# kazuto1011/dusty-gan-v2

Measured on AMD Instinct MI355X. Metric: range-images/sec (G+D step) on dusty_v2 64x512, higher is better.
Workload: dtype bf16; 1 GPU; configs[2]: configs/gans/dusty_v2.yaml full G+D train step (G step + D step + lazy R1 + ADA + EMA + Adam), 64x512 synthetic; global_batch=64, per_gpu_batch=64, parallelism=dp1, hip_graph=True, d_epilogue_dtype=fp32, pe_table_precomputed=True

## Files before the change

dusty-gan-v2_amd/csrc/api.hip:

```cpp
#include "common.h"

extern "C" int dgv2_abi_version(void) { return 53; }
```

dusty-gan-v2_amd/csrc/gemm.hip:

```cpp
#include "gemm_core.h"

namespace {

template <typename T, typename TY, int TO>
int launch_bmm_nn(void* y, const void* x, const void* w, int B, int P, int I, int O, int ldx, int ldy,
                  int64_t wstride, const float* bias, int act, float alpha, float scale, hipStream_t st, float* sumsq,
                  int sumsq_cap, int* sumsq_used, const float* row_scale, const void* resid) {
  constexpr int CE = 16 / sizeof(T);
  DenseRowLoader<T> al{(const T*)w, wstride, I, O, I, (I % CE == 0) && (wstride % CE == 0) && aligned16(w)};
  DenseRowLoader<T> bl{(const T*)x, (int64_t)P * ldx, ldx, P, I, (ldx % CE == 0) && aligned16(x)};
  constexpr int YE = 16 / sizeof(TY);
  StoreEpilogue<TY> epi{(TY*)y, (int64_t)P * ldy, ldy, O, P,
                        (ldy % 4 == 0) && ((reinterpret_cast<uintptr_t>(y) & (4 * sizeof(TY) - 1)) == 0),
                        bias, act, alpha, scale, nullptr, 0.f, row_scale, (const TY*)resid};
  (void)YE;
  dim3 grid((P + 127) / 128, (O + TO - 1) / TO, B);
  const int64_t nblk = (int64_t)grid.x * grid.y * grid.z;
  if (sumsq && sumsq_used && nblk <= sumsq_cap) {
    epi.sumsq = sumsq;
    *sumsq_used = (int)nblk;
  }
  gemm_nn_kernel<T, TO, DenseRowLoader<T>, DenseRowLoader<T>, StoreEpilogue<TY>><<<grid, 256, 0, st>>>(al, bl, epi, I);
  return 0;
}

template <typename T, typename TY>
int dispatch_bmm_nn(void* y, const void* x, const void* w, int B, int P, int I, int O, int ldx, int ldy,
                    int64_t wstride, const float* bias, int act, float alpha, float scale, hipStream_t st, float* sumsq,
                    int sumsq_cap, int* sumsq_used, const float* row_scale, const void* resid) {
  if (O <= 16) return launch_bmm_nn<T, TY, 16>(y, x, w, B, P, I, O, ldx, ldy, wstride, bias, act, alpha, scale, st, sumsq, sumsq_cap, sumsq_used, row_scale, resid);
  if (O <= 32) return launch_bmm_nn<T, TY, 32>(y, x, w, B, P, I, O, ldx, ldy, wstride, bias, act, alpha, scale, st, sumsq, sumsq_cap, sumsq_used, row_scale, resid);
  if (O <= 64) return launch_bmm_nn<T, TY, 64>(y, x, w, B, P, I, O, ldx, ldy, wstride, bias, act, alpha, scale, st, sumsq, sumsq_cap, sumsq_used, row_scale, resid);
  return launch_bmm_nn<T, TY, 128>(y, x, w, B, P, I, O, ldx, ldy, wstride, bias, act, alpha, scale, st, sumsq, sumsq_cap, sumsq_used, row_scale, resid);
}

template <typename T, int TO, int TJ>
int launch_bmm_tn(float* gw, const void* gy, const void* x, int B, int P, int I, int O, int ldgy, int ldx,
                  int ksplit, hipStream_t st) {
  constexpr int CE = 16 / sizeof(T);
  DenseKLoader<T> al{(const T*)gy, (int64_t)P * ldgy, ldgy, O, (ldgy % CE == 0) && aligned16(gy)};
  DenseKLoader<T> bl{(const T*)x, (int64_t)P * ldx, ldx, I, (ldx % CE == 0) && aligned16(x)};
  const int64_t klen = (((int64_t)P + ksplit - 1) / ksplit + 31) / 32 * 32;
  dim3 grid((I + TJ - 1) / TJ, (O + TO - 1) / TO, B * ksplit);
  gemm_tn_kernel<T, TO, TJ, DenseKLoader<T>, DenseKLoader<T>><<<grid, 256, 0, st>>>(al, bl, gw, O, I, P, klen, ksplit,
                                                                                   (int64_t)O * I, I);
  return 0;
}

template <typename T, typename TY, int TO>
int launch_bmm_nn_cat(void* y, const void* xa, const void* xs, const void* w, int B, int P, int Ka, int Ks, int O,
                      const float* bias, int act, float alpha, float scale, hipStream_t st, float* sumsq, int sumsq_cap,
                      int* sumsq_used, const float* row_scale) {
  const int K = Ka + Ks;
  DenseRowLoader<T> al{(const T*)w, (int64_t)O * K, K, O, K, true};
  ConcatRowLoader<T> bl{(const T*)xa, (int64_t)P * Ka, Ka, Ka, (const T*)xs, Ks, Ks, P};
  StoreEpilogue<TY> epi{(TY*)y, (int64_t)P * O, O, O, P, (O % 4 == 0), bias, act, alpha, scale, nullptr, 0.f, row_scale};
  dim3 grid(B, (O + TO - 1) / TO, (P + 127) / 128);
  const int64_t nblk = (int64_t)grid.x * grid.y * grid.z;
  if (sumsq && sumsq_used && nblk <= sumsq_cap) {
    epi.sumsq = sumsq;
    *sumsq_used = (int)nblk;
  }
  gemm_nn_kernel<T, TO, DenseRowLoader<T>, ConcatRowLoader<T>, StoreEpilogue<TY>, true><<<grid, 256, 0, st>>>(al, bl, epi, K);
  return 0;
}

template <typename T, typename TY>
int dispatch_bmm_nn_cat(void* y, const void* xa, const void* xs, const void* w, int B, int P, int Ka, int Ks, int O,
                        const float* bias, int act, float alpha, float scale, hipStream_t st, float* sumsq, int sumsq_cap,
                        int* sumsq_used, const float* row_scale) {
  if (O <= 16) return launch_bmm_nn_cat<T, TY, 16>(y, xa, xs, w, B, P, Ka, Ks, O, bias, act, alpha, scale, st, sumsq, sumsq_cap, sumsq_used, row_scale);
  if (O <= 32) return launch_bmm_nn_cat<T, TY, 32>(y, xa, xs, w, B, P, Ka, Ks, O, bias, act, alpha, scale, st, sumsq, sumsq_cap, sumsq_used, row_scale);
  if (O <= 64) return launch_bmm_nn_cat<T, TY, 64>(y, xa, xs, w, B, P, Ka, Ks, O, bias, act, alpha, scale, st, sumsq, sumsq_cap, sumsq_used, row_scale);
  return launch_bmm_nn_cat<T, TY, 128>(y, xa, xs, w, B, P, Ka, Ks, O, bias, act, alpha, scale, st, sumsq, sumsq_cap, sumsq_used, row_scale);
}

template <typename T, int TO, int TJ>
int launch_bmm_tn_cat(float* gw, const void* gy, const void* xa, const void* xs, int B, int P, int Ca, int Cs, int O,
                      int ksplit, hipStream_t st) {
  constexpr int CE = 16 / sizeof(T);
  const int J = Ca + Cs;
  DenseKLoader<T> al{(const T*)gy, (int64_t)P * O, O, O, (O % CE == 0) && aligned16(gy)};
  ConcatKLoader<T> bl{(const T*)xa, (int64_t)P * Ca, Ca, Ca, (const T*)xs, Cs, Cs};
  const int64_t klen = (((int64_t)P + ksplit - 1) / ksplit + 31) / 32 * 32;
  dim3 grid((J + TJ - 1) / TJ, (O + TO - 1) / TO, B * ksplit);
  gemm_tn_kernel<T, TO, TJ, DenseKLoader<T>, ConcatKLoader<T>><<<grid, 256, 0, st>>>(al, bl, gw, O, J, P, klen, ksplit,
                                                                                  (int64_t)O * J, J);
  return 0;
}

}

extern "C" int dgv2_bmm_nn(void* y, const void* x, const void* w, int B, int P, int I, int O, int ldx, int ldy,
                           int64_t wstride, const float* bias, int act, float alpha, float scale, int dtype,
                           int ydtype, void* stream) {
  return dgv2_bmm_nn_sq(y, x, w, B, P, I, O, ldx, ldy, wstride, nullptr, bias, act, alpha, scale, nullptr, dtype, ydtype,
                        nullptr, 0, nullptr, stream);
}

extern "C" int dgv2_bmm_nn_sq(void* y, const void* x, const void* w, int B, int P, int I, int O, int ldx, int ldy,
                              int64_t wstride, const float* row_scale, const float* bias, int act, float alpha,
                              float scale, const void* resid, int dtype, int ydtype, float* sumsq, int sumsq_cap,
                              int* sumsq_used, void* stream) {
  if (sumsq_used) *sumsq_used = 0;
  if (!y || !x || !w || B <= 0 || P <= 0 || I <= 0 || O <= 0 || ldx < I || ldy < O) return DGV2_EINVAL;
  if (act != 0 && act != 3) return DGV2_EINVAL;
  hipStream_t st = (hipStream_t)stream;
  if (dtype == DGV2_F32 && ydtype == DGV2_F32)
    dispatch_bmm_nn<float, float>(y, x, w, B, P, I, O, ldx, ldy, wstride, bias, act, alpha, scale, st, sumsq, sumsq_cap, sumsq_used, row_scale, resid);
  else if (dtype == DGV2_BF16 && ydtype == DGV2_BF16)
    dispatch_bmm_nn<bf16_t, bf16_t>(y, x, w, B, P, I, O, ldx, ldy, wstride, bias, act, alpha, scale, st, sumsq, sumsq_cap, sumsq_used, row_scale, resid);
  else if (dtype == DGV2_BF16 && ydtype == DGV2_F32)
    dispatch_bmm_nn<bf16_t, float>(y, x, w, B, P, I, O, ldx, ldy, wstride, bias, act, alpha, scale, st, sumsq, sumsq_cap, sumsq_used, row_scale, resid);
  else
    return DGV2_EINVAL;
  DGV2_RETURN_LAST();
}

extern "C" int dgv2_bmm_tn(float* gw, const void* gy, const void* x, int B, int P, int I, int O, int ldgy, int ldx,
                           int dtype, void* stream) {
  if (!gw || !gy || !x || B <= 0 || P <= 0 || I <= 0 || O <= 0 || ldgy < O || ldx < I) return DGV2_EINVAL;
  hipStream_t st = (hipStream_t)stream;
  const int tiles = B * ((O + 63) / 64) * ((I + 127) / 128);
  int ksplit = 1;
  while (tiles * ksplit < 512 && P / (ksplit * 2) >= 512) ksplit *= 2;
  if (ksplit > 1) {
    hipError_t e = hipMemsetAsync(gw, 0, sizeof(float) * (size_t)B * O * I, st);
    if (e != hipSuccess) return (int)e;
  }
  DGV2_DISPATCH_DTYPE(dtype, {
    if (O <= 16) launch_bmm_tn<T, 16, 128>(gw, gy, x, B, P, I, O, ldgy, ldx, ksplit, st);
    else if (O <= 32) launch_bmm_tn<T, 32, 128>(gw, gy, x, B, P, I, O, ldgy, ldx, ksplit, st);
    else launch_bmm_tn<T, 64, 128>(gw, gy, x, B, P, I, O, ldgy, ldx, ksplit, st);
  });
  DGV2_RETURN_LAST();
}

extern "C" int dgv2_bmm_nn_cat(void* y, const void* xa, const void* xs, const void* w, int B, int P, int Ka, int Ks,
                               int O, const float* bias, int act, float alpha, float scale, int dtype, int ydtype,
                               void* stream) {
  return dgv2_bmm_nn_cat_sq(y, xa, xs, w, B, P, Ka, Ks, O, nullptr, bias, act, alpha, scale, dtype, ydtype, nullptr, 0, nullptr,
                            stream);
}

extern "C" int dgv2_bmm_nn_cat_sq(void* y, const void* xa, const void* xs, const void* w, int B, int P, int Ka, int Ks,
                                  int O, const float* row_scale, const float* bias, int act, float alpha, float scale, int dtype, int ydtype,
                                  float* sumsq, int sumsq_cap, int* sumsq_used, void* stream) {
  if (sumsq_used) *sumsq_used = 0;
  if (!y || !xs || !w || (Ka > 0 && !xa) || B <= 0 || P <= 0 || Ka < 0 || Ks <= 0 || O <= 0) return DGV2_EINVAL;
  if (act != 0 && act != 3) return DGV2_EINVAL;
  const int ce = dtype == DGV2_BF16 ? 8 : 4;
  if (Ka % ce || Ks % ce || !aligned16(xs) || (Ka > 0 && !aligned16(xa)) || !aligned16(w) || !aligned16(y))
    return DGV2_EINVAL;
  hipStream_t st = (hipStream_t)stream;
  if (dtype == DGV2_F32 && ydtype == DGV2_F32)
    dispatch_bmm_nn_cat<float, float>(y, xa, xs, w, B, P, Ka, Ks, O, bias, act, alpha, scale, st, sumsq, sumsq_cap, sumsq_used, row_scale);
  else if (dtype == DGV2_BF16 && ydtype == DGV2_BF16)
    dispatch_bmm_nn_cat<bf16_t, bf16_t>(y, xa, xs, w, B, P, Ka, Ks, O, bias, act, alpha, scale, st, sumsq, sumsq_cap, sumsq_used, row_scale);
  else
    return DGV2_EINVAL;
  DGV2_RETURN_LAST();
}

extern "C" int dgv2_bmm_tn_cat(float* gw, const void* gy, const void* xa, const void* xs, int B, int P, int Ka,
                               int Ks, int O, int dtype, void* stream) {
  if (!gw || !gy || !xs || (Ka > 0 && !xa) || B <= 0 || P <= 0 || Ka < 0 || Ks <= 0 || O <= 0) return DGV2_EINVAL;
  const int ce = dtype == DGV2_BF16 ? 8 : 4;
  if (Ka % ce || Ks % ce || !aligned16(xs) || (Ka > 0 && !aligned16(xa))) return DGV2_EINVAL;
  hipStream_t st = (hipStream_t)stream;
  const int J = Ka + Ks;
  const int tiles = B * ((O + 63) / 64) * ((J + 127) / 128);
  int ksplit = 1;
  while (tiles * ksplit < 512 && P / (ksplit * 2) >= 512) ksplit *= 2;
  if (ksplit > 1) {
    hipError_t e = hipMemsetAsync(gw, 0, sizeof(float) * (size_t)B * O * J, st);
    if (e != hipSuccess) return (int)e;
  }
  DGV2_DISPATCH_DTYPE(dtype, {
    if (O <= 16) launch_bmm_tn_cat<T, 16, 128>(gw, gy, xa, xs, B, P, Ka, Ks, O, ksplit, st);
    else if (O <= 32) launch_bmm_tn_cat<T, 32, 128>(gw, gy, xa, xs, B, P, Ka, Ks, O, ksplit, st);
    else launch_bmm_tn_cat<T, 64, 128>(gw, gy, xa, xs, B, P, Ka, Ks, O, ksplit, st);
  });
  DGV2_RETURN_LAST();
}

namespace {

template <typename T, int O>
__global__ __launch_bounds__(256) void bmm_tn_small_kernel(float* __restrict__ gw, const T* __restrict__ gy,
                                                           const T* __restrict__ x, int P, int I, int ppb) {
  constexpr int VN = vec16<T>::N;
  __shared__ float red[256 * VN];
  const int b = blockIdx.y;
  const int cvecs = I / VN, lanes = 256 / cvecs;
  const int cv = threadIdx.x % cvecs, pl = threadIdx.x / cvecs;
  const int p0 = blockIdx.x * ppb, p1 = min(p0 + ppb, P);
  float acc[O][VN];
#pragma unroll
  for (int o = 0; o < O; ++o)
#pragma unroll
    for (int j = 0; j < VN; ++j) acc[o][j] = 0.f;
  const T* xb = x + (int64_t)b * P * I;
  const T* gb = gy + (int64_t)b * P * O;
  constexpr int U = 4;
  for (int p = p0 + pl; p < p1; p += lanes * U) {
    vec16<T> v[U];
    float g[U][O];
#pragma unroll
    for (int u = 0; u < U; ++u) {
      const int q = p + u * lanes;
      const int qc = min(q, p1 - 1);
      v[u].load(xb + (int64_t)qc * I + cv * VN);
#pragma unroll
      for (int o = 0; o < O; ++o) g[u][o] = q < p1 ? to_f32(gb[(int64_t)qc * O + o]) : 0.f;
    }
#pragma unroll
    for (int u = 0; u < U; ++u)
#pragma unroll
      for (int o = 0; o < O; ++o)
#pragma unroll
        for (int j = 0; j < VN; ++j) acc[o][j] = fmaf(g[u][o], v[u].get(j), acc[o][j]);
  }
#pragma unroll
  for (int o = 0; o < O; ++o) {
    __syncthreads();
#pragma unroll
    for (int j = 0; j < VN; ++j) red[threadIdx.x * VN + j] = acc[o][j];
    __syncthreads();
    for (int c = threadIdx.x; c < I; c += 256) {
      const int v = c / VN, j = c - v * VN;
      float s = 0.f;
      for (int k = 0; k < lanes; ++k) s += red[(k * cvecs + v) * VN + j];
      gw[((int64_t)b * O + o) * I + c] = s;
    }
  }
}

}

extern "C" int dgv2_bmm_tn_small(float* gw, const void* gy, const void* x, int B, int P, int I, int O, int dtype,
                                 void* stream) {
  if (!gw || !gy || !x || B <= 0 || P <= 0 || I <= 0 || O <= 0) return DGV2_EINVAL;
  const int vn = dtype == DGV2_BF16 ? 8 : (dtype == DGV2_F32 ? 4 : 0);
  if (!vn) return DGV2_EINVAL;
  if (O > 4 || I % vn || 256 % (I / vn) || !aligned16(x)) return DGV2_ENOTSUP;
  hipStream_t st = (hipStream_t)stream;
  const int ppb = P;
  dim3 grid(1, B);
  DGV2_DISPATCH_DTYPE(dtype, {
    switch (O) {
      case 1: bmm_tn_small_kernel<T, 1><<<grid, 256, 0, st>>>(gw, (const T*)gy, (const T*)x, P, I, ppb); break;
      case 2: bmm_tn_small_kernel<T, 2><<<grid, 256, 0, st>>>(gw, (const T*)gy, (const T*)x, P, I, ppb); break;
      case 3: bmm_tn_small_kernel<T, 3><<<grid, 256, 0, st>>>(gw, (const T*)gy, (const T*)x, P, I, ppb); break;
      default: bmm_tn_small_kernel<T, 4><<<grid, 256, 0, st>>>(gw, (const T*)gy, (const T*)x, P, I, ppb); break;
    }
  });
  DGV2_RETURN_LAST();
}

namespace {

template <typename T, int O, bool ACT>
__global__ __launch_bounds__(256) void bmm_nn_small_kernel(T* __restrict__ y, const T* __restrict__ x,
                                                           const T* __restrict__ w, const T* __restrict__ resid, int P,
                                                           int K, int ppb, const T* __restrict__ ref = nullptr,
                                                           const float* __restrict__ row_scale = nullptr, float alpha = 1.f,
                                                           float ascale = 1.f, float* __restrict__ partial = nullptr) {
  constexpr int VN = vec16<T>::N;
  __shared__ float red[ACT ? 256 * VN : 1];
  const int b = blockIdx.y;
  const int kvecs = K / VN, lanes = 256 / kvecs;
  const int kv = threadIdx.x % kvecs, pl = threadIdx.x / kvecs;
  float wr[VN][O];
#pragma unroll
  for (int j = 0; j < VN; ++j)
#pragma unroll
    for (int o = 0; o < O; ++o) wr[j][o] = to_f32(w[((int64_t)b * K + kv * VN + j) * O + o]);
  const int p0 = blockIdx.x * ppb, p1 = min(p0 + ppb, P);
  const T* xb = x + (int64_t)b * P * O;
  float rs[VN], bsum[VN];
#pragma unroll
  for (int j = 0; j < VN; ++j) {
    rs[j] = (ACT && row_scale) ? row_scale[kv * VN + j] : 1.f;
    bsum[j] = 0.f;
  }
  for (int p = p0 + pl; p < p1; p += lanes) {
    float g[O];
#pragma unroll
    for (int o = 0; o < O; ++o) g[o] = to_f32(xb[(int64_t)p * O + o]);
    const int64_t off = ((int64_t)b * P + p) * K + kv * VN;
    vec16<T> r, f, out;
    if (resid) r.load(resid + off);
    if constexpr (ACT) f.load(ref + off);
#pragma unroll
    for (int j = 0; j < VN; ++j) {
      float s = resid ? r.get(j) : 0.f;
#pragma unroll
      for (int o = 0; o < O; ++o) s = fmaf(g[o], wr[j][o], s);
      if constexpr (ACT) {
        const float v = (f.get(j) > 0.f ? s : s * alpha) * ascale;
        out.set(j, v);
        bsum[j] += out.get(j);
        out.set(j, v * rs[j]);
      } else {
        out.set(j, s);
      }
    }
    out.store(y + off);
  }
  if constexpr (ACT) {
#pragma unroll
    for (int j = 0; j < VN; ++j) red[threadIdx.x * VN + j] = bsum[j];
    __syncthreads();
    for (int c = threadIdx.x; c < K; c += 256) {
      const int v = c / VN, j = c - v * VN;
      float s2 = 0.f;
      for (int t = 0; t < lanes; ++t) s2 += red[(t * kvecs + v) * VN + j];
      partial[((int64_t)blockIdx.y * gridDim.x + blockIdx.x) * K + c] = s2;
    }
  }
}

__global__ __launch_bounds__(256) void small_bias_reduce_kernel(float* __restrict__ gb, const float* __restrict__ partial,
                                                             int nblk, int C) {
  __shared__ float red[16];
  const int c = blockIdx.x;
  float s = 0.f;
#pragma unroll 4
  for (int k = threadIdx.x; k < nblk; k += 256) s += partial[(int64_t)k * C + c];
  s = block_sum(s, red);
  if (threadIdx.x == 0) gb[c] = s;
}

}

namespace {

template <typename T, int O>
__global__ __launch_bounds__(256) void head_bwd_kernel(T* __restrict__ y, const float* __restrict__ gyf,
                                                       const float* __restrict__ cvec, const T* __restrict__ w,
                                                       const T* __restrict__ resid, const T* __restrict__ ref, int P, int K,
                                                       int ppb, const float* __restrict__ row_scale, float alpha,
                                                       float ascale, float* __restrict__ p_gb, float* __restrict__ p_gw,
                                                       float* __restrict__ p_gbh) {
  constexpr int VN = vec16<T>::N;
  __shared__ float red[256 * VN];
  const int b = blockIdx.y;
  const int kvecs = K / VN, lanes = 256 / kvecs;
  const int kv = threadIdx.x % kvecs, pl = threadIdx.x / kvecs;
  float wr[VN][O], cv[O];
#pragma unroll
  for (int j = 0; j < VN; ++j)
#pragma unroll
    for (int o = 0; o < O; ++o) wr[j][o] = to_f32(w[((int64_t)b * K + kv * VN + j) * O + o]);
#pragma unroll
  for (int o = 0; o < O; ++o) cv[o] = cvec[o];
  const int p0 = blockIdx.x * ppb, p1 = min(p0 + ppb, P);
  const float* gb_ = gyf + (int64_t)b * P * O;
  float rs[VN], bsum[VN], hw[O][VN], hb[O];
#pragma unroll
  for (int j = 0; j < VN; ++j) {
    rs[j] = row_scale ? row_scale[kv * VN + j] : 1.f;
    bsum[j] = 0.f;
#pragma unroll
    for (int o = 0; o < O; ++o) hw[o][j] = 0.f;
  }
#pragma unroll
  for (int o = 0; o < O; ++o) hb[o] = 0.f;
  for (int p = p0 + pl; p < p1; p += lanes) {
    float g[O];
#pragma unroll
    for (int o = 0; o < O; ++o) {
      const float raw = gb_[(int64_t)p * O + o];
      if (kv == 0) hb[o] += raw;
      g[o] = to_f32(from_f32<T>(raw * cv[o]));
    }
    const int64_t off = ((int64_t)b * P + p) * K + kv * VN;
    vec16<T> r, f, out;
    if (resid) r.load(resid + off);
    f.load(ref + off);
#pragma unroll
    for (int j = 0; j < VN; ++j) {
      const float xv = f.get(j);
      float s = resid ? r.get(j) : 0.f;
#pragma unroll
      for (int o = 0; o < O; ++o) {
        s = fmaf(g[o], wr[j][o], s);
        hw[o][j] = fmaf(g[o], xv, hw[o][j]);
      }
      const float v = (xv > 0.f ? s : s * alpha) * ascale;
      out.set(j, v);
      bsum[j] += out.get(j);
      out.set(j, v * rs[j]);
    }
    out.store(y + off);
  }
  const int64_t blk = (int64_t)blockIdx.y * gridDim.x + blockIdx.x;
#pragma unroll
  for (int q = 0; q <= O; ++q) {
    __syncthreads();
#pragma unroll
    for (int j = 0; j < VN; ++j) red[threadIdx.x * VN + j] = q == 0 ? bsum[j] : hw[q > 0 ? q - 1 : 0][j];
    __syncthreads();
    for (int c = threadIdx.x; c < K; c += 256) {
      const int v = c / VN, j = c - v * VN;
      float s2 = 0.f;
      for (int t = 0; t < lanes; ++t) s2 += red[(t * kvecs + v) * VN + j];
      if (q == 0) p_gb[blk * K + c] = s2;
      else p_gw[(blk * O + (q - 1)) * K + c] = s2;
    }
  }
  __syncthreads();
#pragma unroll
  for (int o = 0; o < O; ++o) red[threadIdx.x * O + o] = kv == 0 ? hb[o] : 0.f;
  __syncthreads();
  if (threadIdx.x < O) {
    float s2 = 0.f;
    for (int t = 0; t < 256; ++t) s2 += red[t * O + threadIdx.x];
    p_gbh[blk * O + threadIdx.x] = s2;
  }
}

__global__ __launch_bounds__(256) void head_bwd_reduce_kernel(float* __restrict__ gb, float* __restrict__ gw,
                                                              float* __restrict__ gbh, const float* __restrict__ p_gb,
                                                              const float* __restrict__ p_gw, const float* __restrict__ p_gbh,
                                                              int nsplit, int B, int O, int K) {
  __shared__ float red[16];
  const int nblk = nsplit * B;
  int id = blockIdx.x;
  if (id < K) {
    float s = 0.f;
#pragma unroll 4
    for (int k = threadIdx.x; k < nblk; k += 256) s += p_gb[(int64_t)k * K + id];
    s = block_sum(s, red);
    if (threadIdx.x == 0) gb[id] = s;
    return;
  }
  id -= K;
  if (id < B * O) {
    const int b = id / O, o = id - b * O;
    for (int c = threadIdx.x; c < K; c += 256) {
      float s = 0.f;
      for (int k = 0; k < nsplit; ++k) s += p_gw[(((int64_t)b * nsplit + k) * O + o) * K + c];
      gw[((int64_t)b * O + o) * K + c] = s;
    }
    return;
  }
  id -= B * O;
  float s = 0.f;
  for (int k = threadIdx.x; k < nblk; k += 256) s += p_gbh[(int64_t)k * O + id];
  s = block_sum(s, red);
  if (threadIdx.x == 0) gbh[id] = s;
}

}

extern "C" int dgv2_head_bwd(void* y, float* gw, float* gbh, float* gb_up, float* scratch, int64_t scratch_elems,
                             int64_t* blocks_needed, const float* gyf, const float* cvec, const void* w, const void* resid,
                             const void* ref, const float* row_scale, float alpha, float ascale, int B, int P, int O, int K,
                             int dtype, void* stream) {
  if (B <= 0 || P <= 0 || O <= 0 || K <= 0) return DGV2_EINVAL;
  const int vn = dtype == DGV2_BF16 ? 8 : (dtype == DGV2_F32 ? 4 : 0);
  if (!vn) return DGV2_EINVAL;
  if (O > 4 || K % vn || 256 % (K / vn)) return DGV2_ENOTSUP;
  const int lanes = 256 / (K / vn);
  int nsplit = (2048 + B - 1) / B;
  const int minpix = lanes * 8;
  if ((int64_t)nsplit * minpix > P) nsplit = (P + minpix - 1) / minpix;
  nsplit = nsplit < 1 ? 1 : nsplit;
  const int ppb = (P + nsplit - 1) / nsplit;
  dim3 grid((P + ppb - 1) / ppb, B);
  const int64_t nblk = (int64_t)grid.x * grid.y;
  if (blocks_needed) *blocks_needed = nblk;
  if (blocks_needed && !y) return 0;
  if (!y || !gw || !gbh || !gb_up || !scratch || !gyf || !cvec || !w || !ref) return DGV2_EINVAL;
  if (scratch_elems < nblk * ((int64_t)K + (int64_t)O * K + O)) return DGV2_EINVAL;
// ... 67 lines not shown
```

dusty-gan-v2_amd/csrc/gemm_core.h:

```cpp
#pragma once
#include "common.h"

template <typename T> struct Mfma16;

template <> struct Mfma16<bf16_t> {
  __device__ static __forceinline__ void run(f32x4& acc, const uint4& a, const uint4& b) {
    union { uint4 u; bf16x8 v; } ua, ub;
    ua.u = a;
    ub.u = b;
    acc = __builtin_amdgcn_mfma_f32_16x16x32_bf16(ua.v, ub.v, acc, 0, 0, 0);
  }
};

template <> struct Mfma16<fp8_t> {
  __device__ static __forceinline__ void run(f32x4& acc, const uint4& a, const uint4& b) {
    const long a0 = (long)(((unsigned long)a.y << 32) | a.x), a1 = (long)(((unsigned long)a.w << 32) | a.z);
    const long b0 = (long)(((unsigned long)b.y << 32) | b.x), b1 = (long)(((unsigned long)b.w << 32) | b.z);
    acc = __builtin_amdgcn_mfma_f32_16x16x32_fp8_fp8(a0, b0, acc, 0, 0, 0);
    acc = __builtin_amdgcn_mfma_f32_16x16x32_fp8_fp8(a1, b1, acc, 0, 0, 0);
  }
};

template <> struct Mfma16<float> {
  __device__ static __forceinline__ void run(f32x4& acc, const uint4& a, const uint4& b) {
// ... 138 lines not shown
      }
    return v.raw;
  }
};

template <typename T> struct Im2colDgradLoader {
  const T* gy;
  ConvGeom g;
  int Hp, Wp, npix, K;
  bool vec;
  __device__ __forceinline__ const T* src(int b, int hp, int wp, int kk, int& o) const {
    const int tap = kk / g.O;
    o = kk - tap * g.O;
    const int ky = tap / g.kw, kx = tap - ky * g.kw;
    const int nh = hp - ky, nw = wp - kx;
    if (nh < 0 || nw < 0 || nh % g.stride != 0 || nw % g.stride != 0) return nullptr;
    const int ho = nh / g.stride, wo = nw / g.stride;
    if (ho >= g.Ho || wo >= g.Wo) return nullptr;
    return gy + (((int64_t)b * g.Ho + ho) * g.Wo + wo) * g.O;
  }
  __device__ __forceinline__ uint4 load(int, int row, int kchunk) const {
    constexpr int CE = 16 / sizeof(T);
    const int k = kchunk * CE;
    if (row >= npix || k >= K) return make_uint4(0, 0, 0, 0);
    const int wp = row % Wp;
    const int t = row / Wp;
    const int hp = t % Hp;
    const int b = t / Hp;
    int o;
    if (vec) {
      const T* p = src(b, hp, wp, k, o);
      return p ? *reinterpret_cast<const uint4*>(p + o) : make_uint4(0, 0, 0, 0);
    }
    vec16<T> v;
    v.raw = make_uint4(0, 0, 0, 0);
#pragma unroll
    for (int j = 0; j < CE; ++j)
      if (k + j < K) {
        const T* p = src(b, hp, wp, k + j, o);
        if (p) v.e[j] = p[o];
      }
    return v.raw;
  }
};

template <typename T, int TO, class ALoad, class BLoad, class Epi, bool BATCH_FAST = false>
__global__ __launch_bounds__(256) void gemm_nn_kernel(ALoad al, BLoad bl, Epi epi, int K) {
  constexpr int TP = 128;
  constexpr int MF = TO / 16;
  constexpr int NF = 2;
  constexpr int CE = 16 / sizeof(T);
  constexpr int ACH = (TO * 4 + 255) / 256;
  __shared__ __attribute__((aligned(16))) uint4 ldsA[2][TO * 4];
  __shared__ __attribute__((aligned(16))) uint4 ldsB[2][TP * 4];

  const int tid = threadIdx.x;
  const int wave = tid >> 6, lane = tid & 63;
  const int lr = lane & 15, lc = lane >> 4;
  const int batch = BATCH_FAST ? blockIdx.x : blockIdx.z;
  const int m0 = blockIdx.y * TO;
  const int n0 = (BATCH_FAST ? blockIdx.z : blockIdx.x) * TP;
  const int nk = (K + 4 * CE - 1) / (4 * CE);

  uint4 ra[ACH], rb[2];
  auto swz = [](int row, int ch) { return row * 4 + (ch ^ ((row >> 2) & 3)); };
  auto gload = [&](int kt) {
#pragma unroll
    for (int i = 0; i < 2; ++i) {
      const int id = tid + i * 256;
      rb[i] = bl.load(batch, n0 + (id >> 2), kt * 4 + (id & 3));
    }
#pragma unroll
    for (int i = 0; i < ACH; ++i) {
      const int id = tid + i * 256;
      if (id < TO * 4) ra[i] = al.load(batch, m0 + (id >> 2), kt * 4 + (id & 3));
    }
  };
  auto lstore = [&](int buf) {
#pragma unroll
    for (int i = 0; i < 2; ++i) {
      const int id = tid + i * 256;
      ldsB[buf][swz(id >> 2, id & 3)] = rb[i];
    }
#pragma unroll
    for (int i = 0; i < ACH; ++i) {
      const int id = tid + i * 256;
      if (id < TO * 4) ldsA[buf][swz(id >> 2, id & 3)] = ra[i];
    }
  };

  f32x4 acc[MF][NF];
#pragma unroll
  for (int mf = 0; mf < MF; ++mf)
#pragma unroll
    for (int nf = 0; nf < NF; ++nf) acc[mf][nf] = (f32x4){0.f, 0.f, 0.f, 0.f};

  gload(0);
  lstore(0);
  __syncthreads();
  int cur = 0;
  for (int kt = 0; kt < nk; ++kt) {
    if (kt + 1 < nk) gload(kt + 1);
    uint4 a[MF], b[NF];
#pragma unroll
    for (int mf = 0; mf < MF; ++mf) a[mf] = ldsA[cur][swz(mf * 16 + lr, lc)];
#pragma unroll
    for (int nf = 0; nf < NF; ++nf) b[nf] = ldsB[cur][swz(wave * 32 + nf * 16 + lr, lc)];
#pragma unroll
    for (int mf = 0; mf < MF; ++mf)
#pragma unroll
      for (int nf = 0; nf < NF; ++nf) Mfma16<T>::run(acc[mf][nf], a[mf], b[nf]);
    if (kt + 1 < nk) lstore(cur ^ 1);
    __syncthreads();
    cur ^= 1;
  }
#pragma unroll
  for (int mf = 0; mf < MF; ++mf)
#pragma unroll
    for (int nf = 0; nf < NF; ++nf)
      epi(batch, m0 + mf * 16 + lc * 4, n0 + wave * 32 + nf * 16 + lr, acc[mf][nf]);
  if (epi.sumsq) {
    __shared__ float red[16];
    const float s = block_sum(epi.ss, red);
    if (tid == 0) epi.sumsq[(blockIdx.z * gridDim.y + blockIdx.y) * gridDim.x + blockIdx.x] = s;
  }
}

template <typename TY> struct StoreEpilogue {
  TY* y;
  int64_t batch_stride;
  int ld, M, N;
  bool vec;
  const float* bias;
  int act;
  float alpha, scale;
  float* sumsq;
  float ss;
  const float* row_scale;
  const TY* resid;
  __device__ __forceinline__ void operator()(int batch, int m, int n, f32x4 acc) {
    if (n >= N || m >= M) return;
    if (row_scale) {
#pragma unroll
      for (int r = 0; r < 4; ++r)
        if (m + r < M) acc[r] *= row_scale[m + r];
    }
    if (bias || act) {
#pragma unroll
      for (int r = 0; r < 4; ++r) {
        float v = acc[r];
        if (bias && m + r < M) v += bias[m + r];
        if (act == 3) v = (v > 0.f ? v : v * alpha) * scale;
        acc[r] = v;
      }
    }
    TY* p = y + batch * batch_stride + (int64_t)n * ld + m;
    if (resid) {
      const TY* rp = resid + batch * batch_stride + (int64_t)n * ld + m;
      if (vec && m + 3 < M) {
        if constexpr (sizeof(TY) == 4) {
          const f32x4 rv = *reinterpret_cast<const f32x4*>(rp);
#pragma unroll
          for (int r = 0; r < 4; ++r) acc[r] += rv[r];
        } else {
          union { uint2 u; bf16_t e[4]; } rv;
          rv.u = *reinterpret_cast<const uint2*>(rp);
#pragma unroll
          for (int r = 0; r < 4; ++r) acc[r] += (float)rv.e[r];
        }
      } else {
#pragma unroll
        for (int r = 0; r < 4; ++r)
          if (m + r < M) acc[r] += to_f32(rp[r]);
      }
    }
    if (sumsq) {
#pragma unroll
      for (int r = 0; r < 4; ++r)
        if (m + r < M) {
          const float v = to_f32(from_f32<TY>(acc[r]));
          ss = fmaf(v, v, ss);
        }
    }
    if (vec && m + 3 < M) {
      if constexpr (sizeof(TY) == 4) {
        *reinterpret_cast<f32x4*>(p) = acc;
      } else {
        union { uint2 u; bf16_t e[4]; } o;
#pragma unroll
        for (int r = 0; r < 4; ++r) o.e[r] = (bf16_t)acc[r];
        *reinterpret_cast<uint2*>(p) = o.u;
      }
    } else {
#pragma unroll
      for (int r = 0; r < 4; ++r)
        if (m + r < M) p[r] = from_f32<TY>(acc[r]);
    }
  }
};

template <typename T> struct DenseKLoader {
  const T* base;
  int64_t batch_stride;
  int ld, cols;
  bool vec;
  __device__ __forceinline__ uint4 load(int batch, int64_t k, int64_t K, int colchunk) const {
    constexpr int CE = 16 / sizeof(T);
    const int col = colchunk * CE;
    if (k >= K || col >= cols) return make_uint4(0, 0, 0, 0);
    const T* p = base + batch * batch_stride + k * ld + col;
    if (vec && col + CE <= cols) return *reinterpret_cast<const uint4*>(p);
    vec16<T> v;
    v.raw = make_uint4(0, 0, 0, 0);
#pragma unroll
    for (int j = 0; j < CE; ++j)
      if (col + j < cols) v.e[j] = p[j];
    return v.raw;
  }
};

template <typename T> struct ConcatKLoader {
  const T* a;
  int64_t a_batch_stride;
  int lda, Ca;
  const T* s;
  int lds_, Cs;
  __device__ __forceinline__ uint4 load(int batch, int64_t k, int64_t K, int colchunk) const {
    constexpr int CE = 16 / sizeof(T);
    const int col = colchunk * CE;
    if (k >= K) return make_uint4(0, 0, 0, 0);
    if (col < Ca) return *reinterpret_cast<const uint4*>(a + batch * a_batch_stride + k * lda + col);
    const int c2 = col - Ca;
    if (c2 + CE <= Cs) return *reinterpret_cast<const uint4*>(s + k * lds_ + c2);
    return make_uint4(0, 0, 0, 0);
  }
};

template <typename T> struct Im2colWgradLoader {
  const T* x;
  ConvGeom g;
  int cols;
  bool vec;
  __device__ __forceinline__ uint4 load(int, int64_t k, int64_t K, int colchunk) const {
    constexpr int CE = 16 / sizeof(T);
    const int col = colchunk * CE;
    if (k >= K || col >= cols) return make_uint4(0, 0, 0, 0);
    const int wo = (int)(k % g.Wo);
    const int64_t t = k / g.Wo;
    const int ho = (int)(t % g.Ho);
    const int b = (int)(t / g.Ho);
    vec16<T> v;
    v.raw = make_uint4(0, 0, 0, 0);
    if (vec) {
      const int tap = col / g.C, c = col - tap * g.C;
      const int ky = tap / g.kw, kx = tap - ky * g.kw;
      const int hi = conv_src_h(g, ho * g.stride + ky - g.pad);
      const int wi = conv_src_w(g, wo * g.stride + kx - g.pad);
      return *reinterpret_cast<const uint4*>(x + (((int64_t)b * g.H + hi) * g.W + wi) * g.C + c);
    }
#pragma unroll
    for (int j = 0; j < CE; ++j)
      if (col + j < cols) {
        const int cc = col + j;
        const int tap = cc / g.C, c = cc - tap * g.C;
        const int ky = tap / g.kw, kx = tap - ky * g.kw;
        const int hi = conv_src_h(g, ho * g.stride + ky - g.pad);
        const int wi = conv_src_w(g, wo * g.stride + kx - g.pad);
        v.e[j] = x[(((int64_t)b * g.H + hi) * g.W + wi) * g.C + c];
      }
    return v.raw;
  }
};

template <typename T> struct TnFrag;

template <> struct TnFrag<bf16_t> {
  static constexpr int KS = 32;
  template <int ROWLEN>
  __device__ static __forceinline__ uint4 read(const bf16_t* tile, int c0, int lane) {
    const int g = lane >> 4, i = lane & 15;
    const int q = i >> 2, p = i & 3;
    typedef __attribute__((address_space(3))) s16x4 lds_s16x4;
    const bf16_t* a0 = tile + (8 * g + q) * ROWLEN + c0 + 4 * p;
    const bf16_t* a1 = a0 + 4 * ROWLEN;
    union { uint4 u; s16x4 h[2]; } r;
    r.h[0] = __builtin_amdgcn_ds_read_tr16_b64_v4i16((lds_s16x4*)a0);
    r.h[1] = __builtin_amdgcn_ds_read_tr16_b64_v4i16((lds_s16x4*)a1);
    return r.u;
  }
};

template <> struct TnFrag<float> {
  static constexpr int KS = 16;
  template <int ROWLEN>
  __device__ static __forceinline__ uint4 read(const float* tile, int c0, int lane) {
    const int g = lane >> 4, i = lane & 15;
    union { uint4 u; float f[4]; } r;
#pragma unroll
    for (int s = 0; s < 4; ++s) r.f[s] = tile[(4 * s + g) * ROWLEN + c0 + i];
    return r.u;
  }
};

template <typename T, int TO, int TJ, class ALoad, class BLoad>
__global__ __launch_bounds__(256) void gemm_tn_kernel(ALoad al, BLoad bl, float* __restrict__ out, int M, int J,
                                                      int64_t K, int64_t klen, int ksplit, int64_t out_batch_stride,
                                                      int ldo) {
  constexpr int KS = TnFrag<T>::KS;
  constexpr int CE = 16 / sizeof(T);
  constexpr int MF = TO / 16;
  constexpr int NF = TJ / 64;
  constexpr int ACH_ROW = TO / CE, BCH_ROW = TJ / CE;
  constexpr int ACH = (KS * ACH_ROW + 255) / 256, BCH = (KS * BCH_ROW + 255) / 256;
  __shared__ __attribute__((aligned(16))) T ldsA[2][KS * TO];
  __shared__ __attribute__((aligned(16))) T ldsB[2][KS * TJ];

  const int tid = threadIdx.x;
  const int wave = tid >> 6, lane = tid & 63;
  const int batch = blockIdx.z / ksplit;
  const int ks = blockIdx.z % ksplit;
  const int m0 = blockIdx.y * TO;
  const int j0 = blockIdx.x * TJ;
  const int64_t kbeg = ks * klen;
  const int64_t kend = (kbeg + klen < K) ? kbeg + klen : K;
  const int nk = (int)((kend - kbeg + KS - 1) / KS);

  uint4 ra[ACH], rb[BCH];
  auto gload = [&](int kt) {
    const int64_t kb = kbeg + (int64_t)kt * KS;
#pragma unroll
    for (int i = 0; i < ACH; ++i) {
      const int id = tid + i * 256;
      if (id < KS * ACH_ROW) ra[i] = al.load(batch, kb + id / ACH_ROW, kend, (m0 / CE) + id % ACH_ROW);
    }
#pragma unroll
    for (int i = 0; i < BCH; ++i) {
      const int id = tid + i * 256;
      if (id < KS * BCH_ROW) rb[i] = bl.load(batch, kb + id / BCH_ROW, kend, (j0 / CE) + id % BCH_ROW);
    }
  };
  auto lstore = [&](int buf) {
#pragma unroll
    for (int i = 0; i < ACH; ++i) {
      const int id = tid + i * 256;
      if (id < KS * ACH_ROW) reinterpret_cast<uint4*>(ldsA[buf])[id] = ra[i];
    }
#pragma unroll
    for (int i = 0; i < BCH; ++i) {
      const int id = tid + i * 256;
      if (id < KS * BCH_ROW) reinterpret_cast<uint4*>(ldsB[buf])[id] = rb[i];
    }
  };

  f32x4 acc[MF][NF];
#pragma unroll
  for (int mf = 0; mf < MF; ++mf)
#pragma unroll
    for (int nf = 0; nf < NF; ++nf) acc[mf][nf] = (f32x4){0.f, 0.f, 0.f, 0.f};

  if (nk > 0) {
    gload(0);
    lstore(0);
  }
  __syncthreads();
  int cur = 0;
  for (int kt = 0; kt < nk; ++kt) {
    if (kt + 1 < nk) gload(kt + 1);
    uint4 a[MF], b[NF];
#pragma unroll
    for (int mf = 0; mf < MF; ++mf) a[mf] = TnFrag<T>::template read<TO>(ldsA[cur], mf * 16, lane);
#pragma unroll
    for (int nf = 0; nf < NF; ++nf) b[nf] = TnFrag<T>::template read<TJ>(ldsB[cur], wave * (TJ / 4) + nf * 16, lane);
#pragma unroll
    for (int mf = 0; mf < MF; ++mf)
#pragma unroll
      for (int nf = 0; nf < NF; ++nf) Mfma16<T>::run(acc[mf][nf], a[mf], b[nf]);
    if (kt + 1 < nk) lstore(cur ^ 1);
    __syncthreads();
    cur ^= 1;
  }
  const int lr = lane & 15, lc = lane >> 4;
  float* ob = out + batch * out_batch_stride;
#pragma unroll
  for (int mf = 0; mf < MF; ++mf)
#pragma unroll
    for (int nf = 0; nf < NF; ++nf) {
      const int j = j0 + wave * (TJ / 4) + nf * 16 + lr;
      if (j >= J) continue;
#pragma unroll
      for (int r = 0; r < 4; ++r) {
        const int m = m0 + mf * 16 + lc * 4 + r;
        if (m < M) {
          float* p = ob + (int64_t)m * ldo + j;
          if (ksplit > 1) atomicAdd(p, acc[mf][nf][r]);
          else *p = acc[mf][nf][r];
        }
      }
    }
}
```

dusty-gan-v2_amd/dgv2_native/__init__.py:

```python
import ctypes
import os

import torch

_HERE = os.path.dirname(os.path.abspath(__file__))
LIB_PATH = os.environ.get("DGV2_LIB_PATH") or os.path.join(os.path.dirname(_HERE), "lib", "libdgv2.so")

F32, BF16 = 0, 1
ABI_VERSION = 53

_c_int, _c_i64, _c_f32, _c_ptr = ctypes.c_int, ctypes.c_int64, ctypes.c_float, ctypes.c_void_p

SIGNATURES = {
    "dgv2_abi_version": [],
    "dgv2_fused_bias_act": [_c_ptr] * 4 + [_c_i64] * 3 + [_c_int, _c_int, _c_f32, _c_f32, _c_int, _c_ptr],
    "dgv2_bias_grad": [_c_ptr, _c_ptr, _c_i64, _c_i64, _c_i64, _c_int, _c_ptr],
    "dgv2_bias_act_bwd": [_c_ptr] * 4 + [_c_i64, _c_int, _c_f32, _c_f32, _c_ptr, _c_i64, _c_int, _c_ptr],
    "dgv2_bias_act_bwd_rs": [_c_ptr] * 4 + [_c_i64, _c_int, _c_f32, _c_f32, _c_ptr, _c_ptr, _c_i64, _c_int, _c_ptr],
    "dgv2_surface_normal": [_c_ptr, _c_ptr] + [_c_int] * 5 + [_c_ptr],
    "dgv2_mbstd_cat_fwd": [_c_ptr] * 3 + [_c_int] * 7 + [_c_ptr],
    "dgv2_mbstd_cat_bwd": [_c_ptr] * 3 + [_c_int] * 7 + [_c_ptr],
    "dgv2_gemm_x3": [_c_ptr, _c_ptr, _c_i64, _c_ptr, _c_ptr, _c_int, _c_int, _c_i64, _c_int, _c_int, _c_i64, _c_i64, _c_i64,
                     _c_int, _c_f32, _c_ptr],
    "dgv2_pe_wgrad_scratch": [_c_ptr] + [_c_int] * 4,
    "dgv2_pe_wgrad": [_c_ptr, _c_ptr, _c_i64, _c_ptr, _c_ptr] + [_c_int] * 4 + [_c_i64, _c_int, _c_ptr],
    "dgv2_mbstd_cat_fwd_x": [_c_ptr] * 3 + [_c_int] * 8 + [_c_ptr],
    "dgv2_mbstd_cat_bwd_x": [_c_ptr] * 3 + [_c_int] * 8 + [_c_ptr],
    "dgv2_scale_cast": [_c_ptr] * 3 + [_c_i64, _c_int, _c_int, _c_int, _c_ptr],
    "dgv2_upfirdn2d": [_c_ptr] * 3 + [_c_int] * 15 + [_c_ptr],
    "dgv2_resample": [_c_ptr] * 4 + [_c_int] * 19 + [_c_ptr],
    "dgv2_resample_tab": [_c_ptr] * 5 + [_c_int] + [_c_ptr] * 3 + [_c_int] * 10 + [_c_ptr],
    "dgv2_resample_tab_add": [_c_ptr] * 6 + [_c_int] + [_c_ptr] * 3 + [_c_int] * 8 + [_c_ptr],
    "dgv2_resample_tab_add_affine": [_c_ptr] * 8 + [_c_int] + [_c_ptr] * 3 + [_c_int] * 8 + [_c_ptr],
    "dgv2_fourier_feature": [_c_ptr] * 5 + [_c_int] * 8 + [_c_ptr],
    "dgv2_downsample_angle": [_c_ptr] * 4 + [_c_int] * 5 + [_c_ptr],
    "dgv2_bmm_nn": [_c_ptr] * 3 + [_c_int] * 6 + [_c_i64, _c_ptr, _c_int, _c_f32, _c_f32, _c_int, _c_int, _c_ptr],
    "dgv2_bmm_tn": [_c_ptr] * 3 + [_c_int] * 7 + [_c_ptr],
    "dgv2_bmm_nn_cat": [_c_ptr] * 4 + [_c_int] * 5 + [_c_ptr, _c_int, _c_f32, _c_f32, _c_int, _c_int, _c_ptr],
    "dgv2_bmm_nn_cat_sq": [_c_ptr] * 4 + [_c_int] * 5 + [_c_ptr, _c_ptr, _c_int, _c_f32, _c_f32, _c_int, _c_int, _c_ptr, _c_int, _c_ptr,
                           _c_ptr],
    "dgv2_bmm_nn_sq": [_c_ptr] * 3 + [_c_int] * 6 + [_c_i64, _c_ptr, _c_ptr, _c_int, _c_f32, _c_f32, _c_ptr, _c_int, _c_int, _c_ptr, _c_int,
                       _c_ptr, _c_ptr],
    "dgv2_modconv_pe_fwd": [_c_ptr] * 4 + [_c_int] * 5 + [_c_ptr, _c_int, _c_f32, _c_f32, _c_int, _c_ptr],
    "dgv2_modconv_pe_fwd_sq": [_c_ptr] * 4 + [_c_int] * 5 + [_c_ptr, _c_ptr, _c_int, _c_f32, _c_f32, _c_int, _c_ptr, _c_int, _c_ptr,
                               _c_ptr],
    "dgv2_modconv_pe_fwd_head": [_c_ptr] * 4 + [_c_int] * 5 + [_c_ptr, _c_ptr, _c_int, _c_f32, _c_f32, _c_int, _c_ptr, _c_int, _c_ptr,
                                 _c_ptr, _c_ptr, _c_ptr],
    "dgv2_kitti_rows": [_c_ptr, _c_ptr, _c_ptr, _c_int, _c_int, _c_ptr],
    "dgv2_kitti_project": [_c_ptr] * 4 + [_c_int] * 4 + [_c_f32, _c_f32, _c_int, _c_ptr],
    "dgv2_fps_scratch": [_c_ptr, _c_int, _c_int],
    "dgv2_fps": [_c_ptr] * 3 + [_c_int] * 3 + [_c_ptr],
    "dgv2_gather_points": [_c_ptr] * 3 + [_c_int] * 4 + [_c_ptr],
    "dgv2_gather_points_grad": [_c_ptr] * 3 + [_c_int] * 4 + [_c_ptr],
    "dgv2_chamfer_fwd": [_c_ptr] * 6 + [_c_int] * 3 + [_c_ptr],
    "dgv2_nn_search": [_c_ptr] * 4 + [_c_int] * 4 + [_c_ptr],
    "dgv2_chamfer_bwd": [_c_ptr] * 8 + [_c_int] * 3 + [_c_ptr],
    "dgv2_emd_approxmatch": [_c_ptr] * 4 + [_c_int] * 3 + [_c_ptr],
    "dgv2_emd_matchcost": [_c_ptr] * 4 + [_c_int] * 3 + [_c_ptr],
    "dgv2_emd_matchcost_grad": [_c_ptr] * 5 + [_c_int] * 3 + [_c_ptr],
    "dgv2_nsgan_loss": [_c_ptr, _c_ptr, _c_ptr, _c_int, _c_int, _c_f32, _c_ptr, _c_ptr, _c_ptr],
    "dgv2_modconv_pe_dgrad_actbwd": [_c_ptr, _c_ptr, _c_ptr, _c_i64] + [_c_ptr] * 5 + [_c_f32, _c_f32] + [_c_int] * 4 + [_c_ptr],
    "dgv2_colmean_lerp": [_c_ptr, _c_ptr, _c_int, _c_int, _c_i64, _c_f32, _c_ptr],
    "dgv2_d_tail_fwd": [_c_ptr] * 6 + [_c_int, _c_int] + [_c_f32] * 4 + [_c_ptr],
    "dgv2_d_tail_bwd": [_c_ptr] * 7 + [_c_int, _c_int] + [_c_f32] * 4 + [_c_ptr],
    "dgv2_rng_fill": [_c_ptr] * 5 + [_c_int, _c_ptr, _c_ptr],
    "dgv2_modconv_up_fwd": [_c_ptr] * 4 + [_c_int] * 7 + [_c_ptr] * 6 + [_c_int, _c_f32, _c_f32, _c_int, _c_ptr, _c_int, _c_ptr,
                            _c_ptr],
    "dgv2_modconv_up_t_lag": [_c_ptr] * 4 + [_c_f32] + [_c_ptr] * 4 + [_c_int] * 9 + [_c_ptr, _c_int, _c_ptr, _c_ptr],
    "dgv2_fir_same_mfma_q8": [_c_ptr] * 3 + [_c_int] * 4 + [_c_ptr],
    "dgv2_resample_tab_q8": [_c_ptr] * 5 + [_c_int] + [_c_ptr] * 3 + [_c_int] * 7 + [_c_ptr],
    "dgv2_fp8_quant_weights": [_c_ptr] * 6 + [_c_int] + [_c_ptr] * 3,
    "dgv2_fp8_dequant": [_c_ptr, _c_ptr, _c_i64, _c_f32, _c_ptr],
    "dgv2_conv_taps_fp8": [_c_ptr] * 4 + [_c_int] * 14 + [_c_ptr, _c_int, _c_ptr, _c_ptr, _c_int, _c_f32, _c_f32, _c_ptr],
    "dgv2_modconv_up_t": [_c_ptr] * 5 + [_c_f32] + [_c_int] * 9 + [_c_ptr],
    "dgv2_up2_lag_sumsq": [_c_ptr] * 5 + [_c_int] * 5 + [_c_ptr, _c_int, _c_ptr, _c_ptr],
    "dgv2_resample_tab_actbwd": [_c_ptr, _c_ptr, _c_ptr, _c_i64, _c_ptr, _c_ptr, _c_ptr] + [_c_ptr] * 3 + [_c_int] + [_c_ptr] * 3
                                + [_c_int] * 7 + [_c_f32, _c_f32, _c_int, _c_ptr],
    "dgv2_fir_same_mfma_prep": [_c_ptr, _c_i64, _c_ptr] + [_c_ptr] * 3 + [_c_int] + [_c_ptr] * 3 + [_c_int] * 3 + [_c_ptr, _c_ptr],
    "dgv2_fir_same_mfma": [_c_ptr] * 3 + [_c_int] * 4 + [_c_ptr],
    "dgv2_fir_same_mfma_actbwd": [_c_ptr, _c_ptr, _c_ptr, _c_i64, _c_ptr, _c_ptr, _c_ptr, _c_ptr] + [_c_int] * 4
                                 + [_c_f32, _c_f32, _c_ptr],
    "dgv2_resample_tab_sq": [_c_ptr] * 5 + [_c_int] + [_c_ptr] * 3 + [_c_int] * 10 + [_c_ptr, _c_int, _c_ptr, _c_ptr],
    "dgv2_bmm_tn_cat": [_c_ptr] * 4 + [_c_int] * 6 + [_c_ptr],
    "dgv2_lerp_list": [_c_ptr] * 3 + [_c_int, _c_f32, _c_ptr],
    "dgv2_adam_prep": [_c_ptr, _c_ptr, _c_f32, _c_f32, _c_ptr],
    "dgv2_adam_step": [_c_ptr] * 5 + [_c_int, _c_ptr] + [_c_f32] * 4 + [_c_ptr],
    "dgv2_pack2d": [_c_ptr] * 4 + [_c_int] * 3 + [_c_ptr],
    "dgv2_unpack2d": [_c_ptr] * 4 + [_c_int] * 3 + [_c_ptr],
    "dgv2_ema_scalar": [_c_ptr] * 3 + [_c_int] + [_c_f32] * 3 + [_c_int, _c_ptr, _c_int, _c_ptr],
    "dgv2_ema_scalar_group": [_c_ptr, _c_ptr, _c_int, _c_ptr, _c_int] + [_c_f32] * 3 + [_c_int, _c_ptr, _c_ptr],
    "dgv2_bmm_nn_small": [_c_ptr] * 4 + [_c_int] * 5 + [_c_ptr],
    "dgv2_bmm_nn_small_act": [_c_ptr] * 4 + [_c_int] * 4 + [_c_ptr, _c_ptr, _c_f32, _c_f32, _c_ptr, _c_ptr, _c_i64, _c_ptr, _c_int,
                              _c_ptr],
    "dgv2_bmm_tn_small": [_c_ptr] * 3 + [_c_int] * 5 + [_c_ptr],
    "dgv2_head_bwd": [_c_ptr] * 5 + [_c_i64] + [_c_ptr] * 7 + [_c_f32, _c_f32] + [_c_int] * 5 + [_c_ptr],
    "dgv2_transpose_list": [_c_ptr] * 5 + [_c_int] * 3 + [_c_ptr],
    "dgv2_mod_prep_all_fwd": [_c_ptr] * 13 + [_c_ptr, _c_int, _c_int, _c_ptr],
    "dgv2_mod_prep_all_bwd": [_c_ptr, _c_i64] + [_c_ptr] * 15 + [_c_ptr, _c_int, _c_int, _c_ptr, _c_i64, _c_ptr],
    "dgv2_mod_prep_all_bwd_scratch": [_c_ptr, _c_ptr, _c_ptr, _c_int, _c_int],
    "dgv2_mod_prep_fwd": [_c_ptr] * 8 + [_c_int] * 9 + [_c_ptr],
    "dgv2_mod_prep_bwd": [_c_ptr] * 11 + [_c_int] * 9 + [_c_ptr],
    "dgv2_sum_squares": [_c_ptr, _c_ptr, _c_i64, _c_int, _c_int, _c_int, _c_ptr],
    "dgv2_conv_fwd": [_c_ptr] * 3 + [_c_int] * 10 + [_c_ptr, _c_int, _c_f32, _c_f32, _c_int, _c_ptr],
    "dgv2_conv_taps": [_c_ptr] * 3 + [_c_int] * 17 + [_c_ptr] + [_c_int] * 3 + [_c_ptr, _c_ptr, _c_int, _c_f32, _c_f32, _c_int,
                                                                               _c_ptr],
    "dgv2_conv_taps_ex": [_c_ptr] * 3 + [_c_int] * 14 + [_c_ptr, _c_int, _c_int, _c_ptr, _c_int, _c_ptr] + [_c_int] * 3
    + [_c_ptr, _c_ptr, _c_int, _c_f32, _c_f32, _c_int, _c_ptr],
    "dgv2_conv_taps_ld": [_c_ptr, _c_int, _c_ptr, _c_ptr] + [_c_int] * 14 + [_c_ptr, _c_int, _c_int, _c_ptr, _c_int, _c_ptr] + [_c_int] * 3
    + [_c_ptr, _c_ptr, _c_int, _c_f32, _c_f32, _c_int, _c_ptr],
    "dgv2_conv_wgrad_direct": [_c_ptr] * 3 + [_c_int] * 10 + [_c_ptr],
    "dgv2_conv1x1_fwd": [_c_ptr] * 3 + [_c_int] * 4 + [_c_ptr, _c_int, _c_ptr],
    "dgv2_conv1x1_dgrad": [_c_ptr] * 3 + [_c_int] * 4 + [_c_ptr, _c_int, _c_ptr],
    "dgv2_bmm_tn_stream_scratch": [_c_ptr] + [_c_int] * 6,
    "dgv2_bmm_tn_stream": [_c_ptr, _c_ptr, _c_i64, _c_ptr, _c_ptr] + [_c_int] * 6 + [_c_ptr],
    "dgv2_bmm_tn_stream_x": [_c_ptr, _c_ptr, _c_i64, _c_ptr, _c_ptr] + [_c_int] * 7 + [_c_ptr],
    "dgv2_bmm_tn_stream_ld": [_c_ptr, _c_i64, _c_ptr, _c_i64, _c_ptr, _c_ptr] + [_c_int] * 7 + [_c_ptr],
    "dgv2_conv_weight_bank": [_c_ptr] * 8 + [_c_int, _c_int, _c_ptr],
    "dgv2_conv_weight_bank_ex": [_c_ptr] * 10 + [_c_int, _c_int, _c_ptr],
    "dgv2_glin_fwd": [_c_ptr] * 6 + [_c_int] * 3 + [_c_f32, _c_f32, _c_int, _c_f32, _c_int, _c_ptr, _c_ptr],
    "dgv2_glin_dinput": [_c_ptr, _c_int, _c_ptr, _c_i64, _c_ptr, _c_ptr, _c_ptr, _c_ptr, _c_int, _c_int, _c_int, _c_f32, _c_f32,
                         _c_int, _c_ptr],
    "dgv2_glin_dweight": [_c_ptr] * 7 + [_c_int] * 3 + [_c_f32, _c_f32, _c_f32, _c_ptr, _c_ptr],
    "dgv2_conv3x3_dgrad8": [_c_ptr] * 3 + [_c_int] * 5 + [_c_ptr, _c_int, _c_ptr],
    "dgv2_conv3x3_s2_dgrad8": [_c_ptr] * 3 + [_c_int] * 6 + [_c_ptr],
    "dgv2_conv3x3_x3_wgrad_scratch": [_c_ptr] + [_c_int] * 6,
    "dgv2_conv3x3_x3_wgrad": [_c_ptr, _c_ptr, _c_i64] + [_c_ptr] * 2 + [_c_int] * 7 + [_c_f32, _c_int, _c_ptr, _c_ptr],
    "dgv2_conv_x3_images": [_c_ptr] * 3 + [_c_int] * 2 + [_c_ptr],
    "dgv2_conv3x3_x3_dgrad": [_c_ptr] * 4 + [_c_int] * 6 + [_c_ptr, _c_ptr],
    "dgv2_conv3x3_x3_fwd": [_c_ptr] * 3 + [_c_int] * 6 + [_c_ptr, _c_ptr, _c_int, _c_f32, _c_f32, _c_ptr, _c_ptr],
    "dgv2_conv3x3_fwd8": [_c_ptr] * 3 + [_c_int] * 6 + [_c_ptr, _c_ptr, _c_int, _c_f32, _c_f32, _c_int, _c_ptr],
    "dgv2_conv_wgrad_stream_scratch": [_c_ptr] + [_c_int] * 9,
    "dgv2_conv_wgrad_stream": [_c_ptr, _c_ptr, _c_i64, _c_ptr, _c_ptr] + [_c_int] * 10 + [_c_ptr],
    "dgv2_conv_wgrad_stream_pl": [_c_ptr, _c_ptr, _c_i64, _c_ptr, _c_ptr] + [_c_int] * 9 + [_c_f32, _c_int, _c_int, _c_ptr],
    "dgv2_conv_dgrad": [_c_ptr] * 4 + [_c_int] * 11 + [_c_ptr],
    "dgv2_conv_wgrad": [_c_ptr] * 3 + [_c_int] * 11 + [_c_ptr],
    "dgv2_stem_fwd": [_c_ptr] * 4 + [_c_int] * 5 + [_c_f32, _c_f32, _c_int, _c_ptr],
    "dgv2_stem_bwd_scratch": [_c_ptr] + [_c_int] * 4,
    "dgv2_stem_bwd": [_c_ptr] * 4 + [_c_i64] + [_c_ptr] * 4 + [_c_int] * 5 + [_c_f32, _c_f32, _c_int, _c_ptr],
    "dgv2_stem_bwd_skip": [_c_ptr] * 4 + [_c_i64] + [_c_ptr] * 8 + [_c_int] + [_c_ptr] * 3 + [_c_int] * 8 + [_c_f32, _c_f32, _c_int,
                                                                                                        _c_ptr],
    "dgv2_gen_tail_fwd": [_c_ptr] * 7 + [_c_int] * 3 + [_c_f32] * 3 + [_c_ptr],
    "dgv2_gen_tail_bwd": [_c_ptr] * 11 + [_c_int] * 3 + [_c_f32] * 3 + [_c_ptr],
    "dgv2_ada_apply": [_c_ptr] * 8 + [_c_int] * 5 + [_c_ptr],
    "dgv2_ada_sample": [_c_ptr] * 7 + [_c_int] * 3 + [_c_ptr],
    "dgv2_ada_build": [_c_ptr] * 8 + [_c_int] * 4 + [_c_ptr],
    "dgv2_ada_sample_img": [_c_ptr] * 7 + [_c_int, _c_ptr],
    "dgv2_ada_fold": [_c_ptr] * 11 + [_c_int] * 6 + [_c_ptr],
    "dgv2_ada_apply_img": [_c_ptr] * 11 + [_c_int] * 5 + [_c_ptr],
    "dgv2_coords_convert": [_c_ptr] * 4 + [_c_int] * 3 + [_c_f32] * 3 + [_c_int, _c_ptr],
    "dgv2_msml_prepare": [_c_ptr] * 6 + [_c_int] * 5 + [_c_ptr],
    "dgv2_msml_fwd": [_c_ptr] * 7 + [_c_int] * 7 + [_c_ptr],
    "dgv2_msml_bwd": [_c_ptr] * 9 + [_c_int] * 7 + [_c_ptr],
    "dgv2_coords_convert_bwd": [_c_ptr] * 5 + [_c_int] * 3 + [_c_f32, _c_f32, _c_int, _c_ptr],
    "dgv2_fourier_feature_bwd": [_c_ptr] * 6 + [_c_int] * 8 + [_c_ptr],
    "dgv2_frame_points": [_c_ptr] * 4 + [_c_int] * 3 + [_c_f32, _c_f32, _c_int, _c_ptr],
    "dgv2_colorize": [_c_ptr] * 3 + [_c_int] * 4 + [_c_ptr],
    "dgv2_crf_rnn_forward": [_c_ptr] * 11 + [_c_int] * 7 + [_c_ptr],
    "dgv2_crf_rnn_backward_scratch": [_c_ptr] + [_c_int] * 5,
    "dgv2_crf_rnn_backward": [_c_ptr] * 5 + [_c_i64] + [_c_ptr] * 11 + [_c_int] * 7 + [_c_ptr],
    "dgv2_knn2d": [_c_ptr] * 4 + [_c_int] * 7 + [_c_f32, _c_ptr],
    "dgv2_seg_confusion": [_c_ptr] * 4 + [_c_i64, _c_int, _c_ptr],
}


def _load():
    if not os.path.exists(LIB_PATH):
        raise ImportError(
            f"{LIB_PATH} not found: build it with `make` (or __graft_entry__.build()). "
            "The MI355X path has no CPU fallback."
        )
    lib = ctypes.CDLL(LIB_PATH)
    for name, argtypes in SIGNATURES.items():
        fn = getattr(lib, name)
        fn.argtypes = argtypes
        fn.restype = ctypes.c_int
    got = lib.dgv2_abi_version()
    if got != ABI_VERSION:
        raise ImportError(f"libdgv2.so ABI version {got}, binding expects {ABI_VERSION}")
    return lib


lib = _load()


def dtype_code(t):
    if t.dtype == torch.float32:
        return F32
    if t.dtype == torch.bfloat16:
        return BF16
    raise RuntimeError(f"dgv2: unsupported dtype {t.dtype} (float32 / bfloat16 only)")


def check(*tensors):
    for t in tensors:
        if t is None:
            continue
        if not t.is_cuda:
            raise RuntimeError("dgv2: tensor must be a CUDA/HIP tensor (no CPU fallback)")
        if not t.is_contiguous():
            raise RuntimeError("dgv2: tensor must be contiguous")


def ptr(t):
    return None if t is None else t.data_ptr()


def stream():
    return torch.cuda.current_stream().cuda_stream


ENOTSUP = -3


def call(name, *args):
    rc = getattr(lib, name)(*args)
    if rc != 0:
        raise RuntimeError(f"{name} failed with code {rc}")


def try_call(name, *args):
    rc = getattr(lib, name)(*args)
    if rc == ENOTSUP:
        return False
    if rc != 0:
        raise RuntimeError(f"{name} failed with code {rc}")
    return True


STATUS_X_INEXACT, STATUS_FIR_TABLE = 1, 2
_STATUS_TEXT = {
    STATUS_X_INEXACT: "a launch with an x_exact promise (fp32 conv on conv_x3.hip / its weight gradient: 'these input "
                      "channels hold bf16-representable values') staged a value that is not: that launch computed on the "
                      "bf16 rounding of its input",
    STATUS_FIR_TABLE: "dgv2_fir_same_mfma_prep met a table entry outside its contract: the band operands are unusable",
}
_status_words = {}


def status_word(device=None):
    idx = torch.cuda.current_device() if device is None else torch.device(device).index
    idx = torch.cuda.current_device() if idx is None else idx
    w = _status_words.get(idx)
    if w is None:
        if torch.cuda.is_current_stream_capturing():
            raise RuntimeError("dgv2: the status word must exist before a hipGraph capture (call dgv2_native.status_word() "
                               "once outside the capture; gans.trainer.Trainer does)")
        w = _status_words[idx] = torch.zeros(1, device=torch.device("cuda", idx), dtype=torch.int32)
    return w


def status_read(clear=True):
    bits = 0
    for w in _status_words.values():
        v = int(w.item())
        bits |= v
        if v and clear:
            w.zero_()
    return bits


def status_check():
    bits = status_read()
    if bits:
        raise RuntimeError("dgv2: " + "; ".join(t for b, t in _STATUS_TEXT.items() if bits & b))
```

dusty-gan-v2_amd/gans/models/ops/native/misc.py:

```python
import math
import os

import torch
from torch.autograd import Function

import dgv2_native as N
from .act_resample import *
from .modgemm import *
from .conv import *
from .stem_tail_ada import *
from .modlayer import *


def kitti_rows(points, H):
    points = points.contiguous()
    N.check(points)
    n = points.shape[0]
    rows = torch.empty(n, device=points.device, dtype=torch.int32)
    counts = torch.empty((n + 4095) // 4096 + 1, device=points.device, dtype=torch.int32)
    N.call("dgv2_kitti_rows", N.ptr(rows), N.ptr(counts), N.ptr(points), n, int(H), N.stream())
    return rows


def kitti_project(points, rows, H, W, Wout, min_depth, max_depth, apply_mask=True):
# ... 39 lines not shown
    N.check(yf)
    sc, nc = (None, None) if cum is None else cum
    if cum is not None and not all(t.is_cuda and t.dtype == torch.float32 and t.numel() == 1 for t in cum):
        raise ValueError("nsgan_step: cum = (sign_cum, n_pred_cum), fp32 [1] device tensors")
    N.call("dgv2_nsgan_loss", N.ptr(stats), N.ptr(gy), N.ptr(yf), int(n_real), n - int(n_real), float(weight), N.ptr(sc),
           N.ptr(nc), N.stream())
    return stats, gy.reshape(y.shape).to(y.dtype)


_RNG_STATE = {}
RNG_UNIFORM, RNG_NORMAL, RNG_CLAMPED, RNG_BERNOULLI = 0, 1, 2, 3


def rng_state(device=None, seed=None):
    idx = torch.cuda.current_device() if device is None else torch.device(device).index
    idx = torch.cuda.current_device() if idx is None else idx
    st = _RNG_STATE.get(idx)
    if st is None or seed is not None:
        if torch.cuda.is_current_stream_capturing():
            raise RuntimeError("dgv2: the RNG stream must exist before a hipGraph capture (native.rng_state())")
        sd = torch.initial_seed() if seed is None else int(seed)
        vals = torch.tensor([sd & 0x7FFFFFFFFFFFFFFF, 0, 0, 0], dtype=torch.int64)
        if st is None:
            st = _RNG_STATE[idx] = vals.to(torch.device("cuda", idx))
        else:
            st.copy_(vals)
    return st


def rng_fill(specs, device):
    if not 1 <= len(specs) <= 16:
        raise ValueError("rng_fill takes 1..16 segments")
    counts = [int(math.prod(sh)) for sh, _, _, _ in specs]
    offs, tot = [], 0
    for c in counts:
        offs.append(tot)
        tot += (c + 3) // 4 * 4
    st = rng_state(device)
    buf = torch.empty(tot, device=device, dtype=torch.float32)
    outs = [buf[o:o + c].view(sh) for o, c, (sh, _, _, _) in zip(offs, counts, specs)]
    import ctypes as _c
    n = len(specs)
    ptrs = (_c.c_void_p * n)(*[t.data_ptr() for t in outs])
    cnt = (_c.c_int64 * n)(*counts)
    kinds = (_c.c_int * n)(*[int(k) for _, k, _, _ in specs])
    a = (_c.c_float * n)(*[float(v) for _, _, v, _ in specs])
    b = (_c.c_float * n)(*[float(v) for _, _, _, v in specs])
    N.call("dgv2_rng_fill", ptrs, cnt, kinds, a, b, n, N.ptr(st), N.stream())
    return outs


_UP_COMMUTE = os.environ.get("DGV2_NO_UP_COMMUTE") is None


def _spec_cache(spec, name):
    c = spec.__dict__.get(name)
    if c is None:
        c = {}
        setattr(spec, name, c)
    return c


def _up_tables(spec, hl, wl, device):
    key = (hl, wl, str(device))
    _UP_TABLES = _spec_cache(spec, "_dgv2_up_tables")
    if key not in _UP_TABLES:
        (ih, ch, _, Eh), (iw, cw, _, Ew) = spec.tables(hl, wl, False, device)
        if Eh > 2 or Ew > 2:
            return None

        def two(idx, coef, E):
            if E == 2:
                return idx.contiguous(), coef.contiguous()
            return (torch.cat([idx, torch.zeros_like(idx)], dim=1).contiguous(),
                    torch.cat([coef, torch.zeros_like(coef)], dim=1).contiguous())
        ih, ch, iw, cw = two(ih, ch, Eh) + two(iw, cw, Ew)
        wo = iw.shape[0]
        X = torch.arange(wo, device=iw.device)[:, None]
        rel = (iw.long() - ((X // 32) * 16 - 8)) % wl
        ok = wo % 32 == 0 and wl % 8 == 0 and wl >= 32 and bool(((rel < 32) | (cw == 0)).all())
        _UP_TABLES[key] = (ih, ch, iw, cw) if ok else None
    return _UP_TABLES[key]


def _up_gram(spec, hl, wl, device):
    key = (hl, wl, str(device))
    _UP_GRAM = _spec_cache(spec, "_dgv2_up_gram")
    if key not in _UP_GRAM:
        (ih, ch, _, _), (iw, cw, _, _) = spec.tables(hl, wl, False, device)

        def gram(idx, coef, n, ring):
            U = torch.zeros(idx.shape[0], n, dtype=torch.float64)
            U.scatter_add_(1, idx.long().cpu(), coef.double().cpu())
            G = U.T @ U
            d = torch.diagonal(G).clone()
            o = torch.zeros(n, dtype=torch.float64)
            o[:n - 1] = torch.diagonal(G, 1)
            rest = G - torch.diag(d) - torch.diag(o[:n - 1], 1) - torch.diag(o[:n - 1], -1)
            if ring and n > 2:
                o[n - 1] = G[n - 1, 0]
                rest[n - 1, 0] = rest[0, n - 1] = 0.0
            return (d, o) if float(rest.abs().max()) == 0.0 else None
        gh, gw = gram(ih, ch, hl, False), gram(iw, cw, wl, True)
        _UP_GRAM[key] = None if gh is None or gw is None else tuple(
            t.float().to(device).contiguous() for t in (gh[0], gh[1], gw[0], gw[1]))
    return _UP_GRAM[key]


def up2_lag_sumsq(x, spec):
    if x.dtype != torch.bfloat16 or x.shape[3] % 8 or 256 % (x.shape[3] // 8):
        return None
    B, H, W, C = x.shape
    gram = _up_gram(spec, H, W, x.device)
    if gram is None:
        return None
    x = x.contiguous()
    sq = _sq_args(x.device)
    N.check(x)
    if not N.try_call("dgv2_up2_lag_sumsq", N.ptr(x), N.ptr(gram[0]), N.ptr(gram[1]), N.ptr(gram[2]), N.ptr(gram[3]), B,
                      H, W, C, _dt(x), N.ptr(sq[0]), _SQ_CAP, _ct.addressof(sq[1]), N.stream()):
        return None
    return sq[0][:sq[1].value]


def pe_frag16(xs, refresh=False):
    ent = getattr(xs, "_dgv2_frag16", None)
    if ent is not None and ent[0] == xs._version and not refresh:
        return ent[1]
    P, Ks = xs.shape[1] * xs.shape[2], xs.shape[3]
    src = xs.reshape(P // 16, 16, Ks // 32, 4, 8).permute(0, 2, 3, 1, 4)
    if ent is not None and not (xs.is_cuda and torch.cuda.is_current_stream_capturing()):
        ent[1].copy_(src)
        xs._dgv2_frag16 = (xs._version, ent[1])
        return ent[1]
    if refresh:
        return None
    img = src.contiguous()
    if not (xs.is_cuda and torch.cuda.is_current_stream_capturing()):
        xs._dgv2_frag16 = (xs._version, img)
    return img


_UP_O = tuple(int(v) for v in os.environ.get("DGV2_UP_COMMUTE_O", "32,64,128").split(","))


def mod_up_ok(h, xs, wb, spec):
    return bool(_UP_COMMUTE and h is not None and xs is not None and h.is_cuda and h.dtype == torch.bfloat16
                and wb.shape[1] in _UP_O and xs.shape[3] == 512 and h.shape[3] % 8 == 0
                and tuple(a[1] for a in spec.axes) == (2, 2) and tuple(a[2] for a in spec.axes) == (1, 1)
                and h.shape[3] in (64, 128, 256) and h.shape[2] % 32 == 0
                and spec.out_size(h.shape[1], h.shape[2]) == tuple(xs.shape[1:3])
                and _up_tables(spec, h.shape[1], h.shape[2], h.device) is not None)


def resample_sq_only(x, spec):
    x = x.contiguous()
    B, H, W = x.shape[:3]
    Ho, Wo = spec.out_size(H, W)
    (ih_idx, ih_coef, ih_cnt, Eh), (iw_idx, iw_coef, iw_cnt, Ew) = spec.tables(H, W, False, x.device)
    sq = _sq_args(x.device)
    C = x.shape[3]
    N.check(x)
    N.call("dgv2_resample_tab_sq", None, N.ptr(x), N.ptr(ih_idx), N.ptr(ih_coef), N.ptr(ih_cnt), Eh, N.ptr(iw_idx),
           N.ptr(iw_coef), N.ptr(iw_cnt), Ew, B, C, C, C, H, W, Ho, Wo, _dt(x), N.ptr(sq[0]), _SQ_CAP,
           _ct.addressof(sq[1]), N.stream())
    return sq[0][:sq[1].value]


def mod_up_image_shapes(B, hl, wl, Ks, O):
    return (B, hl, O // 16, wl // 8, 16, 8), (B, O // 32, Ks // 32, 2, 4, 16, 8)


def mod_up_images(B, hl, wl, Ks, O, dev, dt, empty=torch.empty):
    st, sw = mod_up_image_shapes(B, hl, wl, Ks, O)
    return empty(st, device=dev, dtype=dt), empty(sw, device=dev, dtype=dt)


def mod_up_prepare(h, xs, wb, spec, act=True, alpha=0.2, scale=math.sqrt(2.0), want_stat=False):
    B, Otot, I = wb.shape
    hl, wl, Ka = h.shape[1:]
    Ks = xs.shape[3]
    dev, dt = h.device, h.dtype
    gram = _up_gram(spec, hl, wl, dev) if want_stat else None
    if want_stat and gram is None:
        return None
    h = h.contiguous()
    t, wimg = mod_up_images(B, hl, wl, Ks, Otot, dev, dt)
    gain = float(scale) * 0.5 * (1.0 + float(alpha)) if act else 1.0
    sq = _sq_args(dev) if want_stat else None
    N.check(h, wb)
    if not N.try_call("dgv2_modconv_up_t_lag", N.ptr(t), N.ptr(wimg), N.ptr(h), N.ptr(wb), gain,
                      *(N.ptr(g) for g in (gram if gram is not None else (None,) * 4)), B, hl, wl, Ka, Ks, Otot, I, Ka,
                      _dt(h), N.ptr(sq[0]) if sq else None, _SQ_CAP if sq else 0,
                      _ct.addressof(sq[1]) if sq else None, N.stream()):
        return None
    return t, wimg, (sq[0][:sq[1].value] if sq else None)


class _ModUpPrepared(Function):
    @staticmethod
    def forward(ctx, cfg, h, xs, bias, handle, wb, cvec, wt, t, wimg):
        ctx.set_materialize_grads(False)
        spec = cfg["spec"]
        h = h.contiguous()
        xs = xs.contiguous()
        dt = h.dtype
        B, Otot, I = wb.shape
        hl, wl, Ka = h.shape[1:]
        H, W_ = xs.shape[1:3]
        Ks = xs.shape[3]
        dev = h.device
        act = 3 if cfg["act"] else 0
        bias32 = None if bias is None else bias.detach().float().contiguous()
        in_scale = None
        if t is not None:
            in_scale = cvec
        else:
            t, wimg = mod_up_images(B, hl, wl, Ks, Otot, dev, dt)
            N.check(h, wb, cvec)
            gain = cfg["scale"] * 0.5 * (1.0 + cfg["alpha"]) if cfg["act"] else 1.0
            N.call("dgv2_modconv_up_t", N.ptr(t), N.ptr(wimg), N.ptr(h), N.ptr(wb), N.ptr(cvec), gain, B, hl, wl, Ka, Ks,
                   Otot, I, Ka, _dt(h), N.stream())
        ih, ch, iw, cw = _up_tables(spec, hl, wl, dev)
        sq = _sq_args(dev) if (cfg["want_sq"] and _FUSED_SQ) else None
        out = torch.empty((B, H, W_, Otot), device=dev, dtype=dt)
        xsf = pe_frag16(xs)
        N.check(t, xsf, wimg, bias32, cvec)
        N.call("dgv2_modconv_up_fwd", N.ptr(out), N.ptr(t), N.ptr(xsf), N.ptr(wimg), B, H, W_, hl, wl, Ks, Otot,
               N.ptr(ih), N.ptr(ch), N.ptr(iw), N.ptr(cw), N.ptr(bias32), N.ptr(in_scale), act, cfg["alpha"],
               cfg["scale"], _dt(h), N.ptr(sq[0]) if sq else None, _SQ_CAP if sq else 0,
               _ct.addressof(sq[1]) if sq else None, N.stream())
        ctx.cfg = dict(cfg, has_bias=bias is not None)
        ctx.save_for_backward(h, xs, wb, out if cfg["act"] else None, cvec, wt)
        if cfg["want_sq"]:
            part = sq[0][:sq[1].value] if (sq is not None and sq[1].value > 0) else sum_squares(out)
            ctx.mark_non_differentiable(part)
            return out, part
        return out

    @staticmethod
    def backward(ctx, gy, *rest):
        cfg = ctx.cfg
        if gy is None:
            return (None,) * 10
        h, xs, wb, out, cvec, wt = ctx.saved_tensors
        spec = cfg["spec"]
        B, Otot, I = wb.shape
        dt = wb.dtype
        gy = gy.contiguous()
        H, W_ = gy.shape[1:3]
        hl, wl, Ka = h.shape[1:]
        P = H * W_
        dev = gy.device
        gb = None
        vn = 8 if gy.dtype == torch.bfloat16 else 4
        rows = gy.numel() // Otot
        link = cfg.get("defer")
        if link is not None and bool(link.get("done")):
            gpre, gb = gy.to(dt), (link.get("gb") if cfg["has_bias"] else None)
            link.clear()
        elif cfg["act"] and gy.dtype == dt and Otot % vn == 0 and 256 % (Otot // vn) == 0:
            gpre = torch.empty((B, H, W_, Otot), device=dev, dtype=dt)
            gb = torch.empty(Otot, device=dev, dtype=torch.float32)
            scratch = torch.empty(2048 * Otot, device=dev, dtype=torch.float32)
            N.call("dgv2_bias_act_bwd_rs", N.ptr(gpre), N.ptr(gb), N.ptr(gy), N.ptr(out), rows, Otot, cfg["alpha"],
                   cfg["scale"], N.ptr(cvec), N.ptr(scratch), scratch.numel(), _dt(gy),
                   N.stream())
            if not cfg["has_bias"]:
                gb = None
        else:
            gpre = torch.empty((B, H, W_, Otot), device=dev, dtype=dt)
            g0 = gy
            if cfg["act"]:
                g0 = _bias_act_raw(gy, None, out, 1, cfg["alpha"], cfg["scale"], 1, Otot)
            if cfg["has_bias"]:
                gb = torch.empty(Otot, device=dev, dtype=torch.float32)
                N.call("dgv2_bias_grad", N.ptr(gb), N.ptr(g0), g0.numel(), 1, Otot, _dt(g0), N.stream())
            N.call("dgv2_scale_cast", N.ptr(gpre), N.ptr(g0), N.ptr(cvec), g0.numel(), Otot, _dt(g0), _dt(gpre),
                   N.stream())
        g3 = gpre.reshape(B, P, Otot)
        need_h, need_w = ctx.needs_input_grad[1], ctx.needs_input_grad[4]
        gh = gwb = None
        if need_h or need_w:
            gt = _resample_raw(gpre, spec, True, (hl, wl))
            gt3 = gt.reshape(B, hl * wl, Otot)
            if need_h:
                if wt is None:
                    wt = wb[:, :, :Ka].transpose(1, 2).contiguous()
                gh = _bmm_nn_raw(gt3, wt, h.dtype).reshape(h.shape)
            Ks = xs.shape[3]
            stream_a = _TN_STREAM and Ka % 8 == 0 and Otot % 8 == 0 and hl * wl >= 2048
            if need_w and stream_a and (Ka + Ks) % 4 == 0 and Ka % 4 == 0:
                gwb = torch.empty((B, Otot, Ka + Ks), device=dev, dtype=torch.float32)
                if pe_wgrad(g3, xs.reshape(H * W_, -1), out=gwb, col0=Ka) is not None:
                    _bmm_tn_stream(gt3, h, B, hl, wl, Ka, Otot, out=gwb)
                else:
                    gwb = None
            if need_w and gwb is None:
                h3 = h.reshape(B, hl * wl, Ka)
                if stream_a:
                    gwa = _bmm_tn_stream(gt3, h, B, hl, wl, Ka, Otot)
                else:
                    gwa = torch.empty((B, Otot, Ka), device=dev, dtype=torch.float32)
                    N.call("dgv2_bmm_tn", N.ptr(gwa), N.ptr(gt3), N.ptr(h3), B, hl * wl, Ka, Otot, Otot, Ka, _dt(h),
                           N.stream())
                gws = _mod_wgrad(g3, None, xs, B, H, W_, xs.shape[3], Otot, dt)
                gwb = torch.cat([gwa, gws], dim=2)
        return None, gh, None, gb, gwb, None, None, None, None, None


def mod_up_layer(h, xs, spec, handle, wb, cvec, bias=None, act=True, alpha=0.2, scale=math.sqrt(2.0), want_sq=False,
                 wt=None, pre=None, defer=None):
    cfg = dict(act=bool(act), alpha=float(alpha), scale=float(scale) if act else 1.0, want_sq=bool(want_sq), spec=spec,
               defer=defer)
    t, wimg = (None, None) if pre is None else pre[:2]
    return _ModUpPrepared.apply(cfg, h, xs, bias, handle, wb, cvec, wt, t, wimg)


def mod_gemm_layer(xa, xs, handle, wb, cvec, bias=None, act=True, alpha=0.2, scale=math.sqrt(2.0), out_dtype=None,
                   want_sq=False, wt=None, fork=False, defer=None, upstream=None, head_w=None, pre_d=None,
                   defer_affine=False):
    ref = xa if xa is not None else xs
    cfg = dict(act=bool(act), alpha=float(alpha), scale=float(scale) if act else 1.0,
               out_dtype=ref.dtype if out_dtype is None else out_dtype, want_sq=bool(want_sq),
               fork=bool(fork and xa is not None and xa.requires_grad), defer=defer, upstream=upstream,
               defer_affine=bool(defer_affine))
    if pre_d is not None and pre_d.numel() == 0:
        pre_d = None
    return _ModGemmPrepared.apply(cfg, xa, xs, bias, handle, wb, cvec, wt, head_w, pre_d)



__all__ = [n_ for n_ in dir() if not n_.startswith("__")]
```

dusty-gan-v2_amd/gans/models/ops/native/modgemm.py:

```python
import math
import contextlib
import os

import torch
from torch.autograd import Function

import dgv2_native as N
from .act_resample import *
from .inversion import fourier_feature_bwd


def _ptr_array(tensors):
    return (_ct.c_void_p * len(tensors))(*[None if t is None else t.data_ptr() for t in tensors])


def _int_array(vals):
    return (_ct.c_int * len(vals))(*[int(v) for v in vals])


class _Pack2d(Function):

    @staticmethod
    def forward(ctx, Rmax, Cmax, *ts):
        ts = [t.detach().float().contiguous() for t in ts]
        rows, cols = [t.shape[0] for t in ts], [t.shape[1] for t in ts]
        out = torch.empty((len(ts), Rmax, Cmax), device=ts[0].device, dtype=torch.float32)
        N.call("dgv2_pack2d", N.ptr(out), _ptr_array(ts), _int_array(rows), _int_array(cols), len(ts), Rmax, Cmax,
               N.stream())
        ctx.cfg = (rows, cols)
        return out

    @staticmethod
    def backward(ctx, g):
        rows, cols = ctx.cfg
        return (None, None) + tuple(_Unpack2d.apply(g, tuple(rows), tuple(cols)))


class _Unpack2d(Function):

    @staticmethod
    def forward(ctx, packed, rows, cols):
        packed = packed.contiguous()
        L, Rmax, Cmax = packed.shape
        outs = [torch.empty((rows[l], cols[l]), device=packed.device, dtype=torch.float32) for l in range(L)]
        N.call("dgv2_unpack2d", _ptr_array(outs), N.ptr(packed), _int_array(rows), _int_array(cols), L, Rmax, Cmax,
               N.stream())
        ctx.cfg = (Rmax, Cmax, rows, cols)
        return tuple(outs)

    @staticmethod
    def backward(ctx, *gs):
        Rmax, Cmax, rows, cols = ctx.cfg
        dev = next(g.device for g in gs if g is not None)
        gs = [None if g is None else g.contiguous().float() for g in gs]
        out = torch.empty((len(gs), Rmax, Cmax), device=dev, dtype=torch.float32)
        N.call("dgv2_pack2d", N.ptr(out), _ptr_array(gs), _int_array(rows), _int_array(cols), len(gs), Rmax, Cmax,
               N.stream())
        return out, None, None


_KIDX_CACHE = {}



_GLIN = os.environ.get("DGV2_NO_GLIN") is None
_GLIN_GRAD = os.environ.get("DGV2_GLIN_GRAD") is not None
_GLIN_GRAD_CTX = [False]
_GLIN_MAX = 24


@contextlib.contextmanager
def glin_grad(on=True):
    old = _GLIN_GRAD_CTX[0]
    _GLIN_GRAD_CTX[0] = bool(on) and os.environ.get("DGV2_NO_GLIN_GRAD") is None
    try:
        yield
    finally:
        _GLIN_GRAD_CTX[0] = old


def glin_wanted(*tensors):
    return _GLIN and (_GLIN_GRAD or _GLIN_GRAD_CTX[0]
                      or not (torch.is_grad_enabled() and any(t is not None and t.requires_grad for t in tensors)))


def _ptrs(ptrs):
    return (_ct.c_void_p * len(ptrs))(*[None if v is None else int(v) for v in ptrs])


class _GroupedLinear(Function):

    @staticmethod
    def forward(ctx, cfg, x, *wb):
        L = len(wb) // 2
        ws_, bs_ = wb[:L], wb[L:]
        alpha, beta, act, slope, prenorm, kidx = cfg
        x = x.contiguous() if x.dim() == 2 else x
        B, K = x.shape[0], x.shape[-1]
        if x.dim() == 3:
            sB, sS = x.stride(0), x.stride(1)
            xptr = [x.data_ptr() + 4 * kidx[l] * sS for l in range(L)]
            lda = [sB] * L
        else:
            xptr, lda = [x.data_ptr()] * L, [x.stride(0)] * L
        Ns = [w.shape[0] for w in ws_]
        ys = [torch.empty((B, n), device=x.device, dtype=torch.float32) for n in Ns]
        rn = torch.empty(B, device=x.device, dtype=torch.float32) if prenorm else None
        N.check(*ws_, *[b for b in bs_ if b is not None])
        N.call("dgv2_glin_fwd", _ptr_array(ys), _ptrs(xptr), _ptr_array(ws_), _ptr_array(bs_), _int_array(Ns),
               _int_array(lda), L, B, K, float(alpha), float(beta), int(act), float(slope), int(prenorm), N.ptr(rn),
               N.stream())
        ctx.cfg = (cfg, L, Ns, xptr, lda)
        ctx.save_for_backward(x, rn, *ws_, *(ys if act else ()))
        ctx.has_bias = [b is not None for b in bs_]
        return tuple(ys)

    @staticmethod
    @torch.autograd.function.once_differentiable
    def backward(ctx, *gs):
        (alpha, beta, act, slope, prenorm, kidx), L, Ns, xptr, lda = ctx.cfg
        saved = ctx.saved_tensors
        x, rn, ws_ = saved[0], saved[1], saved[2:2 + L]
        ys = saved[2 + L:] if act else [None] * L
        B, K = x.shape[0], x.shape[-1]
        dev = x.device
        live = [l for l in range(L) if gs[l] is not None]

        def al16(t):
            t = t.contiguous().float()
            return t if t.data_ptr() % 16 == 0 else t.clone()
        gs = [None if g is None else al16(g) for g in gs]
        gws = [None] * L
        gbs = [None] * L
        if live and any(ctx.needs_input_grad[2 + l] or ctx.needs_input_grad[2 + L + l] for l in live):
            for l in live:
                gws[l] = torch.empty((Ns[l], K), device=dev, dtype=torch.float32)
                gbs[l] = torch.empty(Ns[l], device=dev, dtype=torch.float32) if ctx.has_bias[l] else None
            N.call("dgv2_glin_dweight", _ptr_array([gws[l] for l in live]), _ptr_array([gbs[l] for l in live]),
                   _ptr_array([gs[l] for l in live]), _ptr_array([ys[l] for l in live]), _ptrs([xptr[l] for l in live]),
                   _int_array([Ns[l] for l in live]), _int_array([lda[l] for l in live]), len(live), B, K, float(alpha),
                   float(beta), float(slope), N.ptr(rn), N.stream())
        gx = None
        if ctx.needs_input_grad[1] and live:
            if prenorm:
                raise RuntimeError("dgv2: gradient w.r.t. the input of a pixel-normalised grouped Linear is not built")
            chunks = lambda sel: sum((Ns[l] + 255) // 256 for l in sel)
            if x.dim() == 2:
                gx = torch.empty((B, K), device=dev, dtype=torch.float32)
                scratch = torch.empty(chunks(live) * B * K, device=dev, dtype=torch.float32)
                N.call("dgv2_glin_dinput", N.ptr(gx), K, N.ptr(scratch), scratch.numel(), _ptr_array([gs[l] for l in live]),
                       _ptr_array([ys[l] for l in live]), _ptr_array([ws_[l] for l in live]), _int_array([Ns[l] for l in live]),
                       len(live), B, K, float(alpha), float(slope), 0, N.stream())
            else:
                S = x.shape[1]
                gx = torch.zeros((B, S, K), device=dev, dtype=torch.float32)
                for sidx in sorted({kidx[l] for l in live}):
                    sel = [l for l in live if kidx[l] == sidx]
                    scratch = torch.empty(chunks(sel) * B * K, device=dev, dtype=torch.float32)
                    N.call("dgv2_glin_dinput", gx.data_ptr() + 4 * sidx * K, S * K, N.ptr(scratch), scratch.numel(),
                           _ptr_array([gs[l] for l in sel]), _ptr_array([ys[l] for l in sel]), _ptr_array([ws_[l] for l in sel]),
                           _int_array([Ns[l] for l in sel]), len(sel), B, K, float(alpha), float(slope), 0, N.stream())
        return (None, gx) + tuple(gws) + tuple(gbs)


def grouped_linear(x, weights, biases, alpha, beta=1.0, act=False, slope=0.2, prenorm=False, kidx=None):
    L = len(weights)
    K = x.shape[-1]
    ok = (_GLIN and x.is_cuda and x.dtype == torch.float32 and 1 <= L <= _GLIN_MAX and K % 64 == 0 and x.stride(-1) == 1
          and all(w.dtype == torch.float32 and w.is_contiguous() and w.shape[1] == K and w.shape[0] % 32 == 0 for w in weights)
          and (x.dim() == 2 or (x.dim() == 3 and kidx is not None and x.stride(0) % 4 == 0 and x.stride(1) % 4 == 0)))
    if not ok:
        return None
    cfg = (float(alpha), float(beta), bool(act), float(slope), bool(prenorm), None if kidx is None else tuple(kidx))
    return _GroupedLinear.apply(cfg, x, *weights, *biases)


def style_affines(ws, weights, biases, kidx, scale):
    if ws.dtype == torch.float32 and len(weights) <= _GLIN_MAX and glin_wanted(ws, *weights, *biases):
        x = ws[:, 0] if (ws.stride(1) == 0 or ws.shape[1] == 1) else ws
        out = grouped_linear(x, weights, biases, scale, 1.0, kidx=None if x.dim() == 2 else kidx)
        if out is not None:
            return list(out)
    B, S, K = ws.shape
    L = len(weights)
    Is = [w.shape[0] for w in weights]
    Imax = max(Is)
    Wp = _Pack2d.apply(Imax, K, *weights)
    bp = _Pack2d.apply(1, Imax, *[b.reshape(1, -1) for b in biases])
    key = (tuple(kidx), str(ws.device))
    if key not in _KIDX_CACHE:
        _KIDX_CACHE[key] = torch.tensor(list(kidx), device=ws.device, dtype=torch.long)
    X = ws.float().transpose(0, 1).index_select(0, _KIDX_CACHE[key])
    Sout = torch.baddbmm(bp, X, Wp.transpose(1, 2), alpha=float(scale))
    return list(_Unpack2d.apply(Sout, tuple([B] * L), tuple(Is)))


def lerp_list(dst, src, weight):
    for i in range(0, len(dst), 72):
        d, s_ = dst[i:i + 72], src[i:i + 72]
        N.check(*d, *s_)
        N.call("dgv2_lerp_list", _ptr_array(d), _ptr_array(s_), _int_array([t.numel() for t in d]), len(d),
               float(weight), N.stream())


def fused_adam_step(opt):
    (group,) = opt.param_groups
    if group["weight_decay"] != 0 or group["amsgrad"] or group["maximize"]:
        raise RuntimeError("dgv2 fused Adam: unsupported optimizer options")
    params = [p for p in group["params"] if p.grad is not None]
    if not params:
        return
    dev = params[0].device
    shared = getattr(opt, "_dgv2_step", None)
    if shared is None:
        shared = torch.zeros(1, device=dev, dtype=torch.float32)
        opt._dgv2_step = shared
        opt._dgv2_sc = torch.zeros(4, device=dev, dtype=torch.float32)
    for p in params:
        st = opt.state[p]
        if len(st) == 0:
            st["step"] = shared.view(())
            st["exp_avg"] = torch.zeros_like(p, memory_format=torch.preserve_format)
            st["exp_avg_sq"] = torch.zeros_like(p, memory_format=torch.preserve_format)
        elif st["step"].data_ptr() != shared.data_ptr():
            shared.copy_(st["step"].reshape(1).to(dev, torch.float32))
            st["step"] = shared.view(())
    b1, b2 = group["betas"]
    N.call("dgv2_adam_prep", N.ptr(opt._dgv2_sc), N.ptr(shared), float(b1), float(b2), N.stream())
    for i in range(0, len(params), 72):
        ch = params[i:i + 72]
        ms = [opt.state[p]["exp_avg"] for p in ch]
        vs = [opt.state[p]["exp_avg_sq"] for p in ch]
        gs = [p.grad for p in ch]
        N.check(*ch, *gs, *ms, *vs)
        N.call("dgv2_adam_step", _ptr_array(ch), _ptr_array(gs), _ptr_array(ms), _ptr_array(vs),
               _int_array([p.numel() for p in ch]), len(ch), N.ptr(opt._dgv2_sc), float(group["lr"]), float(b1),
               float(b2), float(group["eps"]), N.stream())


def ema_update(ema, sumsq, add, count, weight, update=True, cvec=None):
    snap = None if cvec is not None else torch.empty(1, device=ema.device, dtype=torch.float32)
    N.call("dgv2_ema_scalar", N.ptr(ema), N.ptr(snap), N.ptr(sumsq), 0 if sumsq is None else sumsq.numel(), float(add),
           1.0 / float(count), float(weight), int(update), N.ptr(cvec), 0 if cvec is None else cvec.numel(), N.stream())
    return snap if cvec is None else cvec


def ema_update_group(emas, rows, sumsq, add, count, weight, update, cvec):
    assert 1 <= len(emas) <= 8 and cvec is not None and cvec.numel() >= sum(rows)
    N.check(*emas, cvec, sumsq)
    N.call("dgv2_ema_scalar_group", _ptr_array(emas), _int_array(rows), len(emas), N.ptr(sumsq),
           0 if sumsq is None else sumsq.numel(), float(add), 1.0 / float(count), float(weight), int(update), N.ptr(cvec),
           N.stream())
    return cvec


class _UpCatPE(Function):
    @staticmethod
    def forward(ctx, h, spec, angle, shift, freqs2, phase, dtype, B):
        F2 = 2 * phase.numel()
        if h is None:
            H, W = angle.shape[2:]
            Cin = 0
        else:
            h = h.contiguous()
            B = h.shape[0]
            Cin = h.shape[3]
            H, W = spec.out_size(h.shape[1], h.shape[2])
        x1 = torch.empty((B, H, W, Cin + F2), device=angle.device, dtype=dtype)
        if h is not None:
            _resample_raw(h, spec, False, (h.shape[1], h.shape[2]), out=x1, ldy=Cin + F2)
        angle_d = angle.detach().float().contiguous()
        fourier_feature_into(x1, Cin, angle_d, shift, freqs2, phase)
        ctx.cfg = (spec, None if h is None else (h.shape[1], h.shape[2]), Cin)
        ctx.pe = (angle_d, shift, freqs2, phase) if ctx.needs_input_grad[2] else None
        return x1

    @staticmethod
    def backward(ctx, g):
        spec, in_hw, Cin = ctx.cfg
        g = g.contiguous()
        gh = ga = None
        if in_hw is not None and ctx.needs_input_grad[0]:
            gh = _resample_raw(g, spec, True, in_hw, ldx=g.shape[3], C=Cin)
        if ctx.pe is not None:
            ga = fourier_feature_bwd(g, Cin, *ctx.pe)
        return gh, None, ga, None, None, None, None, None


def up_cat_pe(h, spec, angle, shift, freqs2, phase, dtype, B):
    return _UpCatPE.apply(h, spec, angle, shift, freqs2, phase, dtype, B)


_HEAD_FWD = os.environ.get("DGV2_NO_HEAD_FWD") is None
_PE_FREE_MINP = {(64, 32): 4096, (32, 64): 4096, (32, 32): 4096, (64, 64): 4096, (128, 64): 2048, (64, 128): 2048,
                 (128, 128): 1024, (256, 256): 512, (256, 128): 512, (128, 256): 512}
if os.environ.get("DGV2_NO_PE_MID"):
    _PE_FREE_MINP = {k: 4096 for k in ((64, 32), (32, 64), (128, 64), (64, 128), (32, 32), (64, 64))}


def _bmm_nn_raw(x3, w3, out_dtype, bias=None, act=0, alpha=0.2, scale=1.0, sq=None, row_scale=None, resid=None, head=None):
    B, P, I = x3.shape
    Bw, O, _ = w3.shape
    N.check(x3, w3, bias)
    y = torch.empty((B, P, O), device=x3.device, dtype=out_dtype)
    if I <= 4 and Bw == B and bias is None and act == 0 and sq is None and row_scale is None and out_dtype == x3.dtype:
        r = None if resid is None else resid.contiguous().to(out_dtype)
        if N.try_call("dgv2_bmm_nn_small", N.ptr(y), N.ptr(x3), N.ptr(w3), N.ptr(r), B, P, I, O, _dt(x3), N.stream()):
            return y
    if (resid is None and _PE_FWD and Bw == B and x3.dtype == torch.bfloat16 and out_dtype == torch.bfloat16
            and P >= _PE_FREE_MINP.get((I, O), 1 << 30)):
        if (head is not None and _HEAD_FWD and head[0].dtype == torch.bfloat16 and tuple(head[0].shape) == (B, 2, O)
                and head[0].is_contiguous()):
            hd = torch.empty((B, P, 2), device=x3.device, dtype=torch.float32)
            if N.try_call("dgv2_modconv_pe_fwd_head", N.ptr(y), N.ptr(x3), None, N.ptr(w3), B, P, I, 0, O, N.ptr(row_scale),
                          N.ptr(bias), act, alpha, scale, _dt(x3), N.ptr(sq[0]) if sq else None, _SQ_CAP if sq else 0,
                          _ct.addressof(sq[1]) if sq else None, N.ptr(head[0]), N.ptr(hd), N.stream()):
                head[1] = hd
                return y
        if sq is not None or row_scale is not None:
            N.call("dgv2_modconv_pe_fwd_sq", N.ptr(y), N.ptr(x3), None, N.ptr(w3), B, P, I, 0, O, N.ptr(row_scale),
                   N.ptr(bias), act, alpha, scale, _dt(x3), N.ptr(sq[0]) if sq else None, _SQ_CAP if sq else 0,
                   _ct.addressof(sq[1]) if sq else None, N.stream())
            return y
        N.call("dgv2_modconv_pe_fwd", N.ptr(y), N.ptr(x3), None, N.ptr(w3), B, P, I, 0, O, N.ptr(bias), act, alpha,
               scale, _dt(x3), N.stream())
        return y
    if sq is not None or row_scale is not None or resid is not None:
        if resid is not None:
            resid = resid.contiguous().to(out_dtype)
            N.check(resid)
        N.call("dgv2_bmm_nn_sq", N.ptr(y), N.ptr(x3), N.ptr(w3), B, P, I, O, I, O, 0 if Bw == 1 else O * I,
               N.ptr(row_scale), N.ptr(bias), act, alpha, scale, N.ptr(resid), _dt(x3), N.dtype_code(y),
               N.ptr(sq[0]) if sq else None, _SQ_CAP if sq else 0, _ct.addressof(sq[1]) if sq else None, N.stream())
        return y
    N.call("dgv2_bmm_nn", N.ptr(y), N.ptr(x3), N.ptr(w3), B, P, I, O, I, O, 0 if Bw == 1 else O * I,
           N.ptr(bias), act, alpha, scale, _dt(x3), N.dtype_code(y), N.stream())
    return y


def _bmm_tn_raw(gy3, x3):
    B, P, O = gy3.shape
    I = x3.shape[2]
    N.check(gy3, x3)
    gw = torch.empty((B, O, I), device=x3.device, dtype=torch.float32)
    N.call("dgv2_bmm_tn", N.ptr(gw), N.ptr(gy3), N.ptr(x3), B, P, I, O, O, I, _dt(x3), N.stream())
    return gw


class _ModGemm(Function):

    @staticmethod
    def forward(ctx, x, w, out_dtype):
        shp = x.shape
        x3 = x.contiguous().reshape(shp[0], -1, shp[-1])
        wc = _values(w, x.dtype)
        y = _bmm_nn_raw(x3, wc, out_dtype)
        ctx.save_for_backward(x3, wc)
        ctx.cfg = (shp, w.shape[0] == 1)
        return y.reshape(*shp[:-1], w.shape[1])

    @staticmethod
    def backward(ctx, gy):
        x3, wc = ctx.saved_tensors
        shp, shared = ctx.cfg
        gy3 = gy.contiguous().reshape(x3.shape[0], -1, wc.shape[1]).to(x3.dtype)
        gx = gw = None
        if ctx.needs_input_grad[0]:
            wt = wc.transpose(1, 2).contiguous()
            gx = _bmm_nn_raw(gy3, wt, x3.dtype).reshape(shp)
        if ctx.needs_input_grad[1]:
            if shared:
                gw = _bmm_tn_raw(gy3.reshape(1, -1, gy3.shape[2]), x3.reshape(1, -1, x3.shape[2]))
            else:
                gw = _bmm_tn_raw(gy3, x3)
        return gx, gw, None


def mod_gemm(x, w, out_dtype=None):
    return _ModGemm.apply(x, w, x.dtype if out_dtype is None else out_dtype)


class _ModGemmAct(Function):

    @staticmethod
    def forward(ctx, x, w, bias, alpha, scale):
        shp = x.shape
        x3 = x.contiguous().reshape(shp[0], -1, shp[-1])
        wc = _values(w, x.dtype)
        out = _bmm_nn_raw(x3, wc, x.dtype, bias.detach().float().contiguous(), 3, alpha, scale)
        ctx.save_for_backward(x3, wc, out)
        ctx.cfg = (shp, w.shape[0] == 1, alpha, scale, bias.numel())
        return out.reshape(*shp[:-1], w.shape[1])

    @staticmethod
    def backward(ctx, gy):
        x3, wc, out = ctx.saved_tensors
        shp, shared, alpha, scale, size_b = ctx.cfg
        gpre, gb = _BiasActBackward.apply(gy.contiguous().reshape(out.shape), out, True, alpha, scale, 1, size_b)
        gx = gw = None
        if ctx.needs_input_grad[0]:
            gx = _bmm_nn_raw(gpre, wc.transpose(1, 2).contiguous(), x3.dtype).reshape(shp)
        if ctx.needs_input_grad[1]:
            if shared:
                gw = _bmm_tn_raw(gpre.reshape(1, -1, gpre.shape[2]), x3.reshape(1, -1, x3.shape[2]))
            else:
                gw = _bmm_tn_raw(gpre, x3)
        return gx, gw, gb, None, None


def mod_gemm_act(x, w, bias, alpha=0.2, scale=math.sqrt(2.0)):
    return _ModGemmAct.apply(x, w, bias, float(alpha), float(scale))


class _ModGemmCatAct(Function):

    @staticmethod
    def forward(ctx, xa, xs, w, bias, alpha, scale):
        B, O = w.shape[0], w.shape[1]
        _, H, W_, Ks = xs.shape
        Ka = 0 if xa is None else xa.shape[3]
        xs = xs.contiguous()
        xa = None if xa is None else xa.contiguous()
        wc = w.detach().to(xs.dtype).contiguous()
        bias32 = bias.detach().float().contiguous()
        N.check(xa, xs, wc, bias32)
        out = torch.empty((B, H, W_, O), device=xs.device, dtype=xs.dtype)
        N.call("dgv2_bmm_nn_cat", N.ptr(out), N.ptr(xa), N.ptr(xs), N.ptr(wc), B, H * W_, Ka, Ks, O, N.ptr(bias32),
               3, alpha, scale, _dt(xs), _dt(xs), N.stream())
        ctx.save_for_backward(xa, xs, wc, out)
        ctx.cfg = (alpha, scale, Ka, Ks)
        return out

    @staticmethod
    def backward(ctx, gy):
        xa, xs, wc, out = ctx.saved_tensors
        alpha, scale, Ka, Ks = ctx.cfg
        B, H, W_, O = out.shape
        gpre, gb = _BiasActBackward.apply(gy.contiguous(), out, True, alpha, scale, 1, O)
        gxa = gw = None
        g3 = gpre.reshape(B, H * W_, O)
        if xa is not None and ctx.needs_input_grad[0]:
            wt = wc[:, :, :Ka].transpose(1, 2).contiguous()
            gxa = _bmm_nn_raw(g3, wt, xa.dtype).reshape(xa.shape)
        if ctx.needs_input_grad[2]:
            gw = torch.empty((B, O, Ka + Ks), device=out.device, dtype=torch.float32)
            N.call("dgv2_bmm_tn_cat", N.ptr(gw), N.ptr(g3), N.ptr(xa), N.ptr(xs), B, H * W_, Ka, Ks, O, _dt(xs),
                   N.stream())
        return gxa, None, gw, gb, None, None


def mod_gemm_cat_act(xa, xs, w, bias, alpha=0.2, scale=math.sqrt(2.0)):
    return _ModGemmCatAct.apply(xa, xs, w, bias, float(alpha), float(scale))


_PE_FWD = os.environ.get("DGV2_NO_PE_FWD") is None


def _values(w, dtype):
    if getattr(w, "_dgv2_bank", None) is not None:
        raise RuntimeError("conv weight handle without values: run this pass without the weight bank "
                           "(Discriminator.forward(double_backward=True))")
    if w.dtype == dtype and w.is_contiguous():
        return w.detach()
    c = getattr(w, "_dgv2_vals", None)
    if c is not None and c[0] == w._version and c[1].dtype == dtype:
        return c[1]
    v = w.detach().to(dtype).contiguous()
    w._dgv2_vals = (w._version, v)
    return v

__all__ = [n_ for n_ in dir() if not n_.startswith("__")]
```

dusty-gan-v2_amd/gans/models/ops/native/modlayer.py:

```python
import math
import os

import torch
from torch.autograd import Function

import dgv2_native as N
from .act_resample import *
from .modgemm import *
from .conv import *
from .stem_tail_ada import *


def _bmm_tn_stream(g3, xa, B, H, W_, I, O, shared=False, out=None):
    key = (B, H, W_, I, O)
    if key not in _TN_SCRATCH:
        n = _ct.c_int64(0)
        N.call("dgv2_bmm_tn_stream_scratch", _ct.addressof(n), B, H, W_, I, O, _dt(xa))
        _TN_SCRATCH[key] = n.value
    gw = torch.empty((B, O, I), device=xa.device, dtype=torch.float32) if out is None else out
    ld = 0 if out is None else int(out.shape[2])
    scratch = torch.empty(_TN_SCRATCH[key], device=xa.device, dtype=torch.float32)
    N.call("dgv2_bmm_tn_stream_ld", N.ptr(gw), ld, N.ptr(scratch), scratch.numel(), N.ptr(g3), N.ptr(xa), int(shared), B, H,
           W_, I, O, _dt(xa), N.stream())
    return gw


class _ModLayer(Function):
    @staticmethod
    def forward(ctx, cfg, xa, xs, bias, shift, fw, *mods):
        ctx.set_materialize_grads(False)
        nm = len(mods) // 3
        Ws = [mods[3 * k].detach().contiguous() for k in range(nm)]
        Ss = [mods[3 * k + 1].detach().float().contiguous() for k in range(nm)]
        Es = [(mods[3 * k + 2].detach() if mods[3 * k + 2].ndim == 1 else mods[3 * k + 2].detach().float().reshape(1).clone())
              for k in range(nm)]
        ref = xa if xa is not None else xs
        dt = ref.dtype
        B = Ss[0].shape[0]
        I = Ws[0].shape[1]
        Os = [w.shape[0] for w in Ws]
        Otot = sum(Os)
        H, W_ = ref.shape[1:3]
        P = H * W_
        dev = ref.device
        wb = torch.empty((B, Otot, I), device=dev, dtype=dt)
        rot = shift is not None and cfg["F"] > 0
        saved_small = []
        off = 0
        for k in range(nm):
            stats = torch.empty(2 + 2 * B, device=dev, dtype=torch.float32)
            dsave = torch.empty((B, Os[k]), device=dev, dtype=torch.float32)
            N.call("dgv2_mod_prep_fwd", N.ptr(wb), N.ptr(dsave), N.ptr(stats), N.ptr(Ws[k]), N.ptr(Ss[k]), N.ptr(Es[k]),
                   N.ptr(shift) if rot else None, N.ptr(fw) if rot else None, B, Os[k], I, Otot, off,
                   int(cfg["demod"][k]), cfg["cin"], cfg["F"] if rot else 0, _dt(wb), N.stream())
            saved_small += [stats, dsave]
            off += Os[k]
        act = 3 if cfg["act"] else 0
        bias32 = None if bias is None else bias.detach().float().contiguous()
        odt = cfg["out_dtype"]
        sq = _sq_args(dev) if (cfg["want_sq"] and _FUSED_SQ) else None
        if xs is not None:
            xs = xs.contiguous()
            xa = None if xa is None else xa.contiguous()
            Ka = 0 if xa is None else xa.shape[3]
            out = torch.empty((B, H, W_, Otot), device=dev, dtype=dt)
            N.check(xa, xs, wb, bias32)
            if _PE_FWD and dt == torch.bfloat16 and (Ka, xs.shape[3], Otot) in ((64, 512, 32), (128, 512, 64), (256, 512, 128)):
                N.call("dgv2_modconv_pe_fwd_sq", N.ptr(out), N.ptr(xa), N.ptr(xs), N.ptr(wb), B, P, Ka, xs.shape[3],
                       Otot, None, N.ptr(bias32), act, cfg["alpha"], cfg["scale"], _dt(xs), N.ptr(sq[0]) if sq else None,
                       _SQ_CAP if sq else 0, _ct.addressof(sq[1]) if sq else None, N.stream())
            else:
                N.call("dgv2_bmm_nn_cat_sq", N.ptr(out), N.ptr(xa), N.ptr(xs), N.ptr(wb), B, P, Ka, xs.shape[3], Otot,
                       None, N.ptr(bias32), act, cfg["alpha"], cfg["scale"], _dt(xs), _dt(xs),
                       N.ptr(sq[0]) if sq else None, _SQ_CAP if sq else 0, _ct.addressof(sq[1]) if sq else None,
                       N.stream())
        else:
            xa = xa.contiguous()
            out = _bmm_nn_raw(xa.reshape(B, P, I), wb, odt, bias32, act, cfg["alpha"], cfg["scale"], sq=sq).reshape(
                B, H, W_, Otot)
        ctx.cfg = dict(cfg, Os=Os, I=I, B=B, rot=rot, has_bias=bias is not None)
        ctx.save_for_backward(xa, xs, wb, out if cfg["act"] else None, shift, fw, *Ws, *Ss, *Es, *saved_small)
        if cfg["want_sq"]:
            part = sq[0][:sq[1].value] if (sq is not None and sq[1].value > 0) else sum_squares(out)
            ctx.mark_non_differentiable(part)
            return out, part
        return out

    @staticmethod
    def backward(ctx, gy, _=None):
        cfg = ctx.cfg
        Os, I, B, rot = cfg["Os"], cfg["I"], cfg["B"], cfg["rot"]
        if gy is None:
            return (None,) * (6 + 3 * len(Os))
        nm = len(Os)
        sv = ctx.saved_tensors
        xa, xs, wb, out, shift, fw = sv[:6]
        Ws, Ss, Es = sv[6:6 + nm], sv[6 + nm:6 + 2 * nm], sv[6 + 2 * nm:6 + 3 * nm]
        small = sv[6 + 3 * nm:]
        Otot = sum(Os)
        dt = wb.dtype
        gy = gy.contiguous()
        H, W_ = gy.shape[1:3]
        P = H * W_
        gb = None
        if cfg["act"]:
            gpre, gb = _BiasActBackward.apply(gy, out, cfg["has_bias"], cfg["alpha"], cfg["scale"], 1, Otot)
        else:
            gpre = gy.to(dt)
            if cfg["has_bias"]:
                gb = torch.empty(Otot, device=gy.device, dtype=torch.float32)
                N.call("dgv2_bias_grad", N.ptr(gb), N.ptr(gy), gy.numel(), 1, Otot, _dt(gy), N.stream())
        g3 = gpre.reshape(B, P, Otot)
        Ka = 0 if xa is None else xa.shape[3]
        gxa = None
        if xa is not None and ctx.needs_input_grad[1]:
            wt = wb[:, :, :Ka].transpose(1, 2).contiguous()
            gxa = _bmm_nn_raw(g3, wt, xa.dtype).reshape(xa.shape)
        gwb = None
        if xs is not None and _LIB_WGRAD and dt == torch.bfloat16 and P >= 2048:
            gT = g3.transpose(1, 2)
            parts = []
            if xa is not None and _TN_STREAM and Ka % 8 == 0 and Otot % 8 == 0:
                parts.append(_bmm_tn_stream(g3, xa, B, H, W_, Ka, Otot))
            elif xa is not None:
                parts.append(torch.bmm(gT, xa.reshape(B, P, Ka), out_dtype=torch.float32))
            gws = pe_wgrad(g3, xs.reshape(P, -1))
            parts.append(gws if gws is not None else
                         torch.bmm(gT, xs.reshape(1, P, -1).expand(B, P, xs.shape[3]), out_dtype=torch.float32))
            gwb = torch.cat(parts, dim=2) if len(parts) > 1 else parts[0]
        if gwb is not None:
            pass
        elif xs is not None:
            gwb = torch.empty((B, Otot, I), device=gy.device, dtype=torch.float32)
            N.call("dgv2_bmm_tn_cat", N.ptr(gwb), N.ptr(g3), N.ptr(xa), N.ptr(xs), B, P, Ka, xs.shape[3], Otot,
                   _dt(xs), N.stream())
        elif _TN_STREAM and dt == torch.bfloat16 and P >= 2048 and I % 8 == 0 and Otot % 8 == 0:
            gwb = _bmm_tn_stream(g3, xa, B, H, W_, I, Otot)
        else:
            gwb = torch.empty((B, Otot, I), device=gy.device, dtype=torch.float32)
            N.call("dgv2_bmm_tn", N.ptr(gwb), N.ptr(g3), N.ptr(xa.reshape(B, P, I)), B, P, I, Otot, Otot, I, _dt(xa),
                   N.stream())
        grads = []
        off = 0
        for k in range(nm):
            ncorr = min(Os[k] * B, 8192)
            buf = torch.empty(Os[k] * I + B * I + ncorr, device=gy.device, dtype=torch.float32)
            gW = buf[:Os[k] * I].view(Os[k], I)
            gs = buf[Os[k] * I:Os[k] * I + B * I].view(B, I)
            corr = buf[Os[k] * I + B * I:]
            N.call("dgv2_mod_prep_bwd", N.ptr(gW), N.ptr(gs), N.ptr(corr), N.ptr(gwb), N.ptr(Ws[k]), N.ptr(Ss[k]),
                   N.ptr(small[2 * k]), N.ptr(small[2 * k + 1]), N.ptr(Es[k]), N.ptr(shift) if rot else None,
                   N.ptr(fw) if rot else None, B, Os[k], I, Otot, off, int(cfg["demod"][k]), cfg["cin"],
                   cfg["F"] if rot else 0, ncorr, N.stream())
            grads += [gW, gs, None]
            off += Os[k]
        return (None, gxa, None, gb, None, None, *grads)


def mod_layer(xa, xs, mods, bias=None, act=True, alpha=0.2, scale=math.sqrt(2.0), out_dtype=None, shift=None,
              fw=None, cin=0, want_sq=False):
    ref = xa if xa is not None else xs
    cfg = dict(act=bool(act), alpha=float(alpha), scale=float(scale) if act else 1.0,
               out_dtype=ref.dtype if out_dtype is None else out_dtype, demod=[bool(m[3]) for m in mods], cin=int(cin),
               F=0 if fw is None else int(fw.numel()), want_sq=bool(want_sq))
    flat = []
    for W, s, ev, _ in mods:
        flat += [W, s, ev]
    return _ModLayer.apply(cfg, xa, xs, bias, shift, fw, *flat)


class _ModPrepAll(Function):
    @staticmethod
    def forward(ctx, meta, shift, *flat):
        ctx.set_materialize_grads(False)
        L = len(meta["layers"])
        Ws = [flat[2 * l].detach().contiguous() for l in range(L)]
        Ss = [flat[2 * l + 1].detach().float().contiguous() for l in range(L)]
        B = Ss[0].shape[0]
        dev = Ws[0].device
        wbs = [torch.empty((B, g["Otot"], g["I"]), device=dev, dtype=g["dtype"]) for g in meta["groups"]]
        lay = meta["layers"]
        dflat = torch.empty(sum(B * m["O"] for m in lay), device=dev, dtype=torch.float32)
        dsaves, off = [], 0
        for m in lay:
            dsaves.append(dflat[off:off + B * m["O"]])
            off += B * m["O"]
        stats = torch.empty(L * (2 + 2 * B), device=dev, dtype=torch.float32)
        rot_tab = torch.empty(L * B * 512, device=dev, dtype=torch.float32)
        fws = [m["fw"] for m in lay]
        rot = shift is not None
        flags = [(1 if m["demod"] else 0) | (2 if (rot and m["fw"] is not None) else 0)
                 | (4 if meta["groups"][m["group"]]["dtype"] == torch.bfloat16 else 0) for m in lay]
        ints = dict(O=_int_array([m["O"] for m in lay]), I=_int_array([m["I"] for m in lay]),
                    Otot=_int_array([meta["groups"][m["group"]]["Otot"] for m in lay]),
                    row_off=_int_array([m["row_off"] for m in lay]), cin=_int_array([m["cin"] for m in lay]),
                    flags=_int_array(flags))
        N.check(*Ws, *Ss, shift, *[f for f in fws if f is not None])
        N.call("dgv2_mod_prep_all_fwd", _ptr_array([wbs[m["group"]] for m in lay]), _ptr_array(dsaves), N.ptr(stats),
               N.ptr(rot_tab), _ptr_array(Ws), _ptr_array(Ss), _ptr_array(fws), ints["O"], ints["I"], ints["Otot"], ints["row_off"],
               ints["cin"], ints["flags"], N.ptr(shift) if rot else None, B, L, N.stream())
        ctx.meta, ctx.ints, ctx.B, ctx.rot = meta, ints, B, rot
        ctx.save_for_backward(shift, stats, dflat, rot_tab, *Ws, *Ss)
        handles = [torch.empty(1, device=dev, dtype=torch.float32).expand(B, g["Otot"], g["I"]) for g in meta["groups"]]
        wts = [torch.empty((B, g.get("Ka", 0), g["Otot"]) if (meta["want_wt"] and g.get("Ka", 0) > 0) else (0,),
                           device=dev, dtype=g["dtype"]) for g in meta["groups"]]
        idx = [k for k, t in enumerate(wts) if t.numel() > 0]
        for es in (2, 4):
            sel = [k for k in idx if wts[k].element_size() == es]
            if sel:
                N.call("dgv2_transpose_list", _ptr_array([wts[k] for k in sel]), _ptr_array([wbs[k] for k in sel]),
                       _int_array([meta["groups"][k]["Otot"] for k in sel]), _int_array([meta["groups"][k]["Ka"] for k in sel]),
                       _int_array([meta["groups"][k]["I"] for k in sel]), len(sel), B, es, N.stream())
        ctx.mark_non_differentiable(*wbs, *wts)
        return (*handles, *wbs, *wts)

    @staticmethod
    def backward(ctx, *grads):
        meta, ints, B = ctx.meta, ctx.ints, ctx.B
        lay, groups = meta["layers"], meta["groups"]
        L, ng = len(lay), len(groups)
        sv = ctx.saved_tensors
        shift, stats, dflat, rot_tab = sv[:4]
        Ws, Ss = sv[4:4 + L], sv[4 + L:4 + 2 * L]
        dev = stats.device
        Gs = []
        for k, g in enumerate(groups):
            gk = grads[k]
            Gs.append(torch.zeros((B, g["Otot"], g["I"]), device=dev) if gk is None else gk.float().contiguous())
        sizes, ncorr = [], []
        for m in lay:
            nc = min(m["O"] * B, 8192)
            ncorr.append(nc)
            sizes.append((m["O"] * m["I"] + B * m["I"] + nc + 3) // 4 * 4)
        flat = torch.empty(sum(sizes), device=dev, dtype=torch.float32)
        outs, off = [], 0
        for n in sizes:
            outs.append(flat[off:off + n])
            off += n
        dsaves, off = [], 0
        for m in lay:
            dsaves.append(dflat[off:off + B * m["O"]])
            off += B * m["O"]
        key = ("prep_all_bwd", tuple((m["O"], m["I"]) for m in lay), B)
        if key not in _TN_SCRATCH:
            n = _ct.c_int64(0)
            N.call("dgv2_mod_prep_all_bwd_scratch", _ct.addressof(n), ints["O"], ints["I"], B, L)
            _TN_SCRATCH[key] = n.value
        scratch = torch.empty(_TN_SCRATCH[key], device=dev, dtype=torch.float32)
        N.call("dgv2_mod_prep_all_bwd", N.ptr(flat), flat.numel(), _ptr_array(outs), _int_array(ncorr),
               _ptr_array([Gs[m["group"]] for m in lay]), _ptr_array(list(Ws)), _ptr_array(list(Ss)), N.ptr(stats),
               N.ptr(rot_tab), _ptr_array(dsaves), _ptr_array([m["fw"] for m in lay]), ints["O"], ints["I"], ints["Otot"],
               ints["row_off"], ints["cin"], ints["flags"], N.ptr(shift) if ctx.rot else None, B, L, N.ptr(scratch),
               scratch.numel(), N.stream())
        res = []
        for m, o in zip(lay, outs):
            OI, BI = m["O"] * m["I"], B * m["I"]
            res += [o[:OI].view(m["O"], m["I"]), o[OI:OI + BI].view(B, m["I"])]
        return (None, None, *res)


def mod_prep_all(layers, groups, shift):
    want_wt = torch.is_grad_enabled() and any(m["W"].requires_grad or m["s"].requires_grad for m in layers)
    meta = dict(layers=[{k: v for k, v in m.items() if k not in ("W", "s")} for m in layers], groups=groups,
                want_wt=want_wt)
    flat = []
    for m in layers:
        flat += [m["W"], m["s"]]
    out = _ModPrepAll.apply(meta, shift, *flat)
    ng = len(groups)
    wts = [t if t.numel() > 0 else None for t in out[2 * ng:]]
    return list(zip(out[:ng], out[ng:2 * ng], wts))


class _ModGemmPrepared(Function):

    @staticmethod
    def forward(ctx, cfg, xa, xs, bias, handle, wb, cvec, wt=None, head_w=None, pre_d=None):
        ctx.set_materialize_grads(False)
        ref = xa if xa is not None else xs
        dt = ref.dtype
        B, Otot, I = wb.shape
        H, W_ = ref.shape[1:3]
        P = H * W_
        dev = ref.device
        act = 3 if cfg["act"] else 0
        bias32 = None if bias is None else bias.detach().float().contiguous()
        odt = cfg["out_dtype"]
        sq = _sq_args(dev) if (cfg["want_sq"] and _FUSED_SQ) else None
        N.check(xa, xs, wb, bias32, cvec)
        if xs is not None:
            xs = xs.contiguous()
            xa = None if xa is None else xa.contiguous()
            Ka = 0 if xa is None else xa.shape[3]
            out = torch.empty((B, H, W_, Otot), device=dev, dtype=dt)
            tail = (N.ptr(sq[0]) if sq else None, _SQ_CAP if sq else 0, _ct.addressof(sq[1]) if sq else None, N.stream())
            if _PE_FWD and dt == torch.bfloat16 and (Ka, xs.shape[3], Otot) in ((64, 512, 32), (128, 512, 64), (256, 512, 128)):
                N.call("dgv2_modconv_pe_fwd_sq", N.ptr(out), N.ptr(xa), N.ptr(xs), N.ptr(wb), B, P, Ka, xs.shape[3],
                       Otot, N.ptr(cvec), N.ptr(bias32), act, cfg["alpha"], cfg["scale"], _dt(xs), *tail)
            else:
                N.call("dgv2_bmm_nn_cat_sq", N.ptr(out), N.ptr(xa), N.ptr(xs), N.ptr(wb), B, P, Ka, xs.shape[3], Otot,
                       N.ptr(cvec), N.ptr(bias32), act, cfg["alpha"], cfg["scale"], _dt(xs), _dt(xs), *tail)
        elif pre_d is not None and not cfg["act"] and not cfg["want_sq"]:
            xa = xa.contiguous()
            if cfg.get("defer_affine"):
                out = pre_d.reshape(B, H, W_, Otot).view(B, H, W_, Otot)
            else:
                b0 = bias32 if bias32 is not None else torch.zeros(Otot, device=dev)
                out = torch.addcmul(b0, pre_d.reshape(B, H, W_, Otot), cvec).to(odt)
        else:
            xa = xa.contiguous()
            head = [head_w, None] if head_w is not None else None
            out = _bmm_nn_raw(xa.reshape(B, P, I), wb, odt, bias32, act, cfg["alpha"], cfg["scale"], sq=sq,
                              row_scale=cvec, head=head).reshape(B, H, W_, Otot)
        ctx.cfg = dict(cfg, has_bias=bias is not None)
        ctx.save_for_backward(xa, xs, wb, out if cfg["act"] else None, cvec, wt)
        outs = [out]
        if cfg["want_sq"]:
            part = sq[0][:sq[1].value] if (sq is not None and sq[1].value > 0) else sum_squares(out)
            ctx.mark_non_differentiable(part)
            outs.append(part)
        if head_w is not None:
            hd = head[1].reshape(B, H, W_, 2) if (xs is None and pre_d is None and head[1] is not None) else \
                torch.empty(0, device=dev, dtype=torch.float32)
            ctx.mark_non_differentiable(hd)
            outs.append(hd)
        if cfg["fork"]:
            outs.append(xa.view_as(xa))
        return outs[0] if len(outs) == 1 else tuple(outs)

    @staticmethod
    def backward(ctx, gy, *rest):
        cfg = ctx.cfg
        g_sib = rest[-1] if cfg["fork"] else None
        if gy is None:
            return (None, g_sib) + (None,) * 8
        xa, xs, wb, out, cvec, wt = ctx.saved_tensors
        B, Otot, I = wb.shape
        dt = wb.dtype
        gy = gy.contiguous()
        if (not cfg["act"] and cfg["fork"] and cfg.get("upstream") is not None and xs is None and xa is not None
                and wt is not None and not torch.is_grad_enabled() and ctx.needs_input_grad[1] and ctx.needs_input_grad[4]):
            fused = _head_bwd_fused(gy, cvec, wt, g_sib, xa, cfg["upstream"])
            if fused is not None:
                gxa, gwb, gbh = fused
                return None, gxa, None, (gbh if cfg["has_bias"] else None), gwb, None, None, None, None, None
        H, W_ = gy.shape[1:3]
        P = H * W_
        dev = gy.device
        gb = None
        vn = 8 if gy.dtype == torch.bfloat16 else 4
        rows = gy.numel() // Otot
        link = cfg.get("defer")
        deferred = link is not None and bool(link.get("done"))
        if deferred:
            gpre, gb = gy.to(dt), (link.get("gb") if cfg["has_bias"] else None)
            link.clear()
        else:
            gpre = torch.empty((B, H, W_, Otot), device=dev, dtype=dt)
        if deferred:
            pass
        elif cfg["act"] and gy.dtype == dt and Otot % vn == 0 and 256 % (Otot // vn) == 0:
            gb = torch.empty(Otot, device=dev, dtype=torch.float32)
            scratch = torch.empty(2048 * Otot, device=dev, dtype=torch.float32)
            N.call("dgv2_bias_act_bwd_rs", N.ptr(gpre), N.ptr(gb), N.ptr(gy), N.ptr(out), rows, Otot, cfg["alpha"],
                   cfg["scale"], N.ptr(cvec), N.ptr(scratch), scratch.numel(), _dt(gy),
                   N.stream())
            if not cfg["has_bias"]:
                gb = None
        else:
            g0 = gy
            if cfg["act"]:
                g0 = _bias_act_raw(gy, None, out, 1, cfg["alpha"], cfg["scale"], 1, Otot)
            if cfg["has_bias"]:
                gb = torch.empty(Otot, device=dev, dtype=torch.float32)
                N.call("dgv2_bias_grad", N.ptr(gb), N.ptr(g0), g0.numel(), 1, Otot, _dt(g0), N.stream())
            N.call("dgv2_scale_cast", N.ptr(gpre), N.ptr(g0), N.ptr(cvec), g0.numel(), Otot, _dt(g0), _dt(gpre),
                   N.stream())
        g3 = gpre.reshape(B, P, Otot)
        Ka = 0 if xa is None else xa.shape[3]
        gxa = None
        up = cfg.get("upstream")
        if xa is not None and ctx.needs_input_grad[1]:
            if wt is None:
                wt = wb[:, :, :Ka].transpose(1, 2).contiguous()
            resid = None if g_sib is None else g_sib.reshape(B, P, Ka)
            fused = None
            if up is not None and cfg["fork"] and not torch.is_grad_enabled():
                fused = _head_dgrad_actbwd(g3, wt, resid, xa, up)
            elif up is not None and resid is None and not torch.is_grad_enabled():
                fused = _dgrad_actbwd(g3, wt, xa, up)
            if fused is not None:
                gxa = fused.reshape(xa.shape)
            else:
                gxa = _bmm_nn_raw(g3, wt, xa.dtype, resid=resid).reshape(xa.shape)
        elif g_sib is not None:
            gxa = g_sib
        gwb = None
        if ctx.needs_input_grad[4]:
            gwb = _mod_wgrad(g3, xa, xs, B, H, W_, I, Otot, dt)
        return None, gxa, None, gb, gwb, None, None, None, None, None


_PE_TN_STREAM = os.environ.get("DGV2_PE_TN_STREAM") is not None


_PE_TN_MINP = int(os.environ.get("DGV2_PE_TN_MINP", "16384"))


_PE_WGRAD = os.environ.get("DGV2_NO_PE_WGRAD") is None
_PE_WGRAD_MINP = int(os.environ.get("DGV2_PE_WGRAD_MINP", "2048"))


def pe_wgrad(g3, xs, out=None, col0=0):
    B, P, O = g3.shape
    Ks = xs.shape[-1]
    if not (_PE_WGRAD and g3.dtype == torch.bfloat16 and xs.dtype == torch.bfloat16 and (P >= _PE_WGRAD_MINP)):
        return None
    n = _ct.c_int64(0)
    if N.lib.dgv2_pe_wgrad_scratch(_ct.byref(n), B, P, O, Ks) != 0 or n.value == 0:
        return None
    g3 = g3.contiguous()
    xs = xs.contiguous()
    ld = Ks if out is None else int(out.shape[2])
    if ld % 4 or col0 % 4 or ld < col0 + Ks:
        return None
    if out is None:
        out = torch.empty((B, O, Ks), device=g3.device, dtype=torch.float32)
    scratch = torch.empty(n.value, device=g3.device, dtype=torch.float32)
    N.check(g3, xs)
    N.call("dgv2_pe_wgrad", N.ptr(out), N.ptr(scratch), n.value, N.ptr(g3), N.ptr(xs), B, P, O, Ks, ld, int(col0), N.stream())
    return out


def _mod_wgrad(g3, xa, xs, B, H, W_, I, Otot, dt):
    P = H * W_
    Ka = 0 if xa is None else xa.shape[3]
    if (xs is not None and xa is not None and _LIB_WGRAD and dt == torch.bfloat16 and P >= 2048 and _TN_STREAM and Ka % 8 == 0
            and Otot % 8 == 0 and I % 4 == 0 and Ka % 4 == 0):
        gwb = torch.empty((B, Otot, I), device=g3.device, dtype=torch.float32)
        if pe_wgrad(g3, xs.reshape(P, -1), out=gwb, col0=Ka) is not None:
            _bmm_tn_stream(g3, xa, B, H, W_, Ka, Otot, out=gwb)
            return gwb
    if xs is not None and _LIB_WGRAD and dt == torch.bfloat16 and P >= 2048:
        gT = g3.transpose(1, 2)
        parts = []
        if xa is not None and _TN_STREAM and Ka % 8 == 0 and Otot % 8 == 0:
            parts.append(_bmm_tn_stream(g3, xa, B, H, W_, Ka, Otot))
        elif xa is not None:
            parts.append(torch.bmm(gT, xa.reshape(B, P, Ka), out_dtype=torch.float32))
        gws = pe_wgrad(g3, xs.reshape(P, -1))
        if gws is not None:
            parts.append(gws)
        elif _PE_TN_STREAM and Otot % 8 == 0 and P >= _PE_TN_MINP:
            parts.append(_bmm_tn_stream(g3, xs.contiguous(), B, H, W_, xs.shape[3], Otot, shared=True))
        else:
            parts.append(torch.bmm(gT, xs.reshape(1, P, -1).expand(B, P, xs.shape[3]), out_dtype=torch.float32))
        return torch.cat(parts, dim=2) if len(parts) > 1 else parts[0]
    if xs is not None:
        gwb = torch.empty((B, Otot, I), device=g3.device, dtype=torch.float32)
        N.call("dgv2_bmm_tn_cat", N.ptr(gwb), N.ptr(g3), N.ptr(xa), N.ptr(xs), B, P, Ka, xs.shape[3], Otot, _dt(xs),
               N.stream())
        return gwb
    if _TN_STREAM and dt == torch.bfloat16 and P >= 2048 and I % 8 == 0 and Otot % 8 == 0:
        return _bmm_tn_stream(g3, xa, B, H, W_, I, Otot)
    if Otot <= 4 and g3.dtype == xa.dtype:
        gwb = _bmm_tn_small(g3, xa, B, P, I, Otot)
        if gwb is not None:
            return gwb
    gwb = torch.empty((B, Otot, I), device=g3.device, dtype=torch.float32)
    N.call("dgv2_bmm_tn", N.ptr(gwb), N.ptr(g3), N.ptr(xa.reshape(B, P, I)), B, P, I, Otot, Otot, I, _dt(xa), N.stream())
    return gwb


_HEAD_ACT_BLOCKS = {}


_HEAD_ACTBWD = os.environ.get("DGV2_NO_HEAD_ACTBWD") is None


_DGRAD_ACTBWD = os.environ.get("DGV2_NO_DGRAD_ACTBWD") is None
_DGRAD_ACT_ROWS = {}


def _dgrad_actbwd(g3, wt, xa, up):
    B, P, O = g3.shape
    K = wt.shape[1]
    if (not _DGRAD_ACTBWD or g3.dtype != torch.bfloat16 or xa.dtype != torch.bfloat16 or wt.dtype != torch.bfloat16
            or K != O or K not in (32, 64) or tuple(wt.shape) != (B, K, O)
            or P < _PE_FREE_MINP.get((O, K), 1 << 30) or up.get("link") is None):
        return None
    key = (B, P, K)
    if key not in _DGRAD_ACT_ROWS:
        nr = _ct.c_int64(0)
        ok = N.try_call("dgv2_modconv_pe_dgrad_actbwd", None, None, None, 0, _ct.addressof(nr), None, None, None, None,
                        1.0, 1.0, B, P, K, N.BF16, N.stream())
        _DGRAD_ACT_ROWS[key] = nr.value if ok else 0
    rows = _DGRAD_ACT_ROWS[key]
    if rows == 0:
        return None
    g3 = g3.contiguous()
    xr = xa.contiguous()
    gpre = torch.empty((B, P, K), device=xa.device, dtype=xa.dtype)
    gb = torch.empty(K, device=xa.device, dtype=torch.float32)
    scratch = torch.empty(rows * K, device=xa.device, dtype=torch.float32)
    N.check(g3, wt, xr, up["cvec"])
    if not N.try_call("dgv2_modconv_pe_dgrad_actbwd", N.ptr(gpre), N.ptr(gb), N.ptr(scratch), scratch.numel(), None, N.ptr(g3),
                      N.ptr(wt), N.ptr(xr), N.ptr(up["cvec"]), up["alpha"], up["scale"], B, P, K, N.BF16, N.stream()):
        return None
    up["link"]["done"] = True
    up["link"]["gb"] = gb
    return gpre


def _head_dgrad_actbwd(g3, wt, resid, xa, up):
    B, P, Otot = g3.shape
    Ka = wt.shape[1]
    if not _HEAD_ACTBWD or Otot > 4 or g3.dtype != xa.dtype or wt.dtype != xa.dtype:
        return None
    key = (B, P, Otot, Ka, _dt(xa))
    if key not in _HEAD_ACT_BLOCKS:
        nb = _ct.c_int64(0)
        ok = N.try_call("dgv2_bmm_nn_small_act", None, None, None, None, B, P, Otot, Ka, None, None, 1.0, 1.0, None, None, 0,
                        _ct.addressof(nb), _dt(xa), N.stream())
        _HEAD_ACT_BLOCKS[key] = nb.value if ok else 0
    nblk = _HEAD_ACT_BLOCKS[key]
    if nblk == 0:
        return None
    r = None if resid is None else resid.contiguous().to(xa.dtype)
    xr = xa.contiguous()
    y = torch.empty((B, P, Ka), device=xa.device, dtype=xa.dtype)
    gb = torch.empty(Ka, device=xa.device, dtype=torch.float32)
    scratch = torch.empty(nblk * Ka, device=xa.device, dtype=torch.float32)
    N.check(g3, wt, r, xr, up["cvec"])
    N.call("dgv2_bmm_nn_small_act", N.ptr(y), N.ptr(g3), N.ptr(wt), N.ptr(r), B, P, Otot, Ka, N.ptr(xr), N.ptr(up["cvec"]),
           up["alpha"], up["scale"], N.ptr(gb), N.ptr(scratch), scratch.numel(), None, _dt(xa), N.stream())
    up["link"]["done"] = True
    up["link"]["gb"] = gb
    return y

_HEAD_BWD = os.environ.get("DGV2_NO_HEAD_BWD") is None


def _head_bwd_fused(gy, cvec, wt, resid, xa, up):
    B, Ka, Otot = wt.shape
    P = gy.numel() // (B * Otot)
    if (not (_HEAD_BWD and _HEAD_ACTBWD) or Otot > 4 or gy.dtype != torch.float32 or wt.dtype != xa.dtype
            or xa.dtype not in (torch.float32, torch.bfloat16)):
        return None
    key = ("head_bwd", B, P, Otot, Ka, _dt(xa))
    if key not in _HEAD_ACT_BLOCKS:
        nb = _ct.c_int64(0)
        ok = N.try_call("dgv2_head_bwd", None, None, None, None, None, 0, _ct.addressof(nb), None, None, None, None, None,
                        None, 1.0, 1.0, B, P, Otot, Ka, _dt(xa), N.stream())
        _HEAD_ACT_BLOCKS[key] = nb.value if ok else 0
    nblk = _HEAD_ACT_BLOCKS[key]
    if nblk == 0:
        return None
    r = None if resid is None else resid.contiguous().to(xa.dtype)
    xr = xa.contiguous()
    y = torch.empty_like(xr)
    gwb = torch.empty((B, Otot, Ka), device=xa.device, dtype=torch.float32)
    gbh = torch.empty(Otot, device=xa.device, dtype=torch.float32)
    gb_up = torch.empty(Ka, device=xa.device, dtype=torch.float32)
    scratch = torch.empty(nblk * (Ka + Otot * Ka + Otot), device=xa.device, dtype=torch.float32)
    N.check(gy, cvec, wt, r, xr, up["cvec"])
    if not N.try_call("dgv2_head_bwd", N.ptr(y), N.ptr(gwb), N.ptr(gbh), N.ptr(gb_up), N.ptr(scratch), scratch.numel(), None,
                      N.ptr(gy), N.ptr(cvec), N.ptr(wt), N.ptr(r), N.ptr(xr), N.ptr(up["cvec"]), up["alpha"], up["scale"],
                      B, P, Otot, Ka, _dt(xa), N.stream()):
        return None
    up["link"]["done"] = True
    up["link"]["gb"] = gb_up
    return y, gwb, gbh


__all__ = [n_ for n_ in dir() if not n_.startswith("__")]
```

include/dgv2.h:

```cpp
#ifndef DGV2_H
#define DGV2_H

#include <stdint.h>

#ifdef __cplusplus
extern "C" {
#endif

#define DGV2_F32 0
#define DGV2_BF16 1
#define DGV2_FP8 2
#define DGV2_EINVAL (-1)
#define DGV2_ENOTSUP (-3)

#define DGV2_STATUS_X_INEXACT 1
#define DGV2_STATUS_FIR_TABLE 2

int dgv2_abi_version(void);

int dgv2_fused_bias_act(void* y, const void* x, const void* bias, const void* ref,
                        int64_t size_x, int64_t step_b, int64_t size_b,
                        int act, int grad, float alpha, float scale, int dtype, void* stream);

int dgv2_bias_grad(float* gb, const void* x, int64_t size_x, int64_t step_b, int64_t size_b,
                   int dtype, void* stream);

int dgv2_bias_act_bwd(void* gx, float* gb, const void* gy, const void* ref, int64_t rows, int C,
                      float alpha, float scale, float* scratch, int64_t scratch_elems, int dtype,
                      void* stream);
int dgv2_bias_act_bwd_rs(void* gx, float* gb, const void* gy, const void* ref, int64_t rows, int C,
                         float alpha, float scale, const float* row_scale, float* scratch,
                         int64_t scratch_elems, int dtype, void* stream);
int dgv2_scale_cast(void* y, const void* x, const float* row_scale, int64_t n, int C, int xdtype, int ydtype,
                    void* stream);

int dgv2_upfirdn2d(void* out, const void* in, const float* kernel,
                   int major, int in_h, int in_w, int minor, int kh, int kw,
                   int up_x, int up_y, int down_x, int down_y,
                   int pad_x0, int pad_x1, int pad_y0, int pad_y1, int dtype, void* stream);

int dgv2_resample(void* y, const void* x, const float* taps_h, const float* taps_w,
                  int B, int H, int W, int C, int Ho, int Wo, int ldx, int ldy,
                  int kh, int up_h, int down_h, int p0_h,
                  int kw, int up_w, int down_w, int p0_w,
                  int ring, int adjoint, int dtype, void* stream);

int dgv2_resample_tab(void* y, const void* x, const int* idx_h, const float* coef_h, const int* cnt_h,
                      int Eh, const int* idx_w, const float* coef_w, const int* cnt_w, int Ew,
                      int B, int C, int ldx, int ldy, int in_h, int in_w, int out_h, int out_w,
                      int dtype, void* stream);

int dgv2_resample_tab_add(void* y, const void* x, const void* resid, const int* idx_h, const float* coef_h,
                          const int* cnt_h, int Eh, const int* idx_w, const float* coef_w, const int* cnt_w, int Ew,
                          int B, int C, int in_h, int in_w, int out_h, int out_w, int dtype, void* stream);
int dgv2_resample_tab_add_affine(void* y, const void* x, const void* resid, const float* rscale, const float* rbias,
                                 const int* idx_h, const float* coef_h, const int* cnt_h, int Eh, const int* idx_w,
                                 const float* coef_w, const int* cnt_w, int Ew, int B, int C, int in_h, int in_w, int out_h,
                                 int out_w, int dtype, void* stream);

int dgv2_resample_tab_sq(void* y, const void* x, const int* idx_h, const float* coef_h, const int* cnt_h,
                         int Eh, const int* idx_w, const float* coef_w, const int* cnt_w, int Ew,
                         int B, int C, int ldx, int ldy, int in_h, int in_w, int out_h, int out_w,
                         int dtype, float* sumsq, int sumsq_cap, int* sumsq_used, void* stream);

int dgv2_resample_tab_actbwd(void* y, float* gb, float* scratch, int64_t scratch_elems, int64_t* blocks_needed,
                             const void* x, const void* ref, const int* idx_h, const float* coef_h,
                             const int* cnt_h, int Eh, const int* idx_w, const float* coef_w, const int* cnt_w,
                             int Ew, int B, int C, int in_h, int in_w, int out_h, int out_w, float alpha,
                             float scale, int dtype, void* stream);

int dgv2_fir_same_mfma_prep(void* bands, int64_t bands_bytes, int64_t* bytes_needed, const int* idx_h, const float* coef_h,
                            const int* cnt_h, int Eh, const int* idx_w, const float* coef_w, const int* cnt_w, int Ew,
                            int H, int W, int* status, void* stream);
int dgv2_fir_same_mfma(void* y, const void* x, const void* bands, int B, int C, int H, int W, void* stream);
int dgv2_fir_same_mfma_actbwd(void* y, float* gb, float* scratch, int64_t scratch_elems, int64_t* blocks_needed,
                              const void* x, const void* ref, const void* bands, int B, int C, int H, int W, float alpha,
                              float scale, void* stream);

int dgv2_fourier_feature(void* out, const float* angle, const float* shift,
                         const float* freqs, const float* phase,
                         int B, int Ba, int H, int W, int F, int ld, int c0, int dtype, void* stream);

int dgv2_downsample_angle(float* out, const float* in, const float* shift, const float* taps,
                          int B, int Ba, int H, int W, int ring, void* stream);

int dgv2_bmm_nn(void* y, const void* x, const void* w, int B, int P, int I, int O,
                int ldx, int ldy, int64_t wstride, const float* bias, int act, float alpha, float scale,
                int dtype, int ydtype, void* stream);
int dgv2_bmm_tn(float* gw, const void* gy, const void* x, int B, int P, int I, int O,
                int ldgy, int ldx, int dtype, void* stream);

int dgv2_bmm_nn_cat(void* y, const void* xa, const void* xs, const void* w, int B, int P, int Ka, int Ks,
                    int O, const float* bias, int act, float alpha, float scale, int dtype, int ydtype,
                    void* stream);
int dgv2_modconv_up_fwd(void* y, const void* t, const void* xs, const void* wimg, int B, int Hout, int Wout, int Hin,
                        int Win, int Ks, int O, const int* idx_h, const float* coef_h, const int* idx_w,
                        const float* coef_w, const float* bias, const float* in_scale, int act, float alpha, float scale,
                        int dtype, float* sumsq, int sumsq_cap, int* sumsq_used, void* stream);
int dgv2_modconv_up_t(void* tcm, void* wimg, const void* h, const void* w, const float* row_scale, float gain, int B,
                      int Hlow, int Wlow, int Ka, int Ks, int O, int I, int koff, int dtype, void* stream);
int dgv2_modconv_up_t_lag(void* tcm, void* wimg, const void* h, const void* w, float gain, const float* ghd,
                          const float* gho, const float* gwd, const float* gwo, int B, int Hlow, int Wlow, int Ka, int Ks,
                          int O, int I, int koff, int dtype, float* sumsq, int sumsq_cap, int* sumsq_used, void* stream);
int dgv2_up2_lag_sumsq(const void* h, const float* ghd, const float* gho, const float* gwd, const float* gwo, int B,
                       int Hin, int Win, int C, int dtype, float* sumsq, int sumsq_cap, int* sumsq_used, void* stream);
int dgv2_bmm_nn_sq(void* y, const void* x, const void* w, int B, int P, int I, int O, int ldx, int ldy,
                   int64_t wstride, const float* row_scale, const float* bias, int act, float alpha, float scale,
                   const void* resid , int dtype, int ydtype,
                   float* sumsq, int sumsq_cap, int* sumsq_used, void* stream);
int dgv2_bmm_nn_cat_sq(void* y, const void* xa, const void* xs, const void* w, int B, int P, int Ka, int Ks,
                       int O, const float* row_scale, const float* bias, int act, float alpha, float scale, int dtype, int ydtype,
                       float* sumsq, int sumsq_cap, int* sumsq_used, void* stream);
int dgv2_bmm_tn_cat(float* gw, const void* gy, const void* xa, const void* xs, int B, int P, int Ka, int Ks,
                    int O, int dtype, void* stream);
int dgv2_bmm_tn_small(float* gw, const void* gy, const void* x, int B, int P, int I, int O, int dtype,
                      void* stream);
int dgv2_bmm_nn_small(void* y, const void* x, const void* w, const void* resid, int B, int P, int O, int K,
                      int dtype, void* stream);
int dgv2_bmm_nn_small_act(void* y, const void* x, const void* w, const void* resid, int B, int P, int O, int K,
                          const void* ref, const float* row_scale, float alpha, float ascale, float* gb,
                          float* scratch, int64_t scratch_elems, int64_t* blocks_needed, int dtype, void* stream);
int dgv2_head_bwd(void* y, float* gw, float* gbh, float* gb_up, float* scratch, int64_t scratch_elems,
                  int64_t* blocks_needed, const float* gyf, const float* cvec, const void* w, const void* resid,
                  const void* ref, const float* row_scale, float alpha, float ascale, int B, int P, int O, int K, int dtype,
                  void* stream);

int dgv2_modconv_pe_fwd(void* y, const void* xa, const void* xs, const void* w, int B, int P, int Ka, int Ks,
                        int O, const float* bias, int act, float alpha, float scale, int dtype, void* stream);
int dgv2_modconv_pe_fwd_sq(void* y, const void* xa, const void* xs, const void* w, int B, int P, int Ka, int Ks,
                           int O, const float* row_scale, const float* bias, int act, float alpha, float scale, int dtype, float* sumsq,
                           int sumsq_cap, int* sumsq_used, void* stream);
int dgv2_modconv_pe_fwd_head(void* y, const void* xa, const void* xs, const void* w, int B, int P, int Ka, int Ks,
                             int O, const float* row_scale, const float* bias, int act, float alpha, float scale, int dtype,
                             float* sumsq, int sumsq_cap, int* sumsq_used, const void* head_w, float* head_out, void* stream);

int dgv2_modconv_pe_dgrad_actbwd(void* gpre, float* gb, float* scratch, int64_t scratch_elems, int64_t* rows_needed,
                                 const void* gy, const void* wt, const void* yref, const float* up_scale, float alpha,
                                 float scale, int B, int P, int K, int dtype, void* stream);

int dgv2_lerp_list(float* const* dst, const float* const* src, const int* n, int L, float weight, void* stream);
int dgv2_adam_prep(float* sc, float* step, float b1, float b2, void* stream);
int dgv2_adam_step(float* const* p, const float* const* g, float* const* m, float* const* v, const int* n,
                   int L, const float* sc, float lr, float b1, float b2, float eps, void* stream);

int dgv2_pack2d(float* packed, const float* const* src, const int* rows, const int* cols, int L, int Rmax,
                int Cmax, void* stream);
int dgv2_unpack2d(float* const* dst, const float* packed, const int* rows, const int* cols, int L, int Rmax,
                  int Cmax, void* stream);

int dgv2_ema_scalar(float* ema, float* snapshot, const float* sumsq, int nsum, float add, float inv_count,
                    float weight, int update, float* cvec, int ncvec, void* stream);
int dgv2_ema_scalar_group(float* const* emas, const int* rows, int n, const float* sumsq, int nsum, float add,
                          float inv_count, float weight, int update, float* cvec, void* stream);
int dgv2_mod_prep_fwd(void* wb, float* dsave, float* stats, const float* W, const float* s,
                      const float* ema_var, const float* shift, const float* fw, int B, int O, int I,
                      int Otot, int row_off, int demod, int cin, int F, int wb_dtype, void* stream);
int dgv2_mod_prep_bwd(float* gW, float* gs, float* corr, const float* G, const float* W, const float* s,
                      const float* stats, const float* dsave, const float* ema_var, const float* shift,
                      const float* fw, int B, int O, int I, int Otot, int row_off, int demod, int cin,
                      int F, int corr_elems, void* stream);

int dgv2_mod_prep_all_fwd(void* const* wb, float* const* dsave, float* stats, float* rot, const float* const* W,
                          const float* const* s, const float* const* fw, const int* O, const int* I,
                          const int* Otot, const int* row_off, const int* cin, const int* flags,
                          const float* shift, int B, int L, void* stream);
int dgv2_mod_prep_all_bwd(float* flat, int64_t flat_elems, float* const* out, const int* ncorr,
                          const float* const* G, const float* const* W, const float* const* s,
                          const float* stats, const float* rot, float* const* dsave,
                          const float* const* fw, const int* O, const int* I, const int* Otot,
                          const int* row_off, const int* cin, const int* flags, const float* shift, int B,
                          int L, float* scratch, int64_t scratch_elems, void* stream);
int dgv2_mod_prep_all_bwd_scratch(int64_t* elems, const int* O, const int* I, int B, int L);

int dgv2_transpose_list(void* const* dst, const void* const* src, const int* rows, const int* cols,
                        const int* ld, int L, int B, int elem_size, void* stream);

int dgv2_sum_squares(float* acc, const void* x, int64_t N, int C, int ld, int dtype, void* stream);

int dgv2_mbstd_cat_fwd(void* out, float* scratch, const void* x, int B, int P, int C, int Cp, int splits,
                       int group, int dtype, void* stream);
int dgv2_mbstd_cat_bwd(void* gx, const void* gout, const void* x, int B, int P, int C, int Cp, int splits,
                       int group, int dtype, void* stream);
int dgv2_gemm_x3(float* c, float* scratch, int64_t scratch_elems, const float* a, const float* b, int I, int J,
                 int64_t T, int a_trans, int b_trans, int64_t lda, int64_t ldb, int64_t ldo, int splits, float scale,
                 void* stream);
int dgv2_pe_wgrad_scratch(int64_t* elems, int B, int P, int O, int Ks);
int dgv2_pe_wgrad(float* gw, float* scratch, int64_t scratch_elems, const void* g, const void* pe, int B, int P, int O,
                  int Ks, int64_t ldo, int col0, void* stream);
int dgv2_mbstd_cat_fwd_x(void* out, float* scratch, const void* x, int B, int P, int C, int Cp, int splits, int group,
                         int xdtype, int ydtype, void* stream);
int dgv2_mbstd_cat_bwd_x(void* gx, const void* gout, const void* x, int B, int P, int C, int Cp, int splits, int group,
                         int xdtype, int gdtype, void* stream);

int dgv2_conv_fwd(void* y, const void* x, const void* w, int B, int H, int W, int C, int O,
                  int kh, int kw, int stride, int pad, int ring,
                  const float* bias, int act, float alpha, float scale, int dtype, void* stream);
int dgv2_conv_dgrad(void* gx, void* gxp_scratch, const void* gy, const void* wt,
                    int B, int H, int W, int C, int O,
                    int kh, int kw, int stride, int pad, int ring, int dtype, void* stream);
int dgv2_conv_wgrad(float* gw, const void* gy, const void* x, int B, int H, int W, int C, int O,
                    int kh, int kw, int stride, int pad, int ring, int dtype, void* stream);

int dgv2_conv_wgrad_direct(float* gw, const void* gy, const void* x, int B, int H, int W, int C, int O,
                           int k, int stride, int pad, int ring, int dtype, void* stream);

int dgv2_bmm_tn_stream_scratch(int64_t* elems, int B, int H, int W, int C, int O, int dtype);
int dgv2_bmm_tn_stream(float* gw, float* scratch, int64_t scratch_elems, const void* gy, const void* x,
                       int B, int H, int W, int C, int O, int dtype, void* stream);
int dgv2_bmm_tn_stream_x(float* gw, float* scratch, int64_t scratch_elems, const void* gy, const void* x,
                         int x_shared, int B, int H, int W, int C, int O, int dtype, void* stream);
int dgv2_bmm_tn_stream_ld(float* gw, int64_t ldo, float* scratch, int64_t scratch_elems, const void* gy, const void* x,
                          int x_shared, int B, int H, int W, int C, int O, int dtype, void* stream);

int dgv2_conv_weight_bank(void* const* wf, void* const* wt, const float* const* src, const int* O,
                          const int* C, const int* Cpad, const int* kk, const float* scale, int L,
                          int dtype, void* stream);
int dgv2_conv_weight_bank_ex(void* const* wf, void* const* wt, void* const* w8, void* const* w8t,
                             const float* const* src, const int* O, const int* C, const int* Cpad, const int* kk,
                             const float* scale, int L, int dtype, void* stream);
int dgv2_conv3x3_fwd8(void* y, const void* x, const void* w8, int B, int Hin, int Win, int Cin, int O, int stride,
                      const float* bias, const void* resid, int act, float alpha, float scale, int dtype, void* stream);
int dgv2_conv3x3_dgrad8(void* gx, const void* gy, const void* w8t, int B, int H, int W, int C, int O, const void* resid,
                        int dtype, void* stream);
int dgv2_conv3x3_s2_dgrad8(void* gx, const void* gy, const void* wt, int B, int Hg, int Wg, int C, int O, int dtype,
                           void* stream);

int dgv2_conv3x3_x3_fwd(void* y, const void* x, const void* w3, int B, int H, int W, int Cx, int x_exact, int O,
                        const float* bias, const void* resid, int act, float alpha, float scale, int* status,
                        void* stream);
int dgv2_conv3x3_x3_dgrad(void* gx, const void* gy, const void* w3t, const void* wt, int B, int H, int W, int C, int ldx,
                          int O, const void* resid, void* stream);
int dgv2_conv3x3_x3_wgrad(float* gw, float* scratch, int64_t scratch_elems, const void* gy, const void* x, int B, int H,
                          int W, int C, int clive, int x_exact, int O, float scale, int param_layout, int* status,
                          void* stream);
int dgv2_conv3x3_x3_wgrad_scratch(int64_t* elems, int B, int H, int W, int C, int clive, int O);
int dgv2_conv_x3_images(void* w3, void* w3t, const void* w, int O, int Cp, void* stream);

int dgv2_conv_wgrad_stream_scratch(int64_t* elems, int B, int H, int W, int C, int O, int k, int stride,
                                   int pad, int dtype);
int dgv2_conv_wgrad_stream(float* gw, float* scratch, int64_t scratch_elems, const void* gy, const void* x,
                           int B, int H, int W, int C, int O, int k, int stride, int pad, int ring,
                           int dtype, void* stream);
int dgv2_conv_wgrad_stream_pl(float* gw, float* scratch, int64_t scratch_elems, const void* gy, const void* x,
                              int B, int H, int W, int C, int O, int k, int stride, int pad, int ring,
                              float scale, int param_layout, int dtype, void* stream);

int dgv2_conv_taps(void* y, const void* x, const void* w, int B, int Hin, int Win, int Cin,
                   int Hg, int Wg, int O, int Hy, int Wy, int in_stride, int ioff_h, int ioff_w,
                   int out_stride, int ooff_h, int ooff_w, int ntaps, int wtaps, const int* taps_host,
                   int hzero, int ring, int accumulate, const float* bias, const void* resid, int act,
                   float alpha, float scale, int dtype, void* stream);
int dgv2_conv_taps_ex(void* y, const void* x, const void* w, int B, int Hin, int Win, int Cin, int Hg,
                      int Wg, int O, int Hy, int Wy, int in_stride, int ioff_h, int ioff_w,
                      int out_stride, int ncls, const int* cls_host, int ntaps, int wtaps,
                      const int* taps_host, int nextra, const int* extras_host, int hzero, int ring,
                      int accumulate, const float* bias, const void* resid, int act, float alpha,
                      float scale, int dtype, void* stream);
int dgv2_conv_taps_ld(void* y, int ldy, const void* x, const void* w, int B, int Hin, int Win, int Cin, int Hg,
                      int Wg, int O, int Hy, int Wy, int in_stride, int ioff_h, int ioff_w, int out_stride, int ncls,
                      const int* cls_host, int ntaps, int wtaps, const int* taps_host, int nextra,
                      const int* extras_host, int hzero, int ring, int accumulate, const float* bias,
                      const void* resid, int act, float alpha, float scale, int dtype, void* stream);

int dgv2_conv1x1_fwd(void* y, const void* x, const void* wf, int B, int P, int C, int O, const void* resid, int dtype,
                     void* stream);
int dgv2_conv1x1_dgrad(void* gx, const void* gy, const void* wt, int B, int P, int C, int O, const void* resid,
                       int dtype, void* stream);

int dgv2_stem_fwd(void* y, const float* x, const float* w, const float* bias, int B, int H, int W, int O,
                  int ring, float alpha, float scale, int ydtype, void* stream);
int dgv2_stem_bwd_scratch(int64_t* elems, int B, int H, int W, int O);
int dgv2_stem_bwd(float* gx, float* gw, float* gb, float* scratch, int64_t scratch_elems, const void* gy,
                  const void* y, const float* x, const float* w, int B, int H, int W, int O, int ring,
                  float alpha, float scale, int dtype, void* stream);
int dgv2_stem_bwd_skip(float* gx, float* gw, float* gb, float* scratch, int64_t scratch_elems, const void* gy, const void* y,
                       const float* x, const float* w, const void* gsk, const int* idx_h, const float* coef_h,
                       const int* cnt_h, int Eh, const int* idx_w, const float* coef_w, const int* cnt_w, int Ew, int Hs,
                       int Ws, int B, int H, int W, int O, int ring, float alpha, float scale, int dtype, void* stream);

int dgv2_gen_tail_fwd(float* image, float* image_orig, float* logit, float* mask,
                      const float* skip, const float* shift, const float* u,
                      int B, int H, int W, float out_scale, float raydrop_const, float temperature,
                      void* stream);
int dgv2_gen_tail_bwd(float* g_skip, float* scratch, const float* g_image, const float* g_image_orig,
                      const float* g_logit, const float* g_mask,
                      const float* image_orig, const float* logit, const float* mask, const float* u,
                      const float* shift, int B, int H, int W, float out_scale, float raydrop_const,
                      float temperature, void* stream);

int dgv2_ada_apply(float* y, const float* x, const float* Ay, const float* kx, const int* off,
                   const int* sgn, const float* a, const float* c, int B, int H, int W, int K,
                   int transpose, void* stream);

int dgv2_ada_sample(float* gaff, float* a, float* c, const float* u, const float* n, const float* p,
                    const float* policy_host, int B, int H, int W, void* stream);
int dgv2_ada_build(float* Ay, float* kx, int* off, int* sgn, const float* gaff, const float* M1y,
                   const float* M1x, const float* taps, int B, int H, int W, int K, void* stream);

int dgv2_ada_sample_img(float* g, float* sigma, float* cut, const float* u2, const float* n2, const float* p,
                        const float* policy_host, int B, void* stream);
int dgv2_ada_fold(float* Ay2, float* kx2, int* off2, float* c2, const float* Ay, const float* kx, const int* off,
                  const int* sgn, const float* c, const float* g, const float* fbank, int B, int H, int W, int K,
                  int NB, int T, void* stream);
int dgv2_ada_apply_img(float* y, const float* x, const float* Ay, const float* kx, const int* off, const int* sgn,
                       const float* a, const float* c, const float* cut, const float* sigma, const float* eps, int B,
                       int H, int W, int K, int transpose, void* stream);

int dgv2_coords_convert(float* out, const float* in, const float* mask, const float* angle,
                        int B, int H, int W, float min_depth, float max_depth, float raydrop_const,
                        int mode, void* stream);

int dgv2_surface_normal(float* out, const float* points, int B, int H, int W, int d, int mode, void* stream);

int dgv2_nsgan_loss(float* stats, float* gy, const float* y, int n_real, int n_fake, float gy_scale, float* sign_cum,
                    float* n_cum, void* stream);

int dgv2_d_tail_fwd(float* y, float* a, const float* h, const float* b1, const float* w2, const float* b2, int B, int K,
                    float alpha, float act_scale, float scale2, float gain2, void* stream);
int dgv2_d_tail_bwd(float* gh, float* gb1, float* gw2, float* gb2, const float* gy, const float* a, const float* w2,
                    int B, int K, float alpha, float act_scale, float scale2, float gain2, void* stream);

int dgv2_colmean_lerp(float* dst, const float* src, int B, int K, int64_t ld, float w, void* stream);

int dgv2_rng_fill(float* const* out, const int64_t* count, const int* kind, const float* a, const float* b, int nseg,
                  uint64_t* state, void* stream);

int dgv2_kitti_rows(int* row, int* counts, const float* pts, int n, int H, void* stream);
int dgv2_kitti_project(float* out, unsigned long long* key, const float* pts, const int* row, int n, int H, int W,
                       int Wout, float min_depth, float max_depth, int apply_mask, void* stream);

int dgv2_fps_scratch(int64_t* floats, int B, int n);
int dgv2_fps(int* idxs, float* temp, const float* xyz, int B, int n, int m, void* stream);
int dgv2_gather_points(float* out, const float* points, const int* idx, int B, int C, int n, int m, void* stream);
int dgv2_gather_points_grad(float* grad_points, const float* grad_out, const int* idx, int B, int C, int n, int m,
                            void* stream);

int dgv2_chamfer_fwd(float* dist1, int* idx1, float* dist2, int* idx2, const float* xyz1, const float* xyz2, int B,
                     int n, int m, void* stream);
int dgv2_nn_search(float* dist, int* idx, const float* xyz, const float* ref, int B, int n, int m, int ref_shared,
                   void* stream);
int dgv2_chamfer_bwd(float* gxyz1, float* gxyz2, const float* xyz1, const float* xyz2, const float* gdist1,
                     const float* gdist2, const int* idx1, const int* idx2, int B, int n, int m, void* stream);

int dgv2_emd_approxmatch(float* match, float* temp, const float* xyz1, const float* xyz2, int B, int n, int m,
                         void* stream);
int dgv2_emd_matchcost(float* cost, const float* match, const float* xyz1, const float* xyz2, int B, int n, int m,
                       void* stream);
int dgv2_emd_matchcost_grad(float* grad1, float* grad2, const float* match, const float* xyz1, const float* xyz2, int B,
                            int n, int m, void* stream);

int dgv2_fir_same_mfma_q8(void* y8, const void* x, const void* bands, int B, int C, int H, int W, void* stream);
int dgv2_resample_tab_q8(void* y8, const void* x, const int* idx_h, const float* coef_h, const int* cnt_h, int Eh,
                         const int* idx_w, const float* coef_w, const int* cnt_w, int Ew, int B, int C, int in_h,
                         int in_w, int out_h, int out_w, void* stream);
int dgv2_fp8_quant_weights(void* const* w8, const void* const* src, const int* O, const int* C, const int* kk,
                           const float* eq, int n, float* descale, void* amax, void* stream);
int dgv2_fp8_dequant(void* y, const void* x, int64_t n, float scale, void* stream);
int dgv2_conv_taps_fp8(void* y, const void* x8, const void* w8, const float* acc_scale, int B, int Hin, int Win, int Cin,
                       int Hg, int Wg, int O, int Hy, int Wy, int in_stride, int ioff_h, int ioff_w, int ntaps, int wtaps,
                       const int* taps_host, int ring, const float* bias, const void* resid, int act, float alpha,
                       float scale, void* stream);

int dgv2_glin_fwd(float* const* y, const float* const* x, const float* const* w, const float* const* bias, const int* N,
                  const int* lda, int L, int B, int K, float alpha, float beta, int act, float slope, int prenorm,
                  float* rnorm, void* stream);
int dgv2_glin_dinput(float* dx, int ldx, float* scratch, int64_t scratch_elems, const float* const* g,
                     const float* const* yact, const float* const* w, const int* N, int L, int B, int K, float alpha,
                     float slope, int accumulate, void* stream);
int dgv2_glin_dweight(float* const* dw, float* const* dbias, const float* const* g, const float* const* yact,
                      const float* const* x, const int* N, const int* ldx, int L, int B, int K, float alpha, float beta,
                      float slope, const float* rnorm, void* stream);

int dgv2_msml_prepare(float* refp, float* maskp, float* normp, float* invm, const float* ref, const float* mask, int B,
                      int C, int H, int W, int L, void* stream);
int dgv2_msml_fwd(float* loss, float* genp, const float* gen, const float* refp, const float* maskp, const float* normp,
                  const float* invm, int B, int C, int H, int W, int L, int metric, int relative, void* stream);
int dgv2_msml_bwd(float* ggen, float* gscratch, const float* gloss, const float* gen, const float* genp,
                  const float* refp, const float* maskp, const float* normp, const float* invm, int B, int C, int H, int W,
                  int L, int metric, int relative, void* stream);
int dgv2_coords_convert_bwd(float* gx, const float* gout, const float* in, const float* mask, const float* angle, int B,
                            int H, int W, float min_depth, float max_depth, int mode, void* stream);
int dgv2_fourier_feature_bwd(float* g_angle, const void* g, const float* angle, const float* shift, const float* freqs,
                             const float* phase, int B, int Ba, int H, int W, int F, int ld, int c0, int dtype,
                             void* stream);

int dgv2_frame_points(float* points, float* colors, const float* image, const float* angle, int B, int H, int W,
                      float min_depth, float max_depth, int border, void* stream);
int dgv2_colorize(float* out, const float* x, const float* lut, int B, int H, int W, int n_colors, void* stream);

int dgv2_crf_rnn_forward(float* out, float* qsave, const float* unary, const float* xyz, const float* mask,
                         const float* kernel_gamma, const float* kernel_alpha, const float* theta_beta,
                         const float* weight_smoothness, const float* weight_appearance, const float* compat, int B,
                         int C, int H, int W, int kh, int kw, int num_iters, void* stream);
int dgv2_crf_rnn_backward_scratch(int64_t* elems, int B, int C, int H, int W, int num_iters);
int dgv2_crf_rnn_backward(float* g_unary, float* g_weight_smoothness, float* g_weight_appearance, float* g_compat,
                          float* scratch, int64_t scratch_elems, const float* g_out, const float* qsave,
                          const float* unary, const float* xyz, const float* mask, const float* kernel_gamma,
                          const float* kernel_alpha, const float* theta_beta, const float* weight_smoothness,
                          const float* weight_appearance, const float* compat, int B, int C, int H, int W, int kh,
                          int kw, int num_iters, void* stream);

int dgv2_knn2d(int64_t* out, const float* depth, const int64_t* label, const float* dist_kernel, int B, int H, int W,
               int kh, int kw, int k, int num_classes, float cutoff, void* stream);
int dgv2_seg_confusion(int64_t* conf, const int64_t* label, const int64_t* pred, const float* mask, int64_t n,
                       int num_classes, void* stream);

#ifdef __cplusplus
}
#endif
#endif
```

Baseline: 5692 range-images/s.

## Add register-staged streaming bf16 GEMM kernels for nn and tn batched matmuls

Adds new bf16 GEMM kernels for the batched nn, nn_cat, tn and tn_cat paths. They stage several K-steps per pass, prefetch the next stage from global memory into registers while MFMAs run, double-buffer the weight tile in swizzled LDS, and stream B fragments straight into registers. Python wrappers try these kernels first under geometry conditions and fall back to the existing bmm kernels when they return not-supported. The aim is to hide global-memory latency and cut LDS traffic on the large modulated-conv GEMMs, at the cost of higher register pressure, lower occupancy and more dispatch paths to keep correct.

```diff
diff --git a/dusty-gan-v2_amd/csrc/api.hip b/dusty-gan-v2_amd/csrc/api.hip
--- a/dusty-gan-v2_amd/csrc/api.hip
+++ b/dusty-gan-v2_amd/csrc/api.hip
@@ -1,3 +1,3 @@
 #include "common.h"
 
-extern "C" int dgv2_abi_version(void) { return 53; }
+extern "C" int dgv2_abi_version(void) { return 54; }
diff --git a/dusty-gan-v2_amd/csrc/gemm.hip b/dusty-gan-v2_amd/csrc/gemm.hip
--- a/dusty-gan-v2_amd/csrc/gemm.hip
+++ b/dusty-gan-v2_amd/csrc/gemm.hip
@@ -121,9 +121,7 @@
                            int dtype, void* stream) {
   if (!gw || !gy || !x || B <= 0 || P <= 0 || I <= 0 || O <= 0 || ldgy < O || ldx < I) return DGV2_EINVAL;
   hipStream_t st = (hipStream_t)stream;
-  const int tiles = B * ((O + 63) / 64) * ((I + 127) / 128);
-  int ksplit = 1;
-  while (tiles * ksplit < 512 && P / (ksplit * 2) >= 512) ksplit *= 2;
+  const int ksplit = bmm_tn_ksplit(B, P, I, O);
   if (ksplit > 1) {
     hipError_t e = hipMemsetAsync(gw, 0, sizeof(float) * (size_t)B * O * I, st);
     if (e != hipSuccess) return (int)e;
@@ -169,9 +167,7 @@
   if (Ka % ce || Ks % ce || !aligned16(xs) || (Ka > 0 && !aligned16(xa))) return DGV2_EINVAL;
   hipStream_t st = (hipStream_t)stream;
   const int J = Ka + Ks;
-  const int tiles = B * ((O + 63) / 64) * ((J + 127) / 128);
-  int ksplit = 1;
-  while (tiles * ksplit < 512 && P / (ksplit * 2) >= 512) ksplit *= 2;
+  const int ksplit = bmm_tn_ksplit(B, P, J, O);
   if (ksplit > 1) {
     hipError_t e = hipMemsetAsync(gw, 0, sizeof(float) * (size_t)B * O * J, st);
     if (e != hipSuccess) return (int)e;
diff --git a/dusty-gan-v2_amd/csrc/gemm_core.h b/dusty-gan-v2_amd/csrc/gemm_core.h
--- a/dusty-gan-v2_amd/csrc/gemm_core.h
+++ b/dusty-gan-v2_amd/csrc/gemm_core.h
@@ -464,6 +464,13 @@
   }
 };
 
+static inline int bmm_tn_ksplit(int B, int P, int J, int O) {
+  const int tiles = B * ((O + 63) / 64) * ((J + 127) / 128);
+  int ksplit = 1;
+  while (tiles * ksplit < 512 && P / (ksplit * 2) >= 512) ksplit *= 2;
+  return ksplit;
+}
+
 template <typename T, int TO, int TJ, class ALoad, class BLoad>
 __global__ __launch_bounds__(256) void gemm_tn_kernel(ALoad al, BLoad bl, float* __restrict__ out, int M, int J,
                                                       int64_t K, int64_t klen, int ksplit, int64_t out_batch_stride,
diff --git a/dusty-gan-v2_amd/csrc/gemm_stream.hip b/dusty-gan-v2_amd/csrc/gemm_stream.hip
--- /dev/null
+++ b/dusty-gan-v2_amd/csrc/gemm_stream.hip
@@ -0,0 +1,340 @@
+#include <type_traits>
+
+#include "gemm_core.h"
+
+namespace {
+
+constexpr int kStageSteps = 4;
+
+struct RowSrc {
+  const bf16_t* a;
+  int64_t a_batch_stride;
+  int lda, Ka;
+  const bf16_t* s;
+  int lds_, rows, K;
+};
+__device__ __forceinline__ uint4 ld16(const bf16_t* base , unsigned off ) {
+  return *reinterpret_cast<const uint4*>(base + off);
+}
+__device__ __forceinline__ uint4 zero_past(uint4 v, int64_t k, int64_t K) {
+  const unsigned keep = k < K ? ~0u : 0u;
+  return make_uint4(v.x & keep, v.y & keep, v.z & keep, v.w & keep);
+}
+struct ColSrc {
+  const bf16_t* a;
+  int64_t a_batch_stride;
+  int lda, Ca;
+  const bf16_t* s;
+  int lds_, cols;
+  __device__ __forceinline__ uint4 load(int batch, int64_t k, int64_t K, int colchunk) const {
+    const int64_t kk = k < K ? k : K - 1;
+    const int col = min(colchunk * 8, cols - 8);
+    const bf16_t* pa = a + batch * a_batch_stride + kk * lda + col;
+    const bf16_t* ps = s + kk * lds_ + (col - Ca);
+    return *reinterpret_cast<const uint4*>(col < Ca ? pa : ps);
+  }
+};
+
+template <class Epi, bool BATCH_FAST>
+__global__ __launch_bounds__(256, 2) void gemm_nn_stream_kernel(RowSrc al, RowSrc bl, Epi epi, int K) {
+  constexpr int TO = 128, TP = 128, MF = TO / 16, NF = 2, KT = kStageSteps;
+  constexpr int ROWCH = 4 * KT;
+  constexpr int ACH = TO * ROWCH / 256;
+  __shared__ __attribute__((aligned(16))) uint4 ldsA[2][TO * ROWCH];
+
+  const int tid = threadIdx.x;
+  const int wave = tid >> 6, lane = tid & 63;
+  const int lr = lane & 15, lc = lane >> 4;
+  const int batch = BATCH_FAST ? blockIdx.x : blockIdx.z;
+  const int m0 = blockIdx.y * TO;
+  const int n0 = (BATCH_FAST ? blockIdx.z : blockIdx.x) * TP;
+  const int nk = K >> 5;
+  const int ns = (nk + KT - 1) / KT;
+
+  uint4 ra[ACH], rb[KT][NF];
+  auto swz = [](int row, int ch) { return row * ROWCH + (ch ^ (row & (ROWCH - 1))); };
+  const bf16_t* abase = al.a + batch * al.a_batch_stride;
+  const bf16_t* bbase_a = bl.a + batch * bl.a_batch_stride;
+  unsigned offA[ACH], offBa[NF], offBs[NF];
+#pragma unroll
+  for (int i = 0; i < ACH; ++i) offA[i] = (unsigned)min(m0 + (tid + i * 256) / ROWCH, al.rows - 1) * (unsigned)al.lda;
+#pragma unroll
+  for (int nf = 0; nf < NF; ++nf) {
+    const unsigned r = (unsigned)min(n0 + wave * 32 + nf * 16 + lr, bl.rows - 1);
+    offBa[nf] = r * (unsigned)bl.lda + lc * 8;
+    offBs[nf] = r * (unsigned)bl.lds_ + lc * 8;
+  }
+  auto gloadA = [&](int s) {
+    const unsigned k = (unsigned)min(s * (32 * KT) + (tid % ROWCH) * 8, K - 8);
+#pragma unroll
+    for (int i = 0; i < ACH; ++i) ra[i] = ld16(abase, offA[i] + k);
+  };
+  auto gloadB = [&](int s, int kt) {
+    const int k0 = min((s * KT + kt) * 32, K - 32);
+    const bool side_a = k0 < bl.Ka;
+    const bf16_t* base = side_a ? bbase_a : bl.s;
+    const unsigned k = (unsigned)(side_a ? k0 : k0 - bl.Ka);
+#pragma unroll
+    for (int nf = 0; nf < NF; ++nf) rb[kt][nf] = ld16(base, (side_a ? offBa[nf] : offBs[nf]) + k);
+  };
+  auto lstore = [&](int buf) {
+#pragma unroll
+    for (int i = 0; i < ACH; ++i) {
+      const int id = tid + i * 256;
+      ldsA[buf][swz(id / ROWCH, id % ROWCH)] = ra[i];
+    }
+  };
+
+  f32x4 acc[MF][NF];
+#pragma unroll
+  for (int mf = 0; mf < MF; ++mf)
+#pragma unroll
+    for (int nf = 0; nf < NF; ++nf) acc[mf][nf] = (f32x4){0.f, 0.f, 0.f, 0.f};
+
+  gloadA(0);
+#pragma unroll
+  for (int kt = 0; kt < KT; ++kt) gloadB(0, kt);
+  lstore(0);
+  __syncthreads();
+  auto steps = [&](auto knc, auto prec, int s, int cur) {
+    constexpr int KN = decltype(knc)::value;
+    constexpr bool PRE = decltype(prec)::value;
+#pragma unroll
+    for (int kt = 0; kt < KN; ++kt) {
+      uint4 a[MF];
+#pragma unroll
+      for (int mf = 0; mf < MF; ++mf) a[mf] = ldsA[cur][swz(mf * 16 + lr, kt * 4 + lc)];
+#pragma unroll
+      for (int mf = 0; mf < MF; ++mf)
+#pragma unroll
+        for (int nf = 0; nf < NF; ++nf) Mfma16<bf16_t>::run(acc[mf][nf], a[mf], rb[kt][nf]);
+      if (PRE) {
+        __builtin_amdgcn_sched_barrier(0);
+        gloadB(s + 1, kt);
+        __builtin_amdgcn_sched_barrier(0);
+      }
+    }
+  };
+  int cur = 0;
+  for (int s = 0; s + 1 < ns; ++s) {
+    gloadA(s + 1);
+    __builtin_amdgcn_sched_barrier(0);
+    steps(std::integral_constant<int, KT>(), std::true_type(), s, cur);
+    lstore(cur ^ 1);
+    __syncthreads();
+    cur ^= 1;
+  }
+  {
+    const int kn = nk - (ns - 1) * KT;
+    if (kn >= KT) steps(std::integral_constant<int, KT>(), std::false_type(), ns - 1, cur);
+    else if (kn == 3) steps(std::integral_constant<int, 3>(), std::false_type(), ns - 1, cur);
+    else if (kn == 2) steps(std::integral_constant<int, 2>(), std::false_type(), ns - 1, cur);
+    else steps(std::integral_constant<int, 1>(), std::false_type(), ns - 1, cur);
+  }
+  __syncthreads();
+#pragma unroll
+  for (int mf = 0; mf < MF; ++mf)
+#pragma unroll
+    for (int nf = 0; nf < NF; ++nf)
+      epi(batch, m0 + mf * 16 + lc * 4, n0 + wave * 32 + nf * 16 + lr, acc[mf][nf]);
+  if (epi.sumsq) {
+    float* red = reinterpret_cast<float*>(&ldsA[0][0]);
+    const float s = block_sum(epi.ss, red);
+    if (tid == 0) epi.sumsq[(blockIdx.z * gridDim.y + blockIdx.y) * gridDim.x + blockIdx.x] = s;
+  }
+}
+
+__global__ __launch_bounds__(256, 3) void gemm_tn_stream_kernel(ColSrc al, ColSrc bl, float* __restrict__ out, int M, int J,
+                                                             int64_t K, int64_t out_batch_stride, int ldo) {
+  constexpr int TO = 64, TJ = 128, KS = 32, CE = 8, KT = kStageSteps;
+  constexpr int MF = TO / 16, NF = TJ / 64;
+  constexpr int ACH_ROW = TO / CE, BCH_ROW = TJ / CE;
+  constexpr int ACH = KT * KS * ACH_ROW / 256, BCH = KT * KS * BCH_ROW / 256;
+  constexpr int OLD = TJ + 4;
+  static_assert(TO * OLD * 4 <= KT * KS * (TO + TJ) * 2, "the output tile reuses the operand image");
+  __shared__ __attribute__((aligned(16))) bf16_t lds[KT * KS * (TO + TJ)];
+  bf16_t* ldsA = lds;
+  bf16_t* ldsB = lds + KT * KS * TO;
+
+  const int tid = threadIdx.x;
+  const int wave = tid >> 6, lane = tid & 63;
+  const int batch = blockIdx.z;
+  const int m0 = blockIdx.y * TO;
+  const int j0 = blockIdx.x * TJ;
+  const int nk = (int)((K + KS - 1) / KS);
+  const int ns = (nk + KT - 1) / KT;
+
+  uint4 ra[ACH], rb[BCH];
+  auto gload = [&](int s) {
+    const int64_t kb = (int64_t)s * (KT * KS);
+#pragma unroll
+    for (int i = 0; i < ACH; ++i) {
+      const int id = tid + i * 256;
+      ra[i] = al.load(batch, kb + id / ACH_ROW, K, (m0 / CE) + id % ACH_ROW);
+    }
+#pragma unroll
+    for (int i = 0; i < BCH; ++i) {
+      const int id = tid + i * 256;
+      rb[i] = bl.load(batch, kb + id / BCH_ROW, K, (j0 / CE) + id % BCH_ROW);
+    }
+  };
+  auto lstore = [&](int s) {
+    const int64_t kb = (int64_t)s * (KT * KS);
+#pragma unroll
+    for (int i = 0; i < ACH; ++i)
+      reinterpret_cast<uint4*>(ldsA)[tid + i * 256] = zero_past(ra[i], kb + (tid + i * 256) / ACH_ROW, K);
+#pragma unroll
+    for (int i = 0; i < BCH; ++i)
+      reinterpret_cast<uint4*>(ldsB)[tid + i * 256] = zero_past(rb[i], kb + (tid + i * 256) / BCH_ROW, K);
+  };
+
+  f32x4 acc[MF][NF];
+#pragma unroll
+  for (int mf = 0; mf < MF; ++mf)
+#pragma unroll
+    for (int nf = 0; nf < NF; ++nf) acc[mf][nf] = (f32x4){0.f, 0.f, 0.f, 0.f};
+
+  auto step = [&](int kt) {
+    uint4 a[MF], b[NF];
+#pragma unroll
+    for (int mf = 0; mf < MF; ++mf) a[mf] = TnFrag<bf16_t>::template read<TO>(ldsA + kt * KS * TO, mf * 16, lane);
+#pragma unroll
+    for (int nf = 0; nf < NF; ++nf)
+      b[nf] = TnFrag<bf16_t>::template read<TJ>(ldsB + kt * KS * TJ, wave * (TJ / 4) + nf * 16, lane);
+#pragma unroll
+    for (int mf = 0; mf < MF; ++mf)
+#pragma unroll
+      for (int nf = 0; nf < NF; ++nf) Mfma16<bf16_t>::run(acc[mf][nf], a[mf], b[nf]);
+  };
+
+  if (ns > 0) {
+    gload(0);
+    lstore(0);
+  }
+  __syncthreads();
+  for (int s = 0; s < ns; ++s) {
+    if (s + 1 < ns) gload(s + 1);
+    const int kn = nk - s * KT;
+    if (kn >= KT) {
+#pragma unroll
+      for (int kt = 0; kt < KT; ++kt) step(kt);
+    } else {
+      for (int kt = 0; kt < kn; ++kt) step(kt);
+    }
+    __syncthreads();
+    if (s + 1 < ns) {
+      lstore(s + 1);
+      __syncthreads();
+    }
+  }
+  float* ot = reinterpret_cast<float*>(lds);
+  const int lr = lane & 15, lc = lane >> 4;
+#pragma unroll
+  for (int mf = 0; mf < MF; ++mf)
+#pragma unroll
+    for (int nf = 0; nf < NF; ++nf)
+#pragma unroll
+      for (int r = 0; r < 4; ++r) ot[(mf * 16 + lc * 4 + r) * OLD + wave * (TJ / 4) + nf * 16 + lr] = acc[mf][nf][r];
+  __syncthreads();
+  float* ob = out + batch * out_batch_stride;
+#pragma unroll
+  for (int i = 0; i < TO * (TJ / 4) / 256; ++i) {
+    const int id = tid + i * 256;
+    const int m = id / (TJ / 4), jv = (id % (TJ / 4)) * 4;
+    if (m0 + m >= M || j0 + jv >= J) continue;
+    *reinterpret_cast<f32x4*>(ob + (int64_t)(m0 + m) * ldo + j0 + jv) = *reinterpret_cast<const f32x4*>(ot + m * OLD + jv);
+  }
+}
+
+bool nn_geometry(int dtype, int ydtype, int K, int O) {
+  return dtype == DGV2_BF16 && ydtype == DGV2_BF16 && O > 64 && K % 32 == 0;
+}
+
+int take_sumsq(StoreEpilogue<bf16_t>& epi, dim3 grid, float* sumsq, int sumsq_cap, int* sumsq_used) {
+  const int64_t nblk = (int64_t)grid.x * grid.y * grid.z;
+  if (sumsq && sumsq_used && nblk <= sumsq_cap) {
+    epi.sumsq = sumsq;
+    *sumsq_used = (int)nblk;
+  }
+  return 0;
+}
+
+}
+
+extern "C" int dgv2_gemm_stream_nn(void* y, const void* x, const void* w, int B, int P, int I, int O, int ldx, int ldy,
+                                   int64_t wstride, const float* row_scale, const float* bias, int act, float alpha,
+                                   float scale, const void* resid, int dtype, int ydtype, float* sumsq, int sumsq_cap,
+                                   int* sumsq_used, void* stream) {
+  if (sumsq_used) *sumsq_used = 0;
+  if (!y || !x || !w || B <= 0 || P <= 0 || I <= 0 || O <= 0 || ldx < I || ldy < O) return DGV2_EINVAL;
+  if (act != 0 && act != 3) return DGV2_EINVAL;
+  if (!nn_geometry(dtype, ydtype, I, O) || (int64_t)P * ldx >= (1ll << 31) || (int64_t)O * I >= (1ll << 31) || ldx % 8 || wstride % 8 || ldy % 4 || !aligned16(y) || !aligned16(x) || !aligned16(w)
+      || (resid && !aligned16(resid)))
+    return DGV2_ENOTSUP;
+  typedef bf16_t T;
+  RowSrc al{(const T*)w, wstride, I, I, (const T*)w, I, O, I};
+  RowSrc bl{(const T*)x, (int64_t)P * ldx, ldx, I, (const T*)x, ldx, P, I};
+  StoreEpilogue<T> epi{(T*)y, (int64_t)P * ldy, ldy, O, P, true, bias, act, alpha, scale, nullptr, 0.f, row_scale, (const T*)resid};
+  dim3 grid((P + 127) / 128, (O + 127) / 128, B);
+  take_sumsq(epi, grid, sumsq, sumsq_cap, sumsq_used);
+  gemm_nn_stream_kernel<StoreEpilogue<T>, false>
+      <<<grid, 256, 0, (hipStream_t)stream>>>(al, bl, epi, I);
+  DGV2_RETURN_LAST();
+}
+
+extern "C" int dgv2_gemm_stream_nn_cat(void* y, const void* xa, const void* xs, const void* w, int B, int P, int Ka, int Ks,
+                                       int O, const float* row_scale, const float* bias, int act, float alpha, float scale,
+                                       int dtype, int ydtype, float* sumsq, int sumsq_cap, int* sumsq_used, void* stream) {
+  if (sumsq_used) *sumsq_used = 0;
+  if (!y || !xs || !w || (Ka > 0 && !xa) || B <= 0 || P <= 0 || Ka < 0 || Ks <= 0 || O <= 0) return DGV2_EINVAL;
+  if (act != 0 && act != 3) return DGV2_EINVAL;
+  if (dtype != DGV2_BF16 && dtype != DGV2_F32) return DGV2_EINVAL;
+  const int ce = dtype == DGV2_BF16 ? 8 : 4;
+  if (Ka % ce || Ks % ce || !aligned16(xs) || (Ka > 0 && !aligned16(xa)) || !aligned16(w) || !aligned16(y))
+    return DGV2_EINVAL;
+  if (!nn_geometry(dtype, ydtype, Ka + Ks, O) || O % 4 || Ka % 32 || (int64_t)P * (Ka > Ks ? Ka : Ks) >= (1ll << 31)
+      || (int64_t)O * (Ka + Ks) >= (1ll << 31))
+    return DGV2_ENOTSUP;
+  typedef bf16_t T;
+  const int K = Ka + Ks;
+  RowSrc al{(const T*)w, (int64_t)O * K, K, K, (const T*)w, K, O, K};
+  RowSrc bl{(const T*)xa, (int64_t)P * Ka, Ka, Ka, (const T*)xs, Ks, P, K};
+  StoreEpilogue<T> epi{(T*)y, (int64_t)P * O, O, O, P, true, bias, act, alpha, scale, nullptr, 0.f, row_scale};
+  dim3 grid(B, (O + 127) / 128, (P + 127) / 128);
+  take_sumsq(epi, grid, sumsq, sumsq_cap, sumsq_used);
+  gemm_nn_stream_kernel<StoreEpilogue<T>, true>
+      <<<grid, 256, 0, (hipStream_t)stream>>>(al, bl, epi, K);
+  DGV2_RETURN_LAST();
+}
+
+extern "C" int dgv2_gemm_stream_tn(float* gw, const void* gy, const void* x, int B, int P, int I, int O, int ldgy, int ldx,
+                                   int dtype, void* stream) {
+  if (!gw || !gy || !x || B <= 0 || P <= 0 || I <= 0 || O <= 0 || ldgy < O || ldx < I) return DGV2_EINVAL;
+  if (dtype != DGV2_BF16 && dtype != DGV2_F32) return DGV2_EINVAL;
+  if (dtype != DGV2_BF16 || O <= 32 || bmm_tn_ksplit(B, P, I, O) != 1 || I % 8 || O % 8 || ldgy % 8 || ldx % 8 || !aligned16(gw)
+      || !aligned16(gy) || !aligned16(x))
+    return DGV2_ENOTSUP;
+  typedef bf16_t T;
+  ColSrc al{(const T*)gy, (int64_t)P * ldgy, ldgy, O, (const T*)gy, ldgy, O};
+  ColSrc bl{(const T*)x, (int64_t)P * ldx, ldx, I, (const T*)x, ldx, I};
+  dim3 grid((I + 127) / 128, (O + 63) / 64, B);
+  gemm_tn_stream_kernel<<<grid, 256, 0, (hipStream_t)stream>>>(al, bl, gw, O, I, P, (int64_t)O * I, I);
+  DGV2_RETURN_LAST();
+}
+
+extern "C" int dgv2_gemm_stream_tn_cat(float* gw, const void* gy, const void* xa, const void* xs, int B, int P, int Ka,
+                                       int Ks, int O, int dtype, void* stream) {
+  if (!gw || !gy || !xs || (Ka > 0 && !xa) || B <= 0 || P <= 0 || Ka < 0 || Ks <= 0 || O <= 0) return DGV2_EINVAL;
+  if (dtype != DGV2_BF16 && dtype != DGV2_F32) return DGV2_EINVAL;
+  const int ce = dtype == DGV2_BF16 ? 8 : 4;
+  if (Ka % ce || Ks % ce || !aligned16(xs) || (Ka > 0 && !aligned16(xa))) return DGV2_EINVAL;
+  const int J = Ka + Ks;
+  if (dtype != DGV2_BF16 || O <= 32 || O % 8 || bmm_tn_ksplit(B, P, J, O) != 1 || !aligned16(gw) || !aligned16(gy))
+    return DGV2_ENOTSUP;
+  typedef bf16_t T;
+  ColSrc al{(const T*)gy, (int64_t)P * O, O, O, (const T*)gy, O, O};
+  ColSrc bl{(const T*)xa, (int64_t)P * Ka, Ka, Ka, (const T*)xs, Ks, J};
+  dim3 grid((J + 127) / 128, (O + 63) / 64, B);
+  gemm_tn_stream_kernel<<<grid, 256, 0, (hipStream_t)stream>>>(al, bl, gw, O, J, P, (int64_t)O * J, J);
+  DGV2_RETURN_LAST();
+}
diff --git a/dusty-gan-v2_amd/dgv2_native/__init__.py b/dusty-gan-v2_amd/dgv2_native/__init__.py
--- a/dusty-gan-v2_amd/dgv2_native/__init__.py
+++ b/dusty-gan-v2_amd/dgv2_native/__init__.py
@@ -7,7 +7,7 @@
 LIB_PATH = os.environ.get("DGV2_LIB_PATH") or os.path.join(os.path.dirname(_HERE), "lib", "libdgv2.so")
 
 F32, BF16 = 0, 1
-ABI_VERSION = 53
+ABI_VERSION = 54
 
 _c_int, _c_i64, _c_f32, _c_ptr = ctypes.c_int, ctypes.c_int64, ctypes.c_float, ctypes.c_void_p
 
@@ -111,6 +111,12 @@
     "dgv2_conv_wgrad_direct": [_c_ptr] * 3 + [_c_int] * 10 + [_c_ptr],
     "dgv2_conv1x1_fwd": [_c_ptr] * 3 + [_c_int] * 4 + [_c_ptr, _c_int, _c_ptr],
     "dgv2_conv1x1_dgrad": [_c_ptr] * 3 + [_c_int] * 4 + [_c_ptr, _c_int, _c_ptr],
+    "dgv2_gemm_stream_nn": [_c_ptr] * 3 + [_c_int] * 6 + [_c_i64, _c_ptr, _c_ptr, _c_int, _c_f32, _c_f32, _c_ptr, _c_int, _c_int, _c_ptr,
+                            _c_int, _c_ptr, _c_ptr],
+    "dgv2_gemm_stream_nn_cat": [_c_ptr] * 4 + [_c_int] * 5 + [_c_ptr, _c_ptr, _c_int, _c_f32, _c_f32, _c_int, _c_int, _c_ptr, _c_int,
+                                _c_ptr, _c_ptr],
+    "dgv2_gemm_stream_tn": [_c_ptr] * 3 + [_c_int] * 7 + [_c_ptr],
+    "dgv2_gemm_stream_tn_cat": [_c_ptr] * 4 + [_c_int] * 6 + [_c_ptr],
     "dgv2_bmm_tn_stream_scratch": [_c_ptr] + [_c_int] * 6,
     "dgv2_bmm_tn_stream": [_c_ptr, _c_ptr, _c_i64, _c_ptr, _c_ptr] + [_c_int] * 6 + [_c_ptr],
     "dgv2_bmm_tn_stream_x": [_c_ptr, _c_ptr, _c_i64, _c_ptr, _c_ptr] + [_c_int] * 7 + [_c_ptr],
diff --git a/dusty-gan-v2_amd/gans/models/ops/native/misc.py b/dusty-gan-v2_amd/gans/models/ops/native/misc.py
--- a/dusty-gan-v2_amd/gans/models/ops/native/misc.py
+++ b/dusty-gan-v2_amd/gans/models/ops/native/misc.py
@@ -365,8 +365,7 @@
                     gwa = _bmm_tn_stream(gt3, h, B, hl, wl, Ka, Otot)
                 else:
                     gwa = torch.empty((B, Otot, Ka), device=dev, dtype=torch.float32)
-                    N.call("dgv2_bmm_tn", N.ptr(gwa), N.ptr(gt3), N.ptr(h3), B, hl * wl, Ka, Otot, Otot, Ka, _dt(h),
-                           N.stream())
+                    bmm_tn_call(N.ptr(gwa), N.ptr(gt3), N.ptr(h3), B, hl * wl, Ka, Otot, Otot, Ka, _dt(h), N.stream())
                 gws = _mod_wgrad(g3, None, xs, B, H, W_, xs.shape[3], Otot, dt)
                 gwb = torch.cat([gwa, gws], dim=2)
         return None, gh, None, gb, gwb, None, None, None, None, None
diff --git a/dusty-gan-v2_amd/gans/models/ops/native/modgemm.py b/dusty-gan-v2_amd/gans/models/ops/native/modgemm.py
--- a/dusty-gan-v2_amd/gans/models/ops/native/modgemm.py
+++ b/dusty-gan-v2_amd/gans/models/ops/native/modgemm.py
@@ -298,6 +298,34 @@
     _PE_FREE_MINP = {k: 4096 for k in ((64, 32), (32, 64), (128, 64), (64, 128), (32, 32), (64, 64))}
 
 
+_GEMM_STREAM = os.environ.get("DGV2_NO_GEMM_STREAM") is None
+_GEMM_STREAM_MAX_P = 512
+
+
+def _stream_wanted(P, per_sample=True):
+    return _GEMM_STREAM and per_sample and P <= _GEMM_STREAM_MAX_P
+
+
+def bmm_nn_sq_call(*args):
+    if not (_stream_wanted(args[4], args[9] != 0) and N.try_call("dgv2_gemm_stream_nn", *args)):
+        N.call("dgv2_bmm_nn_sq", *args)
+
+
+def bmm_nn_cat_sq_call(*args):
+    if not (_stream_wanted(args[5]) and N.try_call("dgv2_gemm_stream_nn_cat", *args)):
+        N.call("dgv2_bmm_nn_cat_sq", *args)
+
+
+def bmm_tn_call(*args):
+    if not (_stream_wanted(args[4]) and N.try_call("dgv2_gemm_stream_tn", *args)):
+        N.call("dgv2_bmm_tn", *args)
+
+
+def bmm_tn_cat_call(*args):
+    if not (_stream_wanted(args[5]) and N.try_call("dgv2_gemm_stream_tn_cat", *args)):
+        N.call("dgv2_bmm_tn_cat", *args)
+
+
 def _bmm_nn_raw(x3, w3, out_dtype, bias=None, act=0, alpha=0.2, scale=1.0, sq=None, row_scale=None, resid=None, head=None):
     B, P, I = x3.shape
     Bw, O, _ = w3.shape
@@ -329,12 +357,15 @@
         if resid is not None:
             resid = resid.contiguous().to(out_dtype)
             N.check(resid)
-        N.call("dgv2_bmm_nn_sq", N.ptr(y), N.ptr(x3), N.ptr(w3), B, P, I, O, I, O, 0 if Bw == 1 else O * I,
-               N.ptr(row_scale), N.ptr(bias), act, alpha, scale, N.ptr(resid), _dt(x3), N.dtype_code(y),
-               N.ptr(sq[0]) if sq else None, _SQ_CAP if sq else 0, _ct.addressof(sq[1]) if sq else None, N.stream())
+        bmm_nn_sq_call(N.ptr(y), N.ptr(x3), N.ptr(w3), B, P, I, O, I, O, 0 if Bw == 1 else O * I,
+                       N.ptr(row_scale), N.ptr(bias), act, alpha, scale, N.ptr(resid), _dt(x3), N.dtype_code(y),
+                       N.ptr(sq[0]) if sq else None, _SQ_CAP if sq else 0, _ct.addressof(sq[1]) if sq else None, N.stream())
         return y
-    N.call("dgv2_bmm_nn", N.ptr(y), N.ptr(x3), N.ptr(w3), B, P, I, O, I, O, 0 if Bw == 1 else O * I,
-           N.ptr(bias), act, alpha, scale, _dt(x3), N.dtype_code(y), N.stream())
+    if not (_stream_wanted(P, Bw == B) and N.try_call("dgv2_gemm_stream_nn", N.ptr(y), N.ptr(x3), N.ptr(w3), B, P, I, O, I, O,
+                                        0 if Bw == 1 else O * I, None, N.ptr(bias), act, alpha, scale, None, _dt(x3),
+                                        N.dtype_code(y), None, 0, None, N.stream())):
+        N.call("dgv2_bmm_nn", N.ptr(y), N.ptr(x3), N.ptr(w3), B, P, I, O, I, O, 0 if Bw == 1 else O * I,
+               N.ptr(bias), act, alpha, scale, _dt(x3), N.dtype_code(y), N.stream())
     return y
 
 
@@ -343,7 +374,7 @@
     I = x3.shape[2]
     N.check(gy3, x3)
     gw = torch.empty((B, O, I), device=x3.device, dtype=torch.float32)
-    N.call("dgv2_bmm_tn", N.ptr(gw), N.ptr(gy3), N.ptr(x3), B, P, I, O, O, I, _dt(x3), N.stream())
+    bmm_tn_call(N.ptr(gw), N.ptr(gy3), N.ptr(x3), B, P, I, O, O, I, _dt(x3), N.stream())
     return gw
 
 
@@ -425,8 +456,8 @@
         bias32 = bias.detach().float().contiguous()
         N.check(xa, xs, wc, bias32)
         out = torch.empty((B, H, W_, O), device=xs.device, dtype=xs.dtype)
-        N.call("dgv2_bmm_nn_cat", N.ptr(out), N.ptr(xa), N.ptr(xs), N.ptr(wc), B, H * W_, Ka, Ks, O, N.ptr(bias32),
-               3, alpha, scale, _dt(xs), _dt(xs), N.stream())
+        bmm_nn_cat_sq_call(N.ptr(out), N.ptr(xa), N.ptr(xs), N.ptr(wc), B, H * W_, Ka, Ks, O, None, N.ptr(bias32),
+                           3, alpha, scale, _dt(xs), _dt(xs), None, 0, None, N.stream())
         ctx.save_for_backward(xa, xs, wc, out)
         ctx.cfg = (alpha, scale, Ka, Ks)
         return out
@@ -444,8 +475,7 @@
             gxa = _bmm_nn_raw(g3, wt, xa.dtype).reshape(xa.shape)
         if ctx.needs_input_grad[2]:
             gw = torch.empty((B, O, Ka + Ks), device=out.device, dtype=torch.float32)
-            N.call("dgv2_bmm_tn_cat", N.ptr(gw), N.ptr(g3), N.ptr(xa), N.ptr(xs), B, H * W_, Ka, Ks, O, _dt(xs),
-                   N.stream())
+            bmm_tn_cat_call(N.ptr(gw), N.ptr(g3), N.ptr(xa), N.ptr(xs), B, H * W_, Ka, Ks, O, _dt(xs), N.stream())
         return gxa, None, gw, gb, None, None
 
 
diff --git a/dusty-gan-v2_amd/gans/models/ops/native/modlayer.py b/dusty-gan-v2_amd/gans/models/ops/native/modlayer.py
--- a/dusty-gan-v2_amd/gans/models/ops/native/modlayer.py
+++ b/dusty-gan-v2_amd/gans/models/ops/native/modlayer.py
@@ -70,10 +70,10 @@
                        Otot, None, N.ptr(bias32), act, cfg["alpha"], cfg["scale"], _dt(xs), N.ptr(sq[0]) if sq else None,
                        _SQ_CAP if sq else 0, _ct.addressof(sq[1]) if sq else None, N.stream())
             else:
-                N.call("dgv2_bmm_nn_cat_sq", N.ptr(out), N.ptr(xa), N.ptr(xs), N.ptr(wb), B, P, Ka, xs.shape[3], Otot,
-                       None, N.ptr(bias32), act, cfg["alpha"], cfg["scale"], _dt(xs), _dt(xs),
-                       N.ptr(sq[0]) if sq else None, _SQ_CAP if sq else 0, _ct.addressof(sq[1]) if sq else None,
-                       N.stream())
+                bmm_nn_cat_sq_call(N.ptr(out), N.ptr(xa), N.ptr(xs), N.ptr(wb), B, P, Ka, xs.shape[3], Otot,
+                                   None, N.ptr(bias32), act, cfg["alpha"], cfg["scale"], _dt(xs), _dt(xs),
+                                   N.ptr(sq[0]) if sq else None, _SQ_CAP if sq else 0,
+                                   _ct.addressof(sq[1]) if sq else None, N.stream())
         else:
             xa = xa.contiguous()
             out = _bmm_nn_raw(xa.reshape(B, P, I), wb, odt, bias32, act, cfg["alpha"], cfg["scale"], sq=sq).reshape(
@@ -132,14 +132,12 @@
             pass
         elif xs is not None:
             gwb = torch.empty((B, Otot, I), device=gy.device, dtype=torch.float32)
-            N.call("dgv2_bmm_tn_cat", N.ptr(gwb), N.ptr(g3), N.ptr(xa), N.ptr(xs), B, P, Ka, xs.shape[3], Otot,
-                   _dt(xs), N.stream())
+            bmm_tn_cat_call(N.ptr(gwb), N.ptr(g3), N.ptr(xa), N.ptr(xs), B, P, Ka, xs.shape[3], Otot, _dt(xs), N.stream())
         elif _TN_STREAM and dt == torch.bfloat16 and P >= 2048 and I % 8 == 0 and Otot % 8 == 0:
             gwb = _bmm_tn_stream(g3, xa, B, H, W_, I, Otot)
         else:
             gwb = torch.empty((B, Otot, I), device=gy.device, dtype=torch.float32)
-            N.call("dgv2_bmm_tn", N.ptr(gwb), N.ptr(g3), N.ptr(xa.reshape(B, P, I)), B, P, I, Otot, Otot, I, _dt(xa),
-                   N.stream())
+            bmm_tn_call(N.ptr(gwb), N.ptr(g3), N.ptr(xa.reshape(B, P, I)), B, P, I, Otot, Otot, I, _dt(xa), N.stream())
         grads = []
         off = 0
         for k in range(nm):
@@ -298,8 +296,8 @@
                 N.call("dgv2_modconv_pe_fwd_sq", N.ptr(out), N.ptr(xa), N.ptr(xs), N.ptr(wb), B, P, Ka, xs.shape[3],
                        Otot, N.ptr(cvec), N.ptr(bias32), act, cfg["alpha"], cfg["scale"], _dt(xs), *tail)
             else:
-                N.call("dgv2_bmm_nn_cat_sq", N.ptr(out), N.ptr(xa), N.ptr(xs), N.ptr(wb), B, P, Ka, xs.shape[3], Otot,
-                       N.ptr(cvec), N.ptr(bias32), act, cfg["alpha"], cfg["scale"], _dt(xs), _dt(xs), *tail)
+                bmm_nn_cat_sq_call(N.ptr(out), N.ptr(xa), N.ptr(xs), N.ptr(wb), B, P, Ka, xs.shape[3], Otot,
+                                   N.ptr(cvec), N.ptr(bias32), act, cfg["alpha"], cfg["scale"], _dt(xs), _dt(xs), *tail)
         elif pre_d is not None and not cfg["act"] and not cfg["want_sq"]:
             xa = xa.contiguous()
             if cfg.get("defer_affine"):
@@ -458,8 +456,7 @@
         return torch.cat(parts, dim=2) if len(parts) > 1 else parts[0]
     if xs is not None:
         gwb = torch.empty((B, Otot, I), device=g3.device, dtype=torch.float32)
-        N.call("dgv2_bmm_tn_cat", N.ptr(gwb), N.ptr(g3), N.ptr(xa), N.ptr(xs), B, P, Ka, xs.shape[3], Otot, _dt(xs),
-               N.stream())
+        bmm_tn_cat_call(N.ptr(gwb), N.ptr(g3), N.ptr(xa), N.ptr(xs), B, P, Ka, xs.shape[3], Otot, _dt(xs), N.stream())
         return gwb
     if _TN_STREAM and dt == torch.bfloat16 and P >= 2048 and I % 8 == 0 and Otot % 8 == 0:
         return _bmm_tn_stream(g3, xa, B, H, W_, I, Otot)
@@ -468,7 +465,7 @@
         if gwb is not None:
             return gwb
     gwb = torch.empty((B, Otot, I), device=g3.device, dtype=torch.float32)
-    N.call("dgv2_bmm_tn", N.ptr(gwb), N.ptr(g3), N.ptr(xa.reshape(B, P, I)), B, P, I, Otot, Otot, I, _dt(xa), N.stream())
+    bmm_tn_call(N.ptr(gwb), N.ptr(g3), N.ptr(xa.reshape(B, P, I)), B, P, I, Otot, Otot, I, _dt(xa), N.stream())
     return gwb
 
 
diff --git a/include/dgv2.h b/include/dgv2.h
--- a/include/dgv2.h
+++ b/include/dgv2.h
@@ -267,6 +267,18 @@
 int dgv2_conv1x1_dgrad(void* gx, const void* gy, const void* wt, int B, int P, int C, int O, const void* resid,
                        int dtype, void* stream);
 
+int dgv2_gemm_stream_nn(void* y, const void* x, const void* w, int B, int P, int I, int O, int ldx, int ldy,
+                        int64_t wstride, const float* row_scale, const float* bias, int act, float alpha, float scale,
+                        const void* resid, int dtype, int ydtype, float* sumsq, int sumsq_cap, int* sumsq_used,
+                        void* stream);
+int dgv2_gemm_stream_nn_cat(void* y, const void* xa, const void* xs, const void* w, int B, int P, int Ka, int Ks, int O,
+                            const float* row_scale, const float* bias, int act, float alpha, float scale, int dtype,
+                            int ydtype, float* sumsq, int sumsq_cap, int* sumsq_used, void* stream);
+int dgv2_gemm_stream_tn(float* gw, const void* gy, const void* x, int B, int P, int I, int O, int ldgy, int ldx, int dtype,
+                        void* stream);
+int dgv2_gemm_stream_tn_cat(float* gw, const void* gy, const void* xa, const void* xs, int B, int P, int Ka, int Ks, int O,
+                            int dtype, void* stream);
+
 int dgv2_stem_fwd(void* y, const float* x, const float* w, const float* bias, int B, int H, int W, int O,
                   int ring, float alpha, float scale, int ydtype, void* stream);
 int dgv2_stem_bwd_scratch(int64_t* elems, int B, int H, int W, int O);
```

After: 5755 range-images/s, median of 6. 1.01x the previous value.
